# JINXER000/GIE-mapping

Measured on AMD Instinct MI355X. Metric: edt_map_update_throughput, higher is better.
Workload: dtype int32; 1 GPU; 512x512x512 @ 0.05 m, sensor-less hash world (BASELINE config 5): occupied iff hash(x,y,z) < 1 %, full observation, 25 ~; preset=c5, fast_mode=False, tiles=single volume, blocks=360448

## Files before the change

gie-mapping_amd/csrc/gie_api.inc.h:

```cpp
#include <stdio.h>
#include <stdlib.h>
#include <string.h>
#include <math.h>
#include <string>
#include <vector>

enum { GIE_K_CLASSIFY = 0, GIE_K_RAY_REGISTER, GIE_K_RAY_FREE, GIE_K_RAY_FINAL, GIE_K_ALLOC, GIE_K_FUSE, GIE_K_EDT_Y, GIE_K_EDT_X,
       GIE_K_EDT_Z, GIE_K_MARK, GIE_K_FRONTIER, GIE_K_WAVE_A, GIE_K_WAVE_B, GIE_K_WAVE_C, GIE_K_COMMIT, GIE_K_EDT_ZFACES, GIE_K_MARKC, GIE_K_NUM };
#include <cstdio>
#include <unistd.h>
static const char *const gie_kernel_names[GIE_K_NUM] = { "ogm_classify", "ray_register", "ray_free", "ray_finalize", "block_alloc", "fuse",
       "edt_pass_y", "edt_pass_x", "edt_pass_z", "mark", "frontiers", "wave_a", "wave_b", "waves", "commit", "edt_prep", "mark_commit" };

#define GIE_REHASH_PERIOD 64
static thread_local std::string g_gie_err;
static void gie_set_err(const std::string &s) { g_gie_err = s; }
extern "C" const char *gie_last_error(void) { return g_gie_err.c_str(); }

enum gie_owed {
    GIE_OWED_NONE,
    GIE_OWED_FRESH,
    GIE_OWED_STALE
};
struct gie_pivots { int pvt[3], upvt[3], tb0[3]; };
struct gie_pair_state {
    gie_owed owed = GIE_OWED_NONE;
    gie_pivots last = {};
    int flushed_ct = -1;
    int coc_pending = 0;
    int lazy_pending = 0;
    uint32_t *bcoc_alt = nullptr;
    int tsp_pvt[3] = {};
    int fuse_fresh = 0;
    int track_want = 0;
};
struct gie_mapper {
    gie_config cfg;
    gie_ctx c;
    be_state be;
    int ncell;
    int has_pose, has_ogm, merge_open;
    int bar_fault_left;
    gie_pair_state pp;
    int pool_base;
    int evictions;
    long long tomb_bound;
    int retain_box_valid, retain_box_lo[3], retain_box_hi[3];
    int32_t *blk_tab2; int tab_valid, tab_tb0[3];
    int edt_partial;
    int ogm_unlabelled;
    float msg_origin[3];
    float *d_sensor; size_t sensor_cap;
    float *d_pts_g; size_t pts_cap;
    float *d_box_ll, *d_box_ur; uint8_t *d_box_act; int box_cap;
    int32_t *d_rank;
    int32_t *d_srank, *d_slist;
    void *d_stage[2], *h_stage[2];
    std::vector<void *> allocs;
    void *scratch[2]; size_t scratch_cap[2];
    int32_t h_cnt[GIE_CNT_NUM];
    int32_t next_off[3], next_whole[3];
    float us[4];
    const int8_t *labels_pending;
    gie_seendist *d_cm; void *h_cm[2]; size_t cm_bytes; int cm_slot, cm_pending;
    long long *d_round_stats;
};

template <class T> static T *gie_dalloc(gie_mapper *m, size_t n, bool zero = true)
{
    void *p = be_alloc(&m->be, n * sizeof(T), zero);
    if (p) m->allocs.push_back(p);
    {
        static const int dbg = GIE_SWITCH("GIE_DEBUG_ALLOC", 0);
        if (dbg && (dbg > 1 || n * sizeof(T) >= (64u << 20))) fprintf(stderr, "[%d] gie alloc %2d: %p  %8.1f MiB\n", (int)getpid(), (int)m->allocs.size(), p, (double)(n * sizeof(T)) / 1048576.0);
    }
    return (T *)p;
}

static void *gie_scratch(gie_mapper *m, int i, size_t bytes, const char *who)
{
    if (bytes > m->scratch_cap[i]) {
        if (m->scratch[i]) be_free(&m->be, m->scratch[i]);
        m->scratch[i] = be_alloc(&m->be, bytes, false);
        m->scratch_cap[i] = m->scratch[i] ? bytes : 0;
    }
    if (!m->scratch[i]) gie_set_err(std::string(who) + ": device allocation of the export buffer failed");
    return m->scratch[i];
}

#define GIE_SCRATCH_KEEP ((size_t)64 << 20)
static void gie_scratch_trim(gie_mapper *m)
{
    for (int i = 0; i < 2; i++)
        if (m->scratch[i] && m->scratch_cap[i] > GIE_SCRATCH_KEEP) { be_free(&m->be, m->scratch[i]); m->scratch[i] = nullptr; m->scratch_cap[i] = 0; }
}

static void gie_place_calibrate(gie_mapper *m, size_t N, size_t GV)
{
    const int tries = m->cfg.place_tries;
    if (tries <= 1 || N < ((size_t)1 << 24) || !m->c.g_coc || !m->c.pair || !m->c.bcoc || !m->c.glb_type) return;
    gie_ctx &c = m->c;
    (void)be_place_probe(&m->be, c, 12);
    float best = be_place_probe(&m->be, c, 5);
    if (best <= 0.f) return;
    const float first = best;
    struct plane { void **pp; size_t bytes; bool zero; } planes[4] = {
        { reinterpret_cast<void **>(&c.g_coc), GV * sizeof(uint64_t), false }, { reinterpret_cast<void **>(&c.pair), N * sizeof(uint64_t), true },
        { reinterpret_cast<void **>(&c.bcoc), N * sizeof(uint32_t), true }, { reinterpret_cast<void **>(&c.glb_type), N, true } };
    int swaps = 0;
    for (plane &pl : planes) {
        for (int t = 1; t < tries; t++) {
            void *alt = be_alloc(&m->be, pl.bytes, pl.zero);
            if (!alt) break;
            void *old = *pl.pp;
            *pl.pp = alt;
            const float ms = be_place_probe(&m->be, c, 5);
            bool take = ms > 0.f && ms < 0.985f * best;
            if (take) {
                *pl.pp = old;
                const float again = be_place_probe(&m->be, c, 5);
                *pl.pp = alt;
                take = again > 0.f && ms < 0.985f * again;
                if (!take && again > 0.f) best = again;
            }
            if (take) {
                best = ms; swaps++;
                for (void *&q : m->allocs) if (q == old) q = alt;
                be_free(&m->be, old);
            } else { *pl.pp = old; be_free(&m->be, alt); }
        }
    }
    if (GIE_SWITCH("GIE_DEBUG_ALLOC", 0)) fprintf(stderr, "[%d] gie placement: probe %.4f -> %.4f ms after %d re-draws\n", (int)getpid(), first, best, swaps);
}

static int gie_pow2_ge(long long v) { int p = 1; while ((long long)p < v) p <<= 1; return p; }

#define GIE_MAX_POOL_BLOCKS (1 << 26)
static void gie_pp_init(gie_mapper *m); static void gie_pp_pose(gie_mapper *m);
extern "C" gie_mapper *gie_create(const gie_config *cfg)
{
    if (!cfg || cfg->voxel_width <= 0.f || cfg->local_size[0] < 1 || cfg->local_size[1] < 1 || cfg->local_size[2] < 1) {
        gie_set_err("gie_create: bad config"); return nullptr;
    }
    const int X = cfg->local_size[0], Y = cfg->local_size[1], Z = cfg->local_size[2];
    const long long M = (long long)X * X + (long long)Y * Y + (long long)Z * Z;
    const int L = X > Z ? X : Z;
    if (X > 1024 || Y > 1024 || Z > 1024 || M + 1 + (long long)L * L >= (1ll << 22) || (long long)X * Y * Z > 0x7fffffffll) {
        gie_set_err("gie_create: local volume too large (side <= 1024 and X²+Y²+Z²+max(X,Z)² < 2^22)"); return nullptr;
    }
    if (cfg->max_blocks > GIE_MAX_POOL_BLOCKS) {
        gie_set_err("gie_create: max_blocks above 67 108 864 is not supported (and would not fit the device: 19.5 KB per block); "
                    "bound the map with retain_radius_blocks instead");
        return nullptr;
    }
    gie_mapper *m = new gie_mapper();
    m->cfg = *cfg;
    m->has_pose = m->has_ogm = 0; m->merge_open = 0; m->bar_fault_left = 0; m->c.bar_fault = 0; m->edt_partial = 0; m->ogm_unlabelled = 0; m->evictions = 0; m->tomb_bound = 0; m->retain_box_valid = 0; m->labels_pending = nullptr;
    m->d_cm = nullptr; m->h_cm[0] = m->h_cm[1] = nullptr; m->cm_bytes = 0; m->cm_slot = 0; m->cm_pending = 0;
    for (int i = 0; i < 3; i++) { m->next_off[i] = 0; m->next_whole[i] = cfg->local_size[i]; }
    m->d_sensor = nullptr; m->sensor_cap = 0; m->d_pts_g = nullptr; m->pts_cap = 0;
    m->d_box_ll = m->d_box_ur = nullptr; m->d_box_act = nullptr; m->box_cap = 0;
    m->d_srank = m->d_slist = nullptr; m->d_stage[0] = m->d_stage[1] = m->h_stage[0] = m->h_stage[1] = nullptr;
    memset(m->h_cnt, 0, sizeof(m->h_cnt)); memset(m->us, 0, sizeof(m->us));
    m->scratch[0] = m->scratch[1] = nullptr; m->scratch_cap[0] = m->scratch_cap[1] = 0;
    if (cfg->wave_workgroups < 0 || cfg->place_tries < 0) { gie_set_err("gie_create: bad config (wave_workgroups / place_tries are >= 0)"); delete m; return nullptr; }
    if (be_init(&m->be, cfg->device_id, cfg->wave_workgroups) != 0) { delete m; return nullptr; }
    gie_ctx &c = m->c;
    memset(&c, 0, sizeof(c));
    c.X = X; c.Y = Y; c.Z = Z; c.N = X * Y * Z;
    c.voxel_width = cfg->voxel_width; c.occ_thresh = cfg->occupancy_threshold;
    c.min_h = cfg->ogm_min_h; c.max_h = cfg->ogm_max_h; c.cutoff_sq = cfg->cutoff_grids_sq;
    c.fast_mode = cfg->fast_mode; c.for_motion_planner = cfg->for_motion_planner; c.robot_r2 = cfg->robot_r2_grids;
    c.max_width = X + Y + Z; c.max_loc_dist_sq = (int)M;
    if (c.max_width < 1022) {
        c.wr[0] = 2046; c.wr[1] = 2046; c.wr[2] = 1022; c.empty_value = GIE_EMPTY_VALUE; c.invalid_dist_min = 900000;
    } else {
        c.wr[0] = 16382; c.wr[1] = 16382; c.wr[2] = 8190; c.empty_value = 4194303; c.invalid_dist_min = 4000000;
    }
    c.L2G = gie_se3_from_quat(1, 0, 0, 0, 0, 0, 0); c.G2L = gie_se3_inv(c.L2G);
    const size_t N = (size_t)c.N;
    c.ray_count = gie_dalloc<int32_t>(m, N);
    c.inst_type = gie_dalloc<int8_t>(m, N);
    c.glb_type = gie_dalloc<int8_t>(m, N);
    c.edt = gie_dalloc<float>(m, N);
    c.cy1 = gie_dalloc<uint16_t>(m, N);
    c.cxy2 = gie_dalloc<uint32_t>(m, N);
    c.bcoc = gie_dalloc<uint32_t>(m, N);
    m->pp.bcoc_alt = gie_dalloc<uint32_t>(m, N);
    c.pair = gie_dalloc<uint64_t>(m, N);
    c.wl = gie_dalloc<uint32_t>(m, N);
    for (int i = 0; i < 3; i++) c.tfd[i] = (cfg->local_size[i] + 7) / 8;
    const size_t ntile = (size_t)c.tfd[0] * c.tfd[1] * c.tfd[2];
    c.tflag = gie_dalloc<uint8_t>(m, 7 * ntile);
    c.tunk = c.tflag + ntile; c.tsum = c.tflag + 2 * ntile; c.tray = c.tflag + 3 * ntile; c.tact = c.tflag + 4 * ntile;
    c.tknown = c.tflag + 5 * ntile; c.tknown_prev = c.tflag + 6 * ntile;
    c.tmax = gie_dalloc<int32_t>(m, 2 * ntile);
    c.tbmax = gie_dalloc<int32_t>(m, ntile);
    c.tmax_prev = c.tmax ? c.tmax + ntile : nullptr;
    c.tskip = gie_dalloc<uint8_t>(m, 2 * ntile);
    c.tskip_prev = c.tskip ? c.tskip + ntile : nullptr;
    c.tlazy = gie_dalloc<uint8_t>(m, ntile);
    c.scan_labels = nullptr;
    c.ucol = gie_dalloc<uint8_t>(m, (((size_t)X * Y * ((Z + 7) / 8)) + 3) & ~(size_t)3);
    c.zocc = gie_dalloc<uint8_t>(m, (size_t)c.Z);
    c.zneed = gie_dalloc<uint64_t>(m, (size_t)c.tfd[0] * c.tfd[1]);
    c.zredo = gie_dalloc<uint32_t>(m, (size_t)((X + 15) / 16) * Y);
    c.zlist = gie_dalloc<uint16_t>(m, (size_t)c.Z + 8);
    c.zcount = gie_dalloc<int32_t>(m, 4);
    c.tl_known = gie_dalloc<int32_t>(m, ntile);
    c.tl_swept = gie_dalloc<int32_t>(m, ntile);
    c.tl_front = gie_dalloc<int32_t>(m, ntile);
    { const int force = GIE_SWITCH("GIE_TILE_LIST", -1); c.force_lists = force < 0 ? -1 : (force != 0); }
    const int bdr = 2 * (X * Y + Y * Z + X * Z);
    c.lprop = gie_dalloc<uint64_t>(m, (size_t)bdr, false);
    c.cand[0] = gie_dalloc<uint64_t>(m, N, false);
    c.cand[1] = gie_dalloc<uint64_t>(m, N, false);
    for (int i = 0; i < 3; i++) c.tdim[i] = cfg->local_size[i] / 8 + 3;
    m->ncell = c.tdim[0] * c.tdim[1] * c.tdim[2];
    c.blk_tab = gie_dalloc<int32_t>(m, (size_t)m->ncell, false);
    m->blk_tab2 = gie_dalloc<int32_t>(m, (size_t)m->ncell, false);
    c.tab_prev = nullptr; m->tab_valid = 0;
    c.blk_need = gie_dalloc<uint8_t>(m, (size_t)m->ncell);
    c.blk_new = gie_dalloc<int32_t>(m, (size_t)m->ncell);
    m->d_rank = gie_dalloc<int32_t>(m, (size_t)m->ncell);
    long long mb = cfg->max_blocks > 0 ? cfg->max_blocks : 3ll * m->ncell + 4096;
    if (mb > GIE_MAX_POOL_BLOCKS) mb = GIE_MAX_POOL_BLOCKS;
    c.max_blocks = (int)mb;
    const int hcap = gie_pow2_ge(4 * mb);
    c.hmask = (uint32_t)(hcap - 1);
    c.hkeys = gie_dalloc<uint64_t>(m, (size_t)hcap, false);
    c.hvals = gie_dalloc<int32_t>(m, (size_t)hcap, false);
    c.pool_count = gie_dalloc<int32_t>(m, 4);
    m->pool_base = 0;
    c.retain = cfg->retain_radius_blocks > 0 ? cfg->retain_radius_blocks : 0;
    c.free_list = gie_dalloc<int32_t>(m, c.retain > 0 ? (size_t)mb : 1, false);
    const size_t GV = (size_t)mb * GIE_VBSZ;
    c.g_key = gie_dalloc<uint64_t>(m, (size_t)mb, false);
    c.g_nbr = gie_dalloc<int32_t>(m, 8 * (size_t)mb, false);
    c.g_occ = gie_dalloc<uint8_t>(m, GV, false);
    c.g_type = gie_dalloc<int8_t>(m, GV, false);
    c.g_coc = gie_dalloc<uint64_t>(m, GV, false);
    c.g_pair = gie_dalloc<uint64_t>(m, GV, false);
    c.g_prop = gie_dalloc<uint64_t>(m, GV, false);
    c.g_prop2 = gie_dalloc<uint64_t>(m, GV, false);
    for (int i = 0; i < 2; i++) c.wb_list[i] = gie_dalloc<int32_t>(m, (size_t)mb, false);
    c.wb_flag[0] = gie_dalloc<int32_t>(m, 2 * (size_t)mb);
    c.wb_flag[1] = c.wb_flag[0] ? c.wb_flag[0] + mb : nullptr;
    c.g_wl = gie_dalloc<int32_t>(m, GV, false);
    c.g_dirty = gie_dalloc<int32_t>(m, (size_t)mb);
    long long qab = 16ll * bdr; if (qab < 65536) qab = 65536; if (qab > (16 << 20)) qab = 16 << 20;
    long long qc = (long long)c.N; if (qc < 4096) qc = 4096; if (qc > (16 << 20)) qc = 16 << 20;
    c.qcap_ab = (int)qab; c.qcap_c = (int)qc;
    c.qa = gie_dalloc<uint64_t>(m, (size_t)qab, false);
    c.qb = gie_dalloc<uint64_t>(m, (size_t)qab, false);
    c.qa_a = gie_dalloc<gie_vaddr>(m, (size_t)qab, false);
    c.qb_a = gie_dalloc<gie_vaddr>(m, (size_t)qab, false);
    for (int i = 0; i < 2; i++) c.qc[i] = gie_dalloc<int32_t>(m, (size_t)qc, false);
    c.cnt = gie_dalloc<int32_t>(m, GIE_CNT_NUM);
    for (int i = 0; i < 2; i++) c.wc_list[i] = gie_dalloc<int32_t>(m, ntile, false);
    c.wc_flag[0] = gie_dalloc<int32_t>(m, 2 * ntile);
    c.wc_flag[1] = c.wc_flag[0] ? c.wc_flag[0] + ntile : nullptr;
    c.lvl_next = gie_dalloc<int32_t>(m, 6 * GIE_MAX_LEVELS);
    c.lvl_vis = c.lvl_next + GIE_MAX_LEVELS;
    c.lvlb_next = c.lvl_next + 2 * GIE_MAX_LEVELS; c.lvlb_vis = c.lvl_next + 3 * GIE_MAX_LEVELS;
    c.lvla_next = c.lvl_next + 4 * GIE_MAX_LEVELS; c.lvla_vis = c.lvl_next + 5 * GIE_MAX_LEVELS;
    m->d_round_stats = gie_dalloc<long long>(m, 4);
    c.gate = nullptr;
    bool ok = c.cnt != nullptr;
    for (void *p : m->allocs) ok = ok && p != nullptr;
    if (!ok) { gie_set_err("gie_create: device allocation failed"); gie_destroy(m); return nullptr; }
    if (GIE_SWITCH("GIE_DEBUG_POOL_BASE", 0) > 0) {
        const long long b = GIE_SWITCH("GIE_DEBUG_POOL_BASE", 0);
        if (b > 0 && b < mb) {
            const int32_t v = (int32_t)b; be_h2d(&m->be, c.pool_count, &v, sizeof(v)); m->pool_base = (int)b;
            be_memset(&m->be, c.g_key, 0xff, (size_t)b * sizeof(uint64_t));
        }
    }
    gie_place_calibrate(m, N, GV);
    gie_pp_init(m);
    be_memset(&m->be, c.hkeys, 0xff, (size_t)hcap * sizeof(uint64_t));
    be_memset(&m->be, c.lprop, 0xff, (size_t)bdr * sizeof(uint64_t));
    be_memset(&m->be, c.cand[0], 0xff, N * sizeof(uint64_t));
    be_memset(&m->be, c.cand[1], 0xff, N * sizeof(uint64_t));
    be_sync(&m->be);
    return m;
}

extern "C" void gie_destroy(gie_mapper *m)
{
    if (!m) return;
    be_sync(&m->be);
    for (void *p : m->allocs) be_free(&m->be, p);
    if (m->d_sensor) be_free(&m->be, m->d_sensor);
    if (m->d_pts_g) be_free(&m->be, m->d_pts_g);
    if (m->d_box_ll) { be_free(&m->be, m->d_box_ll); be_free(&m->be, m->d_box_ur); be_free(&m->be, m->d_box_act); }
    if (m->d_srank) { be_free(&m->be, m->d_srank); be_free(&m->be, m->d_slist); }
    for (int i = 0; i < 2; i++) if (m->scratch[i]) be_free(&m->be, m->scratch[i]);
    if (m->d_cm) be_free(&m->be, m->d_cm);
    for (int i = 0; i < 2; i++) if (m->h_cm[i]) be_host_free(&m->be, m->h_cm[i]);
    for (int i = 0; i < 2; i++) { if (m->d_stage[i]) be_free(&m->be, m->d_stage[i]); if (m->h_stage[i]) be_host_free(&m->be, m->h_stage[i]); }
    be_fini(&m->be);
    delete m;
}

extern "C" int gie_set_pose(gie_mapper *m, const float pos[3], const float q[4])
{
    if (!m || !pos || !q) { gie_set_err("gie_set_pose: null"); return GIE_ERR_INVALID; }
    gie_ctx &c = m->c;
    int crd[3];
    for (int i = 0; i < 3; i++) {
        if (!(fabsf(pos[i]) <= 1.0e6f)) { gie_set_err("gie_set_pose: position is not finite"); return GIE_ERR_INVALID; }
        crd[i] = gie_pos2coord(pos[i], c.voxel_width);
        if (crd[i] > 900000 || crd[i] < -900000) { gie_set_err("gie_set_pose: position outside the representable map"); return GIE_ERR_INVALID; }
    }
    c.map_ct += 1;
    c.gate = nullptr;
    c.L2G = gie_se3_from_quat(q[0], q[1], q[2], q[3], pos[0], pos[1], pos[2]);
    c.G2L = gie_se3_inv(c.L2G);
    const int sz[3] = { c.X, c.Y, c.Z };
    for (int i = 0; i < 3; i++) {
        c.origin[i] = pos[i];
        c.pvt[i] = crd[i] - sz[i] / 2 + m->next_off[i];
        c.tile_off[i] = m->next_off[i];
        c.whole_lo[i] = -(m->next_whole[i] / 2) + sz[i] / 2 - m->next_off[i];
        c.whole_hi[i] = c.whole_lo[i] + m->next_whole[i];
        m->msg_origin[i] = (float)c.pvt[i] * c.voxel_width;
        c.upvt[i] = crd[i] - c.wr[i] / 2;
        c.tb0[i] = (c.pvt[i] - 1) >> 3;
        c.vb_lo[i] = (c.pvt[i] - 1) >> 3; c.vb_hi[i] = (c.pvt[i] + sz[i]) >> 3;
    }
    c.wr_inside = 1;
    for (int i = 0; i < 3; i++) if (c.pvt[i] - c.upvt[i] < 0 || c.pvt[i] - c.upvt[i] + sz[i] > c.wr[i]) c.wr_inside = 0;
    gie_pp_pose(m);
    c.tab_prev = nullptr;
    const uint32_t f = (uint32_t)c.map_ct & 0x3ffffu;
    if (f == 0) {
        be_memset(&m->be, c.wl, 0, (size_t)c.N * sizeof(uint32_t));
        be_memset(&m->be, c.g_wl, 0xff, (size_t)c.max_blocks * GIE_VBSZ * sizeof(int32_t));
    }
    c.stamp_base = (f + 1u) << 12;
    m->has_pose = 1;
    return GIE_OK;
}

static int gie_need_pose(gie_mapper *m, const char *who)
{
    if (!m) { gie_set_err(std::string(who) + ": null handle"); return GIE_ERR_INVALID; }
    if (!m->has_pose) { gie_set_err(std::string(who) + ": gie_set_pose has not been called"); return GIE_ERR_INVALID; }
    return GIE_OK;
}

static void gie_labels_materialise(gie_mapper *m)
{
    if (!m->labels_pending) return;
    be_labels(&m->be, m->c, m->labels_pending, 0);
    m->labels_pending = nullptr; m->c.scan_labels = nullptr;
}

static int gie_stage_sensor(gie_mapper *m, const float *host, size_t n)
{
    gie_labels_materialise(m);
    if (n > m->sensor_cap) {
        if (m->d_sensor) { be_sync(&m->be); be_free(&m->be, m->d_sensor); }
        m->d_sensor = (float *)be_alloc(&m->be, n * sizeof(float), false);
        m->sensor_cap = m->d_sensor ? n : 0;
        if (!m->d_sensor) { gie_set_err("sensor buffer allocation failed"); return GIE_ERR_DEVICE; }
    }
    be_h2d(&m->be, m->d_sensor, host, n * sizeof(float));
    return GIE_OK;
}

extern "C" int gie_ogm_depth_dev(gie_mapper *m, const float *d_depth, const gie_cam_param *p)
{
    int rc = gie_need_pose(m, "gie_ogm_depth"); if (rc) return rc;
    if (!d_depth || !p || p->rows < 1 || p->cols < 1) { gie_set_err("gie_ogm_depth: bad arguments"); return GIE_ERR_INVALID; }
    gie_labels_materialise(m);
    m->c.pntcld_mode = 0;
    be_time(&m->be, 0);
    op_classify_depth op; op.img = d_depth; op.p = *p;
    be_prof(&m->be, GIE_K_CLASSIFY, 0); be_vox(&m->be, m->c, op); be_prof(&m->be, GIE_K_CLASSIFY, 1);
    be_time(&m->be, 1);
    m->has_ogm = 1;
    return GIE_OK;
}
extern "C" int gie_ogm_depth(gie_mapper *m, const float *depth, const gie_cam_param *p)
{
    int rc = gie_need_pose(m, "gie_ogm_depth"); if (rc) return rc;
    if (!depth || !p || p->rows < 1 || p->cols < 1) { gie_set_err("gie_ogm_depth: bad arguments"); return GIE_ERR_INVALID; }
    rc = gie_stage_sensor(m, depth, (size_t)p->rows * p->cols); if (rc) return rc;
    return gie_ogm_depth_dev(m, m->d_sensor, p);
}
extern "C" int gie_ogm_multiscan_dev(gie_mapper *m, const float *d_ranges, const gie_multiscan_param *p)
{
    int rc = gie_need_pose(m, "gie_ogm_multiscan"); if (rc) return rc;
    if (!d_ranges || !p || p->scan_num < 1 || p->ring_num < 1) { gie_set_err("gie_ogm_multiscan: bad arguments"); return GIE_ERR_INVALID; }
    gie_labels_materialise(m);
    m->c.pntcld_mode = 0;
    be_time(&m->be, 0);
    op_classify_multiscan op; op.img = d_ranges; op.p = *p;
    {
        const double lo = (double)p->phi_min - 0.5 * (double)p->phi_inc, hi = (double)p->phi_min + ((double)p->ring_num - 0.5) * (double)p->phi_inc;
        const double a = (lo < hi ? lo : hi) - 1e-3, b = (lo < hi ? hi : lo) + 1e-3;
        op.fov_test = (a > -1.5 && b < 1.5) ? 1 : 0;
        op.tan_lo = op.fov_test ? (float)(tan(a) - 1e-4 * (1.0 + fabs(tan(a)))) : 0.f;
        op.tan_hi = op.fov_test ? (float)(tan(b) + 1e-4 * (1.0 + fabs(tan(b)))) : 0.f;
    }
    be_prof(&m->be, GIE_K_CLASSIFY, 0); be_vox(&m->be, m->c, op); be_prof(&m->be, GIE_K_CLASSIFY, 1);
    be_time(&m->be, 1);
    m->has_ogm = 1;
    return GIE_OK;
}
extern "C" int gie_ogm_multiscan(gie_mapper *m, const float *ranges, const gie_multiscan_param *p)
{
    int rc = gie_need_pose(m, "gie_ogm_multiscan"); if (rc) return rc;
    if (!ranges || !p || p->scan_num < 1 || p->ring_num < 1) { gie_set_err("gie_ogm_multiscan: bad arguments"); return GIE_ERR_INVALID; }
    rc = gie_stage_sensor(m, ranges, (size_t)p->scan_num * p->ring_num); if (rc) return rc;
    return gie_ogm_multiscan_dev(m, m->d_sensor, p);
}
extern "C" int gie_ogm_scan2d(gie_mapper *m, const float *ranges, const gie_scan_param *p)
{
    int rc = gie_need_pose(m, "gie_ogm_scan2d"); if (rc) return rc;
    if (!ranges || !p || p->scan_num < 1) { gie_set_err("gie_ogm_scan2d: bad arguments"); return GIE_ERR_INVALID; }
    rc = gie_stage_sensor(m, ranges, (size_t)p->scan_num); if (rc) return rc;
    gie_labels_materialise(m);
    m->c.pntcld_mode = 0;
    be_time(&m->be, 0);
    op_classify_scan2d op; op.img = m->d_sensor; op.p = *p;
    be_prof(&m->be, GIE_K_CLASSIFY, 0); be_vox(&m->be, m->c, op); be_prof(&m->be, GIE_K_CLASSIFY, 1);
    be_time(&m->be, 1);
    m->has_ogm = 1;
    return GIE_OK;
}
static int gie_ogm_labels_dev_impl(gie_mapper *m, const int8_t *d_labels, int may_borrow, int *borrowed)
{
    if (borrowed) *borrowed = 0;
    int rc = gie_need_pose(m, "gie_ogm_labels"); if (rc) return rc;
    if (!d_labels) { gie_set_err("gie_ogm_labels: bad arguments"); return GIE_ERR_INVALID; }
    gie_labels_materialise(m);
    m->c.pntcld_mode = 0;
    be_time(&m->be, 0);
    const int in_place = may_borrow && be_labels_in_place_ok(m->c, d_labels);
    be_prof(&m->be, GIE_K_CLASSIFY, 0); be_labels(&m->be, m->c, d_labels, in_place); be_prof(&m->be, GIE_K_CLASSIFY, 1);
    be_time(&m->be, 1);
    if (in_place) { m->labels_pending = d_labels; m->c.scan_labels = d_labels; }
    m->has_ogm = 1;
    if (borrowed) *borrowed = in_place;
    return GIE_OK;
}
extern "C" int gie_ogm_labels_dev(gie_mapper *m, const int8_t *d_labels)
{
    return gie_ogm_labels_dev_impl(m, d_labels, 0, nullptr);
}
extern "C" int gie_ogm_labels_dev_borrow(gie_mapper *m, const int8_t *d_labels, int *borrowed)
{
    return gie_ogm_labels_dev_impl(m, d_labels, 1, borrowed);
}
extern "C" int gie_ogm_labels(gie_mapper *m, const int8_t *labels)
{
    int rc = gie_need_pose(m, "gie_ogm_labels"); if (rc) return rc;
    if (!labels) { gie_set_err("gie_ogm_labels: bad arguments"); return GIE_ERR_INVALID; }
    gie_labels_materialise(m);
    const size_t nfl = ((size_t)m->c.N + 3) / 4;
    if (nfl > m->sensor_cap) {
        if (m->d_sensor) { be_sync(&m->be); be_free(&m->be, m->d_sensor); }
        m->d_sensor = (float *)be_alloc(&m->be, nfl * sizeof(float), false);
        m->sensor_cap = m->d_sensor ? nfl : 0;
        if (!m->d_sensor) { gie_set_err("sensor buffer allocation failed"); return GIE_ERR_DEVICE; }
    }
    be_h2d(&m->be, m->d_sensor, labels, (size_t)m->c.N);
    return gie_ogm_labels_dev_impl(m, (const int8_t *)m->d_sensor, 1, nullptr);
}
extern "C" int gie_ogm_pointcloud_dev(gie_mapper *m, const float *d_xyz, int n)
{
    int rc = gie_need_pose(m, "gie_ogm_pointcloud"); if (rc) return rc;
    if (n < 0 || (n > 0 && !d_xyz)) { gie_set_err("gie_ogm_pointcloud: bad arguments"); return GIE_ERR_INVALID; }
    if ((size_t)n * 3 > m->pts_cap) {
        if (m->d_pts_g) { be_sync(&m->be); be_free(&m->be, m->d_pts_g); }
        m->d_pts_g = (float *)be_alloc(&m->be, (size_t)n * 3 * sizeof(float), false);
        m->pts_cap = m->d_pts_g ? (size_t)n * 3 : 0;
        if (!m->d_pts_g) { gie_set_err("point buffer allocation failed"); return GIE_ERR_DEVICE; }
    }
    gie_labels_materialise(m);
    m->c.pntcld_mode = 1;
    be_time(&m->be, 0);
    if (n > 0) {
        op_register_point r; r.xyz = d_xyz; r.g = m->d_pts_g;
        be_prof(&m->be, GIE_K_RAY_REGISTER, 0); be_lin(&m->be, m->c, r, n); be_prof(&m->be, GIE_K_RAY_REGISTER, 1);
        be_prof(&m->be, GIE_K_RAY_FREE, 0); be_free_rays(&m->be, m->c, m->d_pts_g, n); be_prof(&m->be, GIE_K_RAY_FREE, 1);
// ... 848 lines not shown
```

gie-mapping_amd/csrc/gie_hip.hip:

```cpp
#include <cstdio>
#include <unistd.h>
#include <cstring>
#include <cstdlib>
#include <string>
#include <algorithm>
#include <vector>
#include <hip/hip_runtime.h>
#include <hip/hip_ext.h>
#include <rocprim/rocprim.hpp>
#include "gie_kernels.hip.h"

#define GIE_NEV 8

struct be_state {
    int device;
    int num_cu;
    int cu_total;
    hipStream_t stream;
    hipEvent_t ev[GIE_NEV];
    int ev_set[GIE_NEV];
    void *scan_tmp; size_t scan_bytes;
    void *arena;
    hipEvent_t copy_ev[2];
    hipStream_t side;
    hipEvent_t side_ready, side_done; int side_on, side_busy;
    int prof_on;
    std::vector<hipEvent_t> *pool;
    std::vector<int> *pending;
    int pool_used;
    int cur_id;
    double acc_ms[32]; int acc_n[32];
};
#include <vector>

struct be_arena { char *base; size_t size, top; int k; std::vector<long long> skew; };
static void gie_set_err(const std::string &s);
#include <string>

#define GIE_HIP_OK(expr) do { hipError_t e_ = (expr); if (e_ != hipSuccess) { gie_set_err(std::string(#expr) + ": " + hipGetErrorString(e_)); } } while (0)

#include <mutex>
static std::mutex g_waves_mutex;
static hipEvent_t g_waves_event[64];
static bool g_waves_event_set[64];
static int g_live_mappers[64];

static int be_init(be_state *b, int device, int wave_workgroups)
{
    int n = 0;
    if (hipGetDeviceCount(&n) != hipSuccess || n <= 0) { gie_set_err("no HIP device visible (libgie_hip.so needs an AMD GPU; there is no CPU fallback)"); return 1; }
    if (device < 0 || device >= n) { gie_set_err("bad device_id"); return 1; }
    b->device = device;
    if (hipSetDevice(device) != hipSuccess) { gie_set_err("hipSetDevice failed"); return 1; }
    { hipDeviceProp_t pr; b->num_cu = (hipGetDeviceProperties(&pr, device) == hipSuccess && pr.multiProcessorCount > 0) ? pr.multiProcessorCount : 64; }
    b->cu_total = b->num_cu;
    b->num_cu = b->num_cu >= 64 ? b->num_cu / 2 : b->num_cu;
    if (wave_workgroups > 0) b->num_cu = wave_workgroups < b->cu_total ? wave_workgroups : b->cu_total;
    {
        int per_cu = 0, per_cu_c = 0;
        hipError_t oe = hipOccupancyMaxActiveBlocksPerMultiprocessor(&per_cu, reinterpret_cast<const void *>(&k_waves_ab), GIE_WAVE_THREADS, 0);
        if (oe == hipSuccess) oe = hipOccupancyMaxActiveBlocksPerMultiprocessor(&per_cu_c, reinterpret_cast<const void *>(&k_waves_c), GIE_WAVE_THREADS, 0);
        if (per_cu_c < per_cu) per_cu = per_cu_c;
        if (oe != hipSuccess || per_cu < 1) {
            gie_set_err(std::string("the wavefront kernels cannot be resident on this device (occupancy query: ") + hipGetErrorString(oe) + ", " + std::to_string(per_cu) + " workgroups per compute unit)");
            (void)hipGetLastError();
            return 1;
        }
        if (b->num_cu > per_cu * b->cu_total) b->num_cu = per_cu * b->cu_total;
    }
    if (hipStreamCreateWithFlags(&b->stream, hipStreamNonBlocking) != hipSuccess) { gie_set_err("hipStreamCreate failed"); return 1; }
    for (int i = 0; i < GIE_NEV; i++) { GIE_HIP_OK(hipEventCreate(&b->ev[i])); b->ev_set[i] = 0; }
    b->scan_tmp = nullptr; b->scan_bytes = 0; b->arena = nullptr; b->side_on = 0; b->side_busy = 0;
    for (int i = 0; i < 2; i++) GIE_HIP_OK(hipEventCreateWithFlags(&b->copy_ev[i], hipEventDisableTiming));
    b->prof_on = 0; b->cur_id = -1; b->pool = new std::vector<hipEvent_t>(); b->pending = new std::vector<int>(); b->pool_used = 0;
    for (int i = 0; i < 32; i++) { b->acc_ms[i] = 0; b->acc_n[i] = 0; }
    {
        std::lock_guard<std::mutex> lock(g_waves_mutex);
        if (++g_live_mappers[device & 63] == 2) (void)hipDeviceSynchronize();
    }
    return 0;
}
static void be_fini(be_state *b)
{
    { std::lock_guard<std::mutex> lock(g_waves_mutex); g_live_mappers[b->device & 63]--; }
    if (b->scan_tmp) (void)hipFree(b->scan_tmp);
    for (hipEvent_t e : *b->pool) (void)hipEventDestroy(e);
    delete b->pool; delete b->pending;
    for (int i = 0; i < GIE_NEV; i++) (void)hipEventDestroy(b->ev[i]);
    for (int i = 0; i < 2; i++) (void)hipEventDestroy(b->copy_ev[i]);
    (void)hipStreamDestroy(b->stream);
    if (b->side_on) { (void)hipStreamSynchronize(b->side); (void)hipEventDestroy(b->side_ready); (void)hipEventDestroy(b->side_done); (void)hipStreamDestroy(b->side); }
    if (b->arena) { be_arena *a = (be_arena *)b->arena; if (a->base) (void)hipFree(a->base); delete a; b->arena = nullptr; }
}
static be_arena *be_arena_of(be_state *b)
{
#if !defined(GIE_TEST_HOOKS)
    (void)b; return nullptr;
#else
    static const char *e = getenv("GIE_ARENA_MB");
    if (!e || atoll(e) <= 0) return nullptr;
    if (!b->arena) {
        be_arena *a = new be_arena();
        a->size = (size_t)atoll(e) << 20; a->top = 0; a->k = 0; a->base = nullptr;
        if (const char *sk = getenv("GIE_ARENA_SKEW")) { std::string t(sk); size_t i = 0; while (i < t.size()) { size_t j = t.find(',', i); if (j == std::string::npos) j = t.size(); a->skew.push_back(atoll(t.substr(i, j - i).c_str())); i = j + 1; } }
        if (hipMalloc((void **)&a->base, a->size) != hipSuccess) { a->base = nullptr; a->size = 0; }
        b->arena = a;
    }
    return (be_arena *)b->arena;
#endif
}
static void *be_alloc(be_state *b, size_t bytes, bool zero)
{
    void *p = nullptr;
    (void)hipSetDevice(b->device);
    be_arena *a = bytes >= ((size_t)64 << 20) ? be_arena_of(b) : nullptr;
    if (a && a->base) {
        const size_t sk = (size_t)((a->k < (int)a->skew.size() ? a->skew[a->k] : 0) << 20);
        const size_t at = ((a->top + ((size_t)2 << 20) - 1) & ~(((size_t)2 << 20) - 1)) + sk;
        if (at + bytes <= a->size) { p = a->base + at; a->top = at + bytes; a->k++; }
    }
    if (!p && hipMalloc(&p, bytes ? bytes : 1) != hipSuccess) return nullptr;
    if (zero) GIE_HIP_OK(hipMemsetAsync(p, 0, bytes, b->stream));
    return p;
}
static void be_free(be_state *b, void *p)
{
    (void)hipStreamSynchronize(b->stream);
    be_arena *a = (be_arena *)b->arena;
    if (a && a->base && (char *)p >= a->base && (char *)p < a->base + a->size) return;
    (void)hipFree(p);
}
static void be_memset(be_state *b, void *p, int v, size_t bytes) { GIE_HIP_OK(hipMemsetAsync(p, v, bytes, b->stream)); }
static void be_h2d(be_state *b, void *d, const void *h, size_t bytes)
{
    GIE_HIP_OK(hipMemcpyAsync(d, h, bytes, hipMemcpyHostToDevice, b->stream));
    GIE_HIP_OK(hipStreamSynchronize(b->stream));
}
static void be_d2h(be_state *b, void *h, const void *d, size_t bytes)
{
    GIE_HIP_OK(hipMemcpyAsync(h, d, bytes, hipMemcpyDeviceToHost, b->stream));
    GIE_HIP_OK(hipStreamSynchronize(b->stream));
}
static void *be_host_alloc(be_state *b, size_t bytes) { void *p = nullptr; (void)hipSetDevice(b->device); return hipHostMalloc(&p, bytes, hipHostMallocDefault) == hipSuccess ? p : nullptr; }
static void be_host_free(be_state *, void *p) { (void)hipHostFree(p); }
static void be_d2h_async(be_state *b, void *h, const void *d, size_t bytes, int slot)
{
    GIE_HIP_OK(hipMemcpyAsync(h, d, bytes, hipMemcpyDeviceToHost, b->stream));
    GIE_HIP_OK(hipEventRecord(b->copy_ev[slot], b->stream));
}
static void be_wait(be_state *b, int slot) { GIE_HIP_OK(hipEventSynchronize(b->copy_ev[slot])); }
static void be_side_on(be_state *b)
{
    if (b->side_on) return;
    (void)hipSetDevice(b->device);
    GIE_HIP_OK(hipStreamCreateWithFlags(&b->side, hipStreamNonBlocking));
    GIE_HIP_OK(hipEventCreateWithFlags(&b->side_ready, hipEventDisableTiming));
    GIE_HIP_OK(hipEventCreateWithFlags(&b->side_done, hipEventDisableTiming));
    b->side_on = 1;
}
static void be_side_copy_begin(be_state *b) { be_side_on(b); if (b->side_busy) GIE_HIP_OK(hipStreamWaitEvent(b->stream, b->side_done, 0)); }
static void be_side_copy(be_state *b, void *h, const void *d, size_t bytes)
{
    be_side_on(b);
    GIE_HIP_OK(hipEventRecord(b->side_ready, b->stream));
    GIE_HIP_OK(hipStreamWaitEvent(b->side, b->side_ready, 0));
    GIE_HIP_OK(hipMemcpyAsync(h, d, bytes, hipMemcpyDeviceToHost, b->side));
    GIE_HIP_OK(hipEventRecord(b->side_done, b->side));
    b->side_busy = 1;
}
static int be_side_copy_wait(be_state *b)
{
    if (!b->side_busy) return 0;
    const hipError_t e = hipEventSynchronize(b->side_done);
    if (e != hipSuccess) { gie_set_err(std::string("hipEventSynchronize: ") + hipGetErrorString(e)); return 1; }
    return 0;
}
static void *be_stream_handle(be_state *b) { return (void *)b->stream; }
static int be_sync(be_state *b)
{
    hipError_t e = hipStreamSynchronize(b->stream);
    if (e != hipSuccess) { gie_set_err(std::string("hipStreamSynchronize: ") + hipGetErrorString(e)); return 1; }
    e = hipGetLastError();
    if (e != hipSuccess) { gie_set_err(std::string("HIP error: ") + hipGetErrorString(e)); return 1; }
    return 0;
}
static void be_time(be_state *b, int i)
{
    if (!b->prof_on) { b->ev_set[i] = 0; return; }
    GIE_HIP_OK(hipEventRecord(b->ev[i], b->stream)); b->ev_set[i] = 1;
}
static void be_times(be_state *b, float *ogm, float *fuse, float *edt, float *merge)
{
    float *out[4] = { ogm, fuse, edt, merge };
    for (int k = 0; k < 4; k++) {
        float ms = 0.f;
        if (b->ev_set[2 * k] && b->ev_set[2 * k + 1] && hipEventElapsedTime(&ms, b->ev[2 * k], b->ev[2 * k + 1]) == hipSuccess) *out[k] = ms * 1000.f;
        else *out[k] = 0.f;
    }
}

static int be_prof_event(be_state *b)
{
    if (b->pool_used == (int)b->pool->size()) { hipEvent_t e; GIE_HIP_OK(hipEventCreate(&e)); b->pool->push_back(e); }
    return b->pool_used++;
}
static int be_trace_on() { static const int on = GIE_SWITCH("GIE_TRACE_LAUNCHES", 0); return on; }
#define GIE_LAUNCH(b, kern, grid, block, lds, ...) do { \
        if (be_trace_on()) { fprintf(stderr, "[%d] launch %s\n", (int)getpid(), #kern); fflush(stderr); } \
        GIE_LAUNCH_(b, kern, grid, block, lds, __VA_ARGS__); \
        if (be_trace_on()) { hipError_t e_ = hipStreamSynchronize((b)->stream); if (e_ != hipSuccess) { fprintf(stderr, "[%d] %s: %s\n", (int)getpid(), #kern, hipGetErrorString(e_)); fflush(stderr); } } \
    } while (0)
#define GIE_LAUNCH_(b, kern, grid, block, lds, ...) do { \
        if ((b)->prof_on && (b)->cur_id >= 0) { \
            const int e0_ = be_prof_event(b), e1_ = be_prof_event(b); \
            hipExtLaunchKernelGGL(kern, grid, block, lds, (b)->stream, (*(b)->pool)[e0_], (*(b)->pool)[e1_], 0, __VA_ARGS__); \
            (b)->pending->push_back((b)->cur_id); (b)->pending->push_back(e0_); (b)->pending->push_back(e1_); \
        } else hipLaunchKernelGGL(kern, grid, block, lds, (b)->stream, __VA_ARGS__); \
    } while (0)
static void be_prof_resolve(be_state *b)
{
    if (b->pending->empty()) { b->pool_used = 0; return; }
    GIE_HIP_OK(hipStreamSynchronize(b->stream));
    for (size_t i = 0; i + 2 < b->pending->size(); i += 3) {
        float ms = 0.f;
        if (hipEventElapsedTime(&ms, (*b->pool)[(*b->pending)[i + 1]], (*b->pool)[(*b->pending)[i + 2]]) == hipSuccess) {
            b->acc_ms[(*b->pending)[i]] += ms;
        }
    }
    b->pending->clear(); b->pool_used = 0;
}
static void be_prof(be_state *b, int id, int end)
{
    if (!b->prof_on) return;
    if (!end) {
        if (b->pool_used > 4000) be_prof_resolve(b);
        b->cur_id = id;
    } else { b->cur_id = -1; b->acc_n[id] += 1; }
}
static void be_prof_enable(be_state *b, int on) { be_prof_resolve(b); b->prof_on = on; b->cur_id = -1; }
static void be_prof_collect(be_state *b, float *ms, int *n, int num)
{
    be_prof_resolve(b);
    for (int i = 0; i < num; i++) { ms[i] = (float)b->acc_ms[i]; n[i] = b->acc_n[i]; b->acc_ms[i] = 0; b->acc_n[i] = 0; }
}

template <class F> static void be_vox(be_state *b, const gie_ctx &c, const F &f)
{
    dim3 blk(GIE_VOX_BX, GIE_VOX_BY, 1);
    dim3 grd((c.X + GIE_VOX_BX - 1) / GIE_VOX_BX, (c.Y + GIE_VOX_BY - 1) / GIE_VOX_BY, (c.Z + GIE_VOX_ZPER - 1) / GIE_VOX_ZPER);
    GIE_LAUNCH(b, k_voxz<F>, grd, blk, 0, c, f);
}
template <class F> static void be_lin(be_state *b, const gie_ctx &c, const F &f, int n)
{
    if (n <= 0) return;
    GIE_LAUNCH(b, k_lin<F>, dim3((n + 255) / 256), dim3(256), 0, c, f, n);
}
static void be_flush_clear(be_state *b, const gie_ctx &c, const op_pair_flush &f, int n, const gie_clear_list &l)
{
    const int nclr = gie_clear_total_wgs(l);
    GIE_LAUNCH(b, k_flush_clear, dim3(nclr + (n + 255) / 256), dim3(256), 0, c, f, n, l, nclr);
}
static int be_labels_in_place_ok(const gie_ctx &c, const int8_t *labels)
{ return (c.X & 15) == 0 && !c.for_motion_planner && ((uintptr_t)labels & 15) == 0; }
static void be_labels(be_state *b, const gie_ctx &c, const int8_t *labels, int in_place = 0)
{
    if ((c.X & 15) == 0 && !c.for_motion_planner && ((uintptr_t)labels & 15) == 0) {
        const int nvec = c.N >> 4;
        if (in_place) GIE_LAUNCH(b, k_labels16<false>, dim3((nvec + 255) / 256), dim3(256), 0, c, labels, nvec);
        else GIE_LAUNCH(b, k_labels16<true>, dim3((nvec + 255) / 256), dim3(256), 0, c, labels, nvec);
    } else { op_classify_labels op; op.labels = labels; be_vox(b, c, op); }
}
static void be_clear(be_state *b, const gie_clear_list &l, const int32_t *gate = nullptr)
{
    if (l.n > 0) GIE_LAUNCH(b, k_clear, dim3(gie_clear_total_wgs(l)), dim3(256), 0, l, gate);
}
static void be_round_note(be_state *b, const gie_ctx &c, int32_t *changed, long long *stats, const int32_t *go, int end)
{
    GIE_LAUNCH(b, k_round_note, dim3(1), dim3(64), 0, c, changed, stats, go, end);
}
static void be_block_alloc(be_state *b, const gie_ctx &c, int ncell, int32_t *, int clear_list, int fuse_list_ntile = 0)
{
    if (clear_list) GIE_HIP_OK(hipMemsetAsync(&c.cnt[GIE_CNT_NEWLIST], 0, sizeof(int32_t), b->stream));
    GIE_LAUNCH(b, k_cell_alloc, dim3((ncell + 255) / 256), dim3(256), 0, c, ncell);
    static const int imult = GIE_SWITCH("GIE_INIT_MULT", 4);
    const int ninit = b->cu_total * imult;
    int nfl = (fuse_list_ntile + 255) / 256; if (nfl > 2 * b->cu_total) nfl = 2 * b->cu_total;
    GIE_LAUNCH(b, k_block_init_list, dim3(ninit + nfl), dim3(256), 0, c, ninit, fuse_list_ntile);
}
static void be_free_rays(be_state *b, const gie_ctx &c, const float *g, int n)
{
    if (n <= 0) return;
    GIE_LAUNCH(b, k_free_rays, dim3((n + 63) / 64), dim3(64 * GIE_RAY_SEGS), 0, c, g, n, gie_ray_max_steps(c));
}
static void be_exclusive_scan(be_state *b, const int32_t *flag, int32_t *rank, int n)
{
    size_t bytes = 0;
    (void)hipSetDevice(b->device);
    GIE_HIP_OK(rocprim::exclusive_scan(nullptr, bytes, flag, rank, 0, (size_t)n, rocprim::plus<int32_t>(), b->stream));
    if (bytes > b->scan_bytes) {
        if (b->scan_tmp) { (void)hipStreamSynchronize(b->stream); (void)hipFree(b->scan_tmp); }
        GIE_HIP_OK(hipMalloc(&b->scan_tmp, bytes)); b->scan_bytes = bytes;
    }
    GIE_HIP_OK(rocprim::exclusive_scan(b->scan_tmp, bytes, flag, rank, 0, (size_t)n, rocprim::plus<int32_t>(), b->stream));
}

template <int CP, int TX, int WAVES> static void gie_launch_edt_z(be_state *b, const gie_ctx &c, int full)
{
    constexpr int LP = 64 * CP;
    const size_t tile = ((size_t)c.Z * (TX + 1) + 3) & ~(size_t)3;
    const size_t lds = tile * 4 + (size_t)WAVES * LP * 8 + (size_t)LP * 2 + 16;
    static bool attr_done = false;
    if (!attr_done) {
        GIE_HIP_OK(hipFuncSetAttribute(reinterpret_cast<const void *>(&k_edt_z<CP, TX, WAVES>), hipFuncAttributeMaxDynamicSharedMemorySize, 160 * 1024));
        attr_done = true;
    }
    const int ntx = (c.X + TX - 1) / TX, ntiles = ntx * c.Y;
    int wgs = (int)((160 * 1024) / (lds + 256));
    if (wgs < 1) wgs = 1; if (wgs > 4) wgs = 4;
    int grid = wgs * b->cu_total; if (grid > (ntiles + 1) / 2) grid = (ntiles + 1) / 2;
    GIE_LAUNCH(b, (k_edt_z<CP, TX, WAVES>), dim3(grid), dim3(64 * WAVES), lds, c, ntx, ntiles, full);
}
template <int CP> static void gie_launch_edt_xz(be_state *b, const gie_ctx &c, bool zpass, int full, int zs_fused = 0, bool redo = false)
{
    if (redo) {
        GIE_LAUNCH(b, k_edt_x_redo<CP>, dim3(b->cu_total * 8), dim3(64 * GIE_EDTX_WAVES), 0, c);
    } else if (!zpass) {
        GIE_LAUNCH(b, k_edt_x<CP>, dim3((c.Y + GIE_EDTX_WAVES - 1) / GIE_EDTX_WAVES, c.Z), dim3(64 * GIE_EDTX_WAVES), 0, c, zs_fused, full);
    } else {
        gie_launch_edt_z<CP, 16, 8>(b, c, full);
    }
}
static void gie_launch_edt_dim(be_state *b, const gie_ctx &c, int L, bool zpass, int full, int zs_fused = 0, bool redo = false)
{
    if (L <= 64) gie_launch_edt_xz<1>(b, c, zpass, full, zs_fused, redo);
    else if (L <= 128) gie_launch_edt_xz<2>(b, c, zpass, full, zs_fused, redo);
    else if (L <= 256) gie_launch_edt_xz<4>(b, c, zpass, full, zs_fused, redo);
    else if (L <= 512) gie_launch_edt_xz<8>(b, c, zpass, full, zs_fused, redo);
    else gie_launch_edt_xz<16>(b, c, zpass, full, zs_fused, redo);
}
static int be_zs_mode(const gie_ctx &c)
{
    if (c.Z < 64 || c.Z > 1024) return 0;
    static const int on = GIE_SWITCH("GIE_ZSTREAM", 1);
    static const int fused = GIE_SWITCH("GIE_ZS_FUSED", 1);
    return on ? ((fused && (c.X & 1) == 0) ? 2 : 1) : 0;
}
static int be_edt_z_stream(be_state *b, const gie_ctx &c, int full);
static void be_edt_z_rest(be_state *b, const gie_ctx &c, int full, int zs)
{
    if (zs == 2) gie_launch_edt_dim(b, c, c.X, false, full, 0, true);
    gie_launch_edt_dim(b, c, c.Z, true, full);
}
static void be_edt_z(be_state *b, const gie_ctx &c, int full) { be_edt_z_rest(b, c, full, be_edt_z_stream(b, c, full) ? be_zs_mode(c) : 0); }
template <bool STAGED, class F> static void be_vox_list(be_state *b, const gie_ctx &c, const F &f, const int32_t *list, int count_idx, int always_list, int lx = 64)
{
    static const int mult = GIE_SWITCH("GIE_VOXA_MULT", 32);
    const dim3 g(b->cu_total * mult), t(256);
    if (lx == 32) GIE_LAUNCH(b, (k_voxa<F, STAGED, 32>), g, t, 0, c, f, list, count_idx, always_list);
    else if (lx == 16) GIE_LAUNCH(b, (k_voxa<F, STAGED, 16>), g, t, 0, c, f, list, count_idx, always_list);
    else if (lx == 8) GIE_LAUNCH(b, (k_voxa<F, STAGED, 8>), g, t, 0, c, f, list, count_idx, always_list);
    else GIE_LAUNCH(b, (k_voxa<F, STAGED, 64>), g, t, 0, c, f, list, count_idx, always_list);
}
static void be_markc(be_state *b, const gie_ctx &c, const int32_t *list)
{
    static const int generic = GIE_SWITCH("GIE_MARKC_GENERIC", 0);
    static const int lx = GIE_SWITCH("GIE_MARKC_LX", 32);
    static const int mult = GIE_SWITCH("GIE_VOXA_MULT", 64);
    if (generic) { be_vox_list<true>(b, c, op_markc(), list, GIE_CNT_TL_KNOWN, 0, lx == 16 || lx == 8 || lx == 32 ? lx : 64); return; }
    static const int lmult = GIE_SWITCH("GIE_MARKC_LGRID", 40);
    const dim3 g(b->cu_total * ((c.coc_defer && c.lazy_ok) ? lmult : mult)), t(256);
    if (lx == 16) GIE_LAUNCH(b, k_markc<16>, g, t, 0, c, list);
    else if (lx == 64) GIE_LAUNCH(b, k_markc<64>, g, t, 0, c, list);
    else GIE_LAUNCH(b, k_markc<32>, g, t, 0, c, list);
}
static float be_place_probe(be_state *b, const gie_ctx &c, int reps, int streams = 15)
{
    static const int mult = GIE_SWITCH("GIE_VOXA_MULT", 64);
    const long long ntile = (long long)c.tfd[0] * c.tfd[1] * c.tfd[2];
    const int nslot = (int)(ntile < c.max_blocks ? ntile : c.max_blocks);
    hipEvent_t e0, e1;
    if (hipEventCreate(&e0) != hipSuccess || hipEventCreate(&e1) != hipSuccess) return -1.f;
    std::vector<float> ms;
    hipLaunchKernelGGL(k_place_probe, dim3(b->cu_total * mult), dim3(256), 0, b->stream, c, nslot, streams);
    for (int r = 0; r < reps; r++) {
        (void)hipEventRecord(e0, b->stream);
        hipLaunchKernelGGL(k_place_probe, dim3(b->cu_total * mult), dim3(256), 0, b->stream, c, nslot, streams);
        (void)hipEventRecord(e1, b->stream);
        (void)hipEventSynchronize(e1);
        float t = 0.f; (void)hipEventElapsedTime(&t, e0, e1); ms.push_back(t);
    }
    (void)hipEventDestroy(e0); (void)hipEventDestroy(e1);
    std::sort(ms.begin(), ms.end());
    GIE_HIP_OK(hipMemsetAsync(c.pair, 0, (size_t)c.N * sizeof(uint64_t), b->stream));
    return ms.empty() ? -1.f : ms[ms.size() / 2];
}
static int be_rows_mode() { static const int v = GIE_SWITCH("GIE_ROWS", 1); return v ? 2 : 0; }
static void be_fuse(be_state *b, const gie_ctx &c, const int32_t *list)
{
    static const int mult = GIE_SWITCH("GIE_ROWS_MULT", 32);
    if (be_rows_mode()) {
        if (c.pntcld_mode) GIE_LAUNCH(b, k_fuse_rows<true>, dim3(b->cu_total * mult), dim3(256), 0, c, op_fuse(), list);
        else GIE_LAUNCH(b, k_fuse_rows<false>, dim3(b->cu_total * mult), dim3(256), 0, c, op_fuse(), list);
    }
    else be_vox_list<true>(b, c, op_fuse(), list, GIE_CNT_TL_FUSE, 0);
}
static void be_frontier_tiles(be_state *b, const gie_ctx &c, const int32_t *known, int known_idx, const int32_t *list, int count_idx)
{
    gie_face_patches fp;
    const int da[6] = { c.Y, c.Y, c.X, c.X, c.X, c.X }, db[6] = { c.Z, c.Z, c.Z, c.Z, c.Y, c.Y };
    fp.off[0] = 0;
    for (int f = 0; f < 6; f++) { fp.na[f] = (da[f] + 7) / 8; fp.off[f + 1] = fp.off[f] + fp.na[f] * ((db[f] + 7) / 8); }
    const long long ntile = (long long)c.tfd[0] * c.tfd[1] * c.tfd[2];
    int nsum = (int)((ntile + 64 * GIE_FF_WAVES - 1) / (64 * GIE_FF_WAVES));
    if (nsum > 2 * b->cu_total) nsum = 2 * b->cu_total;
    const int nface = (fp.off[6] + GIE_FF_WAVES - 1) / GIE_FF_WAVES;
    GIE_LAUNCH(b, k_frontier_faces, dim3(nsum + nface), dim3(64 * GIE_FF_WAVES), 0, c, fp, known, known_idx, nsum);
    static int mult = GIE_SWITCH("GIE_FRONT_MULT", 0);
    if (mult <= 0) {
        int per_cu = 0;
        if (hipOccupancyMaxActiveBlocksPerMultiprocessor(&per_cu, reinterpret_cast<const void *>(&k_frontier_tiles), 64 * GIE_FR_WAVES, 0) != hipSuccess || per_cu < 1) per_cu = 2;
        mult = per_cu;
    }
    GIE_LAUNCH(b, k_frontier_tiles, dim3(b->cu_total * mult), dim3(64 * GIE_FR_WAVES), 0, c, list, count_idx);
}
static void be_edt_z_direct(be_state *b, const gie_ctx &c)
{
    GIE_LAUNCH(b, k_edt_z_direct, dim3(b->cu_total * 16), dim3(256), 0, c);
}
static int be_edt_z_stream(be_state *b, const gie_ctx &c, int full)
{
    const int zs = be_zs_mode(c);
    if (!zs) return 0;
    const int nxr = (c.X + 63) / 64;
    static const int target = GIE_SWITCH("GIE_ZSTREAM_WAVES", 8);
    const long long want = (long long)b->cu_total * 4 * target;
    int nseg = (int)((want + (long long)nxr * c.Y - 1) / ((long long)nxr * c.Y));
    const int maxseg = c.Z / 64 > 0 ? c.Z / 64 : 1;
    if (nseg > maxseg) nseg = maxseg; if (nseg < 1) nseg = 1;
    int seg_len = ((c.Z + nseg - 1) / nseg + 31) & ~31;
    nseg = (c.Z + seg_len - 1) / seg_len;
    const long long waves = (long long)nxr * nseg * c.Y;
    long long grid = (waves + 3) / 4;
    const long long cap = (long long)b->cu_total * 8 * 4;
    if (grid > cap) grid = cap;
    if (!full && grid < (long long)b->cu_total * 16) grid = (long long)b->cu_total * 16;
    if (zs == 2) GIE_LAUNCH(b, k_edt_z_stream<true>, dim3((unsigned)grid), dim3(256), 0, c, full, nseg, seg_len, zs);
    else GIE_LAUNCH(b, k_edt_z_stream<false>, dim3((unsigned)grid), dim3(256), 0, c, full, nseg, seg_len, zs);
    return 1;
}
static void be_tile_oldskip(be_state *b, const gie_ctx &c, const int pupvt[3])
{
    const int ntile = c.tfd[0] * c.tfd[1] * c.tfd[2];
    int32_t *const count = &c.cnt[GIE_CNT_STATE1];
    GIE_LAUNCH(b, k_tile_oldskip, dim3((ntile + 255) / 256), dim3(256), 0, c, ntile, c.wc_list[0], count);
    if (c.catchup_fast) GIE_LAUNCH(b, k_coc_catchup_new, dim3(b->cu_total * 8), dim3(256), 0, c, pupvt[0], pupvt[1], pupvt[2], c.wc_list[0], count);
}
static void be_pair_materialise(be_state *b, const gie_ctx &c, int stay)
{
    const int ntile = c.tfd[0] * c.tfd[1] * c.tfd[2];
    int32_t *const count = &c.cnt[GIE_CNT_STATE2];
    GIE_LAUNCH(b, k_pair_lazy_list, dim3((ntile + 255) / 256), dim3(256), 0, c, ntile, stay, c.wc_list[1], count);
    GIE_LAUNCH(b, k_pair_lazy_run, dim3(b->cu_total * 8), dim3(256), 0, c, c.wc_list[1], count);
}
static void be_coc_catchup(be_state *b, const gie_ctx &c, const gie_catchup &p)
{
    const int ntile = c.tfd[0] * c.tfd[1] * c.tfd[2];
    int32_t *const count = &c.cnt[GIE_CNT_STATE1];
    GIE_HIP_OK(hipMemsetAsync(count, 0, sizeof(int32_t), b->stream));
    GIE_LAUNCH(b, k_coc_catchup_list, dim3((ntile + 255) / 256), dim3(256), 0, c, p, ntile, c.wc_list[0], count);
    GIE_LAUNCH(b, k_coc_catchup_run, dim3(b->cu_total * 4), dim3(256), 0, c, p, c.wc_list[0], count);
}
static void be_edt_prep(be_state *b, const gie_ctx &c)
{
    const int ncol = c.tfd[0] * c.tfd[1];
    GIE_LAUNCH(b, k_edt_prep, dim3((ncol + GIE_PREP_WAVES - 1) / GIE_PREP_WAVES), dim3(64 * GIE_PREP_WAVES), 0, c, ncol);
}
static void be_edt(be_state *b, const gie_ctx &c, int full)
{
    dim3 gy((c.X + GIE_EDTY_COLS - 1) / GIE_EDTY_COLS, c.Z);
    be_prof(b, 6, 0);
    static const int y4 = GIE_SWITCH("GIE_EDTY4", 1);
    if (y4 && (c.X & 3) == 0) {
        const int yb = c.Y > 512 ? 32 : 16, nq = (c.Y + yb - 1) / yb;
        const int lanes = (y4 == 3) ? 32 : 16;
        dim3 g4((c.X / 4 + lanes - 1) / lanes, c.Z), b4(lanes, nq);
        if (yb == 16 && lanes == 16) GIE_LAUNCH(b, (k_edt_y4<16, 16>), g4, b4, 0, c);
        else if (yb == 16) GIE_LAUNCH(b, (k_edt_y4<16, 32>), g4, b4, 0, c);
        else if (lanes == 16) GIE_LAUNCH(b, (k_edt_y4<32, 16>), g4, b4, 0, c);
        else GIE_LAUNCH(b, (k_edt_y4<32, 32>), g4, b4, 0, c);
    }
    else if (c.Y <= 256) GIE_LAUNCH(b, (k_edt_y<8, 8>), gy, dim3(GIE_EDTY_COLS, 8), 0, c);
    else if (c.Y <= 512) GIE_LAUNCH(b, (k_edt_y<16, 16>), gy, dim3(GIE_EDTY_COLS, 16), 0, c);
    else GIE_LAUNCH(b, (k_edt_y<32, 16>), gy, dim3(GIE_EDTY_COLS, 16), 0, c);
    be_prof(b, 6, 1);
    const int zs = be_zs_mode(c);
    be_prof(b, 7, 0); gie_launch_edt_dim(b, c, c.X, false, full, zs == 2 ? zs : 0); be_prof(b, 7, 1);
    be_prof(b, 8, 0);
    const int zl = be_edt_z_stream(b, c, full);
    if (!zl && !full) be_edt_z_direct(b, c);
    be_edt_z_rest(b, c, full, zl ? zs : 0);
    be_prof(b, 8, 1);

}
static void be_waves(be_state *b, const gie_ctx &c, int with_ab, int record_seeds, int clear_first)
{
    std::lock_guard<std::mutex> lock(g_waves_mutex);
    const int dv = b->device & 63;
    (void)hipSetDevice(b->device);
    const bool chain = g_live_mappers[dv] > 1;
    if (chain) {
        if (g_waves_event_set[dv]) GIE_HIP_OK(hipStreamWaitEvent(b->stream, g_waves_event[dv], 0));
        else { GIE_HIP_OK(hipEventCreateWithFlags(&g_waves_event[dv], hipEventDisableTiming)); g_waves_event_set[dv] = true; }
    }
    if (clear_first) {
        GIE_HIP_OK(hipMemsetAsync(&c.cnt[GIE_CNT_BAR_B], 0, 2 * sizeof(int32_t), b->stream));
        GIE_HIP_OK(hipMemsetAsync(c.lvl_next, 0, 2 * GIE_MAX_LEVELS * sizeof(int32_t), b->stream));
    }
    if (with_ab) GIE_LAUNCH(b, k_waves_ab, dim3(b->num_cu), dim3(GIE_WAVE_THREADS), 0, c);
    GIE_LAUNCH(b, k_waves_c, dim3(b->num_cu), dim3(GIE_WAVE_THREADS), 0, c, with_ab, record_seeds);
    if (chain) GIE_HIP_OK(hipEventRecord(g_waves_event[dv], b->stream));
}

#include "gie_api.inc.h"
```

gie-mapping_amd/csrc/gie_kernels.hip.h:

```cpp
#ifndef GIE_KERNELS_HIP_H
#define GIE_KERNELS_HIP_H

#include <hip/hip_runtime.h>
#include "gie_functors.h"

#if defined(GIE_WAVE_TIMING) || defined(GIE_RAY_TIMING)
#include "../../tools/measure/gie_timing.h"
#endif
#if !defined(GIE_WAVE_TIMING)
#define GIE_TS2(tag, n) do { } while (0)
#define GIE_WPROF_DECL do { } while (0)
#define GIE_WPROF_MARK(base) do { } while (0)
#define GIE_WPROF_ADD(i, v) do { } while (0)
#define GIE_WPROF_END(base) do { } while (0)
#define GIE_WPROF_DRAIN() do { } while (0)
#define GIE_WPROF_SUB(i) do { } while (0)
#define GIE_WPROF_SUBSTART() do { } while (0)
#define GIE_WPROF_DUMP() do { } while (0)
#define GIE_WPROF_CLK() 0ull
#define GIE_WAVE_TIMING_RESET(cond) do { } while (0)
#endif
#if !defined(GIE_RAY_TIMING)
#define GIE_RTS(k) do { } while (0)
#endif
// ... 33 lines not shown
    } else {
#pragma unroll
        for (int k = 0; k < GIE_VOX_ZPER; k++)
            if (!sk[k]) f(c, x, y, z0 + k);
    }
}

template <class F>
__global__ __launch_bounds__(256) void k_lin(const gie_ctx c, const F f, const int n)
{
    if (GIE_GATE_CLOSED(c)) return;
    const int i = blockIdx.x * 256 + threadIdx.x;
    if (i < n) f(c, i);
}

template <bool STORE>
__global__ __launch_bounds__(256) void k_labels16(const gie_ctx c, const int8_t *labels, const int nvec)
{
    const int v = blockIdx.x * 256 + threadIdx.x;
    if (v >= nvec) return;
    const int xv = c.X >> 4;
    const int x0 = (v % xv) << 4, row = v / xv, y = row % c.Y, z = row / c.Y;
    const uint4 q = reinterpret_cast<const uint4 *>(labels)[v];
    uint32_t w[4] = { q.x, q.y, q.z, q.w };
    unsigned known = 0;
#pragma unroll
    for (int j = 0; j < 4; j++) {
#pragma unroll
        for (int b = 0; b < 4; b++) {
            const uint32_t l = (w[j] >> (8 * b)) & 0xffu;
            const bool ok = (l == (uint32_t)GIE_VOX_FREE) | (l == (uint32_t)GIE_VOX_OCCUPIED);
            if (!ok) w[j] &= ~(0xffu << (8 * b));
            known |= (ok ? 1u : 0u) << (4 * j + b);
        }
    }
    if (STORE) reinterpret_cast<uint4 *>(c.inst_type)[v] = make_uint4(w[0], w[1], w[2], w[3]);
    if (!known) return;
    const int gx0 = x0 + c.pvt[0], gy = y + c.pvt[1], gz = z + c.pvt[2];
    const int cell0 = (((gz >> 3) - c.tb0[2]) * c.tdim[1] + ((gy >> 3) - c.tb0[1])) * c.tdim[0] - c.tb0[0];
    const int b0 = gx0 >> 3, b1 = (gx0 + 15) >> 3;
    for (int bx = b0; bx <= b1; bx++) {
        const int lo = max(bx * 8 - gx0, 0), hi = min(bx * 8 + 7 - gx0, 15);
        const unsigned m = ((2u << hi) - 1u) & ~((1u << lo) - 1u);
        if (known & m) c.blk_need[cell0 + bx] = 1;
    }
}

#ifndef GIE_RAY_SEGS
#define GIE_RAY_SEGS 8
#endif
#ifndef GIE_RAY_SPIN_SLEEP
#define GIE_RAY_SPIN_SLEEP 4
#endif
__device__ __forceinline__ int gie_ray_cell(const gie_ctx &c, const gie_dda &d, int &lx, int &ly, int &lz)
{
    lx = d.cur[0] - c.pvt[0]; ly = d.cur[1] - c.pvt[1]; lz = d.cur[2] - c.pvt[2];
    const bool in = ((unsigned)lx < (unsigned)c.X) & ((unsigned)ly < (unsigned)c.Y) & ((unsigned)lz < (unsigned)c.Z);
    return in ? __mul24(__mul24(lz, c.Y) + ly, c.X) + lx : -1;
}
__device__ __forceinline__ void gie_ray_touch_k(const gie_ctx &c, const gie_dda &d, const int lx, const int ly, const int lz, gie_ray_marks *last)
{
    const int t = __mul24(__mul24(lz >> 3, c.tfd[1]) + (ly >> 3), c.tfd[0]) + (lx >> 3);
    const int b = __mul24(__mul24((d.cur[2] >> 3) - c.tb0[2], c.tdim[1]) + ((d.cur[1] >> 3) - c.tb0[1]), c.tdim[0]) + ((d.cur[0] >> 3) - c.tb0[0]);
    if ((t != last->tile) | (b != last->blk)) { c.tray[t] = 1; c.blk_need[b] = 1; last->tile = t; last->blk = b; }
}
__device__ __forceinline__ bool gie_dda_before(const gie_dda &d, const float limit)
{
    return fminf(fminf(d.tMax[0], d.tMax[1]), d.tMax[2]) < limit;
}

__device__ __forceinline__ void gie_dda_skip_to(gie_dda &d, const float limit, const int max_steps)
{
    float t0 = d.tMax[0], t1 = d.tMax[1], t2 = d.tMax[2];
    int n0 = 0, n1 = 0, n2 = 0;
    for (int k0 = 0; k0 < max_steps && __any((t0 < limit) | (t1 < limit) | (t2 < limit)); k0 += 8) {
#pragma unroll
        for (int k = 0; k < 8; k++) {
            const bool a0 = t0 < limit, a1 = t1 < limit, a2 = t2 < limit;
            t0 += a0 ? d.tDelta[0] : 0.0f; n0 += a0 ? 1 : 0;
            t1 += a1 ? d.tDelta[1] : 0.0f; n1 += a1 ? 1 : 0;
            t2 += a2 ? d.tDelta[2] : 0.0f; n2 += a2 ? 1 : 0;
        }
    }
    d.cur[0] += d.step[0] * n0; d.tMax[0] = t0;
    d.cur[1] += d.step[1] * n1; d.tMax[1] = t1;
    d.cur[2] += d.step[2] * n2; d.tMax[2] = t2;
}

__global__ __launch_bounds__(64 * GIE_RAY_SEGS) void k_free_rays(const gie_ctx c, const float *g, const int n, const int max_steps)
{
    __shared__ int s_stop[64];
    __shared__ int s_cur[GIE_RAY_SEGS][3][64];
    __shared__ float s_tmax[GIE_RAY_SEGS][3][64];
    __shared__ int s_ready[GIE_RAY_SEGS];
    const int lane = threadIdx.x & 63, seg = threadIdx.x >> 6;
    const int i = blockIdx.x * 64 + lane;
    const bool ray = i < n && gie_point_ok(g[3 * (i < n ? i : 0)], g[3 * (i < n ? i : 0) + 1], g[3 * (i < n ? i : 0) + 2]);
    if (seg == 0) s_stop[lane] = 0x7fffffff;
    if (threadIdx.x < GIE_RAY_SEGS) s_ready[threadIdx.x] = 0;
    gie_dda d;
    int s0[3] = { 0, 0, 0 };
    gie_ray_marks last_tile = { -1, -1 };
    const bool walk = ray && gie_dda_init(c, g, i, d, s0);
    if (!walk) {
#pragma unroll
        for (int k = 0; k < 3; k++) { d.cur[k] = 0; d.step[k] = 0; d.tMax[k] = 3.402823466e+38f; d.tDelta[k] = 0.0f; }
        d.len = 0.0f;
    }
    __syncthreads();
    const float L = walk ? (d.len < d.max_length ? d.len : d.max_length) : 0.0f;
    float Ts = 0.0f, Te = L;
    bool open_end = true;
    if (walk) {
        const float w = c.voxel_width;
        const int dim[3] = { c.X, c.Y, c.Z };
        float tin = 0.0f, tout = 3.402823466e+38f;
        bool hit = true;
#pragma unroll
        for (int a = 0; a < 3; a++) {
            const float lo = ((float)c.pvt[a] - 1.5f) * w, hi = ((float)(c.pvt[a] + dim[a]) + 0.5f) * w;
            if (d.step[a] != 0) {
                const float inv = (float)d.step[a] * d.tDelta[a] / w;
                const float ta = (lo - c.origin[a]) * inv, tb = (hi - c.origin[a]) * inv;
                tin = fmaxf(tin, fminf(ta, tb)); tout = fminf(tout, fmaxf(ta, tb));
            } else if (c.origin[a] < lo || c.origin[a] > hi) hit = false;
        }
        const float slack = 2.0f * w;
        float te_box = tout + slack;
        Ts = fmaxf(0.0f, tin - slack);
        if (!hit || !(Ts < te_box)) { Ts = 0.0f; te_box = 0.0f; }
        if (te_box < L) { Te = te_box; open_end = false; }
        if (Ts > Te) Ts = Te;
    }
    const float Tn = (seg + 1 < GIE_RAY_SEGS) ? Ts + (Te - Ts) * ((float)(seg + 1) * (1.0f / (float)GIE_RAY_SEGS))
                                              : (open_end ? __builtin_inff() : Te);
    if (seg == 0) {
        const int id0 = (ray && gie_in_loc(c, s0[0], s0[1], s0[2])) ? gie_lid(c, s0[0], s0[1], s0[2]) : -1;
        if (id0 >= 0) gie_ray_touch(c, s0[0], s0[1], s0[2], &last_tile);
        gie_wave_add(c, (id0 >= 0 && c.inst_type[id0] != GIE_VOX_OCCUPIED) ? id0 : -1, -1);
        gie_dda_skip_to(d, Ts, max_steps);
    } else {
        volatile int *rdy = &s_ready[seg - 1];
        while (*rdy == 0) __builtin_amdgcn_s_sleep(GIE_RAY_SPIN_SLEEP);
        __builtin_amdgcn_fence(__ATOMIC_ACQUIRE, "workgroup");
#pragma unroll
        for (int k = 0; k < 3; k++) { d.cur[k] = s_cur[seg - 1][k][lane]; d.tMax[k] = s_tmax[seg - 1][k][lane]; }
    }
    GIE_RTS(0);
    const int base = seg << 20;
    const gie_dda at_start = d;
    if (seg + 1 < GIE_RAY_SEGS) {
        gie_dda nx = d;
        gie_dda_skip_to(nx, Tn, max_steps);
#pragma unroll
        for (int k = 0; k < 3; k++) { s_cur[seg][k][lane] = nx.cur[k]; s_tmax[seg][k][lane] = nx.tMax[k]; }
        __builtin_amdgcn_fence(__ATOMIC_RELEASE, "workgroup");
        if (lane == 0) { volatile int *w = &s_ready[seg]; *w = 1; }
    }
    GIE_RTS(1);
    if (walk) {
        int stop = 0x7fffffff;
        bool more = true;
        for (int k0 = 0; k0 < max_steps && more && stop == 0x7fffffff; k0 += GIE_RAY_BATCH) {
            if (*(volatile int *)&s_stop[lane] < base) break;
            int ids[GIE_RAY_BATCH], end[GIE_RAY_BATCH];
            bool went[GIE_RAY_BATCH];
#pragma unroll
            for (int j = 0; j < GIE_RAY_BATCH; j++) {
                went[j] = gie_dda_before(d, Tn);
                end[j] = 0; ids[j] = -1;
                if (went[j]) { int lx, ly, lz; end[j] = gie_dda_step(d); ids[j] = gie_ray_cell(c, d, lx, ly, lz); }
            }
            int8_t ty[GIE_RAY_BATCH];
#pragma unroll
            for (int j = 0; j < GIE_RAY_BATCH; j++) ty[j] = ids[j] >= 0 ? c.inst_type[ids[j]] : (int8_t)GIE_VOX_UNKNOWN;
#pragma unroll
            for (int j = 0; j < GIE_RAY_BATCH; j++) {
                if (stop != 0x7fffffff || !went[j]) continue;
                if (ty[j] == GIE_VOX_OCCUPIED) stop = base + k0 + j;
                else if (end[j]) stop = base + k0 + j + 1;
            }
            more = went[GIE_RAY_BATCH - 1];
        }
        if (stop != 0x7fffffff) atomicMin(&s_stop[lane], stop);
    }
    GIE_RTS(2);
    __syncthreads();
    GIE_RTS(3);
    const int stop = s_stop[lane];
    d = at_start;
    for (int k = 0; k < max_steps; k++) {
        int id = -1;
        const bool went = walk && base + k < stop && gie_dda_before(d, Tn);
        if (went) {
            int lx, ly, lz;
            gie_dda_step(d);
            id = gie_ray_cell(c, d, lx, ly, lz);
            if (id >= 0) gie_ray_touch_k(c, d, lx, ly, lz, &last_tile);
        }
        if (__ballot(went) == 0ull) break;
        if (__ballot(id >= 0) == 0ull) continue;
        gie_wave_add(c, id, -1);
    }
    GIE_RTS(4);
}

__device__ __forceinline__ void gie_clear_part(const gie_clear_list &l, int w)
{
    int r = 0, nw = gie_clear_wgs(l.bytes[0]);
    while (w >= nw && r + 1 < l.n) { w -= nw; r++; nw = gie_clear_wgs(l.bytes[r]); }
    if (w >= nw) return;
    unsigned char *p = (unsigned char *)l.p[r];
    const uint32_t bytes = l.bytes[r];
    const uint32_t head = (uint32_t)((16u - ((uintptr_t)p & 15u)) & 15u) < bytes ? (uint32_t)((16u - ((uintptr_t)p & 15u)) & 15u) : bytes;
    const uint32_t nvec = (bytes - head) / 16u, tail0 = head + nvec * 16u;
    const uint32_t tid = (uint32_t)w * 256u + threadIdx.x, nth = (uint32_t)nw * 256u;
    for (uint32_t i = tid; i < head; i += nth) p[i] = 0;
    uint4 *v = (uint4 *)(p + head);
    for (uint32_t i = tid; i < nvec; i += nth) v[i] = make_uint4(0, 0, 0, 0);
    for (uint32_t i = tail0 + tid; i < bytes; i += nth) p[i] = 0;
}
__global__ __launch_bounds__(256) void k_clear(const gie_clear_list l, const int32_t *gate)
{
    if (gate != nullptr && *(const volatile int32_t *)gate == 0) return;
    gie_clear_part(l, (int)blockIdx.x);
}

__global__ __launch_bounds__(256) void k_flush_clear(const gie_ctx c, const op_pair_flush f, const int n, const gie_clear_list l, const int nclr)
{
    if ((int)blockIdx.x >= nclr) { const int i = ((int)blockIdx.x - nclr) * 256 + (int)threadIdx.x; if (i < n) f(c, i); return; }
    gie_clear_part(l, (int)blockIdx.x);
}

__global__ __launch_bounds__(256) void k_cell_alloc(const gie_ctx c, const int ncell)
{
    if (GIE_GATE_CLOSED(c)) return;
    const int i = blockIdx.x * 256 + threadIdx.x;
    int found = -1;
    bool isnew = false;
    if (i < ncell) {
        const int bx = i % c.tdim[0], by = (i / c.tdim[0]) % c.tdim[1], bz = i / (c.tdim[0] * c.tdim[1]);
        found = gie_cell_prev_slot(c, bx, by, bz);
        if (found < 0) found = gie_hash_find(c, bx + c.tb0[0], by + c.tb0[1], bz + c.tb0[2]);
        isnew = found < 0 && c.blk_need[i];
        c.blk_need[i] = 0;
    }
    __shared__ int s_cnt[4], s_base[4];
    const int lane = __lane_id(), wave = threadIdx.x >> 6;
    const unsigned long long m = __ballot(isnew);
    if (lane == 0) s_cnt[wave] = __popcll(m);
    __syncthreads();
    const int c0 = s_cnt[0], c1 = s_cnt[1], c2 = s_cnt[2], c3 = s_cnt[3];
    const int cnt = c0 + c1 + c2 + c3;
    if (cnt > 0) {
        if (threadIdx.x == 0) {
            int ftop = 0, nf = 0, base = 0;
            if (c.retain > 0) { ftop = atomicSub(&c.pool_count[1], cnt); nf = ftop < 0 ? 0 : (ftop < cnt ? ftop : cnt); }
            if (cnt > nf) base = atomicAdd(&c.pool_count[0], cnt - nf);
            const int lbase = atomicAdd(&c.cnt[GIE_CNT_NEWLIST], cnt);
            atomicAdd(&c.cnt[GIE_CNT_NEWBLK], cnt);
            s_base[0] = base; s_base[1] = lbase; s_base[2] = nf; s_base[3] = ftop;
        }
        __syncthreads();
        if (isnew) {
            const int base = s_base[0], lbase = s_base[1], nf = s_base[2], ftop = s_base[3];
            const int before = (wave > 0 ? c0 : 0) + (wave > 1 ? c1 : 0) + (wave > 2 ? c2 : 0);
            const int r = before + __popcll(m & ((1ull << lane) - 1ull));
            const int slot = gie_alloc_slot(c, r, nf, ftop, base);
            if (slot >= c.max_blocks) { gie_aor32(&c.cnt[GIE_CNT_ERR], GIE_ERRF_POOL); c.blk_new[lbase + r] = -1; }
            else { gie_cell_insert(c, i, slot); c.blk_new[lbase + r] = slot; found = slot; }
        }
    }
    if (i < ncell) {
        c.blk_tab[i] = found;
        if (found >= 0) gie_cell_mark_tiles(c, i);
    }
}
__global__ __launch_bounds__(256) void k_block_init_list(const gie_ctx c, const int ninit, const int ntile)
{
    if (GIE_GATE_CLOSED(c)) return;
    if ((int)blockIdx.x >= ninit) {
        const op_fuse_list f;
        const int nfl = (int)gridDim.x - ninit;
        for (int i0 = ((int)blockIdx.x - ninit) * 256; i0 < ntile; i0 += nfl * 256) {
            const int i = i0 + (int)threadIdx.x;
            f(c, i < ntile ? i : -1);
        }
        return;
    }
    const int n = c.cnt[GIE_CNT_NEWLIST];
    if (blockIdx.x == 0 && threadIdx.x == 0) {
        if (c.pool_count[0] > c.max_blocks) c.pool_count[0] = c.max_blocks;
        if (c.pool_count[1] < 0) c.pool_count[1] = 0;
    }
    for (int e = blockIdx.x; e < n; e += ninit) {
        const int slot = c.blk_new[e];
        if (slot < 0) continue;
        gie_init_voxel(c, slot, threadIdx.x);
        gie_init_voxel(c, slot, threadIdx.x + 256);
        if (threadIdx.x < 6) gie_nbr_link(c, slot, (int)threadIdx.x);
    }
}

#ifndef GIE_EDTY_COLS
#define GIE_EDTY_COLS 64
#endif
template <int YW, int TPC>
__global__ __launch_bounds__(GIE_EDTY_COLS * TPC) void k_edt_y(const gie_ctx c)
{
    constexpr int QW = YW / TPC;
    __shared__ uint32_t s_bits[YW][GIE_EDTY_COLS];
    const int col = threadIdx.x, q = threadIdx.y;
    const int x = blockIdx.x * GIE_EDTY_COLS + col;
    const int z = blockIdx.y;
    if (!c.zocc[z]) return;
    const int X = c.X, Y = c.Y;
    const bool in = x < X;
    const int8_t *t = c.glb_type + (size_t)z * X * Y + (in ? x : 0);
#pragma unroll
    for (int j = 0; j < QW; j++) {
        const int w = q * QW + j;
        uint32_t m = 0;
        if (in && w * 32 < Y) {
#pragma unroll
            for (int k = 0; k < 32; k++) {
                const int y = w * 32 + k;
                if (y < Y) m |= (uint32_t)(t[(size_t)y * X] == GIE_VOX_OCCUPIED) << k;
            }
        }
        s_bits[w][col] = m;
    }
    __syncthreads();
    if (!in) return;
    uint32_t bits[YW];
#pragma unroll
    for (int w = 0; w < YW; w++) bits[w] = s_bits[w][col];
    int prev_last[YW], next_first[YW];
    int last = -1;
#pragma unroll
    for (int w = 0; w < YW; w++) { prev_last[w] = last; if (bits[w]) last = w * 32 + 31 - __clz(bits[w]); }
    int first = -1;
#pragma unroll
    for (int w = YW - 1; w >= 0; w--) { next_first[w] = first; if (bits[w]) first = w * 32 + __ffs(bits[w]) - 1; }
    uint16_t *out = c.cy1 + (size_t)z * X * Y + x;
#pragma unroll
    for (int w = 0; w < YW; w++) {
        if (w / QW != q) continue;
        if (w * 32 >= Y) break;
        const uint32_t bw = bits[w];
        const int pl = prev_last[w], nf = next_first[w];
        for (int k = 0; k < 32; k++) {
            const int y = w * 32 + k;
            if (y >= Y) break;
            const uint32_t lo = bw & (0xffffffffu >> (31 - k));
            const int below = lo ? w * 32 + 31 - __clz(lo) : pl;
            const uint32_t hi = bw >> k;
            const int above = hi ? y + __ffs(hi) - 1 : nf;
            int r;
            if (above >= 0 && (below < 0 || above - y <= y - below)) r = above; else r = below;
            out[(size_t)y * X] = r < 0 ? (uint16_t)0xffff : (uint16_t)r;
        }
    }
}

template <int YB, int LANES>
__global__ __launch_bounds__(32 * LANES) void k_edt_y4(const gie_ctx c)
{
    __shared__ __attribute__((aligned(16))) uint32_t s_m[32][LANES * 4];
    const int l = threadIdx.x, q = threadIdx.y, nq = blockDim.y;
    const int x = (blockIdx.x * LANES + l) * 4;
    const int z = blockIdx.y;
    if (!c.zocc[z]) return;
    const int X = c.X, Y = c.Y;
    const bool in = x < X;
    const size_t base = (size_t)z * X * Y + (in ? x : 0);
    uint32_t m[4] = {0u, 0u, 0u, 0u};
    if (in) {
        const int8_t *t = c.glb_type + base;
        uint32_t v[YB];
#pragma unroll
        for (int k = 0; k < YB; k++) {
            const int y = q * YB + k;
            v[k] = *reinterpret_cast<const uint32_t *>(t + (size_t)min(y, Y - 1) * X);
        }
        const uint32_t ymask = (q * YB + YB <= Y) ? 0xffffffffu : ((q * YB < Y) ? (0xffffffffu >> (32 - (Y - q * YB))) : 0u);
#pragma unroll
        for (int k = 0; k < YB; k++) {
#pragma unroll
            for (int cc = 0; cc < 4; cc++) m[cc] |= (uint32_t)(((v[k] >> (8 * cc)) & 0xffu) == (uint32_t)GIE_VOX_OCCUPIED) << k;
        }
#pragma unroll
        for (int cc = 0; cc < 4; cc++) m[cc] &= ymask;
    }
    *reinterpret_cast<uint4 *>(&s_m[q][4 * l]) = make_uint4(m[0], m[1], m[2], m[3]);
    __syncthreads();
    if (!in) return;
    int pl[4] = {-1, -1, -1, -1}, nf[4] = {-1, -1, -1, -1};
    for (int w = 0; w < q; w++) {
        const uint4 o = *reinterpret_cast<const uint4 *>(&s_m[w][4 * l]);
        const uint32_t ow[4] = {o.x, o.y, o.z, o.w};
#pragma unroll
        for (int cc = 0; cc < 4; cc++) if (ow[cc]) pl[cc] = w * YB + 31 - __clz(ow[cc]);
    }
    for (int w = nq - 1; w > q; w--) {
        const uint4 o = *reinterpret_cast<const uint4 *>(&s_m[w][4 * l]);
        const uint32_t ow[4] = {o.x, o.y, o.z, o.w};
#pragma unroll
        for (int cc = 0; cc < 4; cc++) if (ow[cc]) nf[cc] = w * YB + __ffs(ow[cc]) - 1;
    }
    uint16_t *out = c.cy1 + base;
#pragma unroll
    for (int k = 0; k < YB; k++) {
        const int y = q * YB + k;
        if (y >= Y) break;
        uint32_t r4[4];
#pragma unroll
        for (int cc = 0; cc < 4; cc++) {
            const uint32_t bw = m[cc];
            const uint32_t lo = bw & (0xffffffffu >> (31 - k));
            const int below = lo ? q * YB + 31 - __clz(lo) : pl[cc];
            const uint32_t hi = bw >> k;
            const int above = hi ? y + __ffs(hi) - 1 : nf[cc];
            int r;
            if (above >= 0 && (below < 0 || above - y <= y - below)) r = above; else r = below;
            r4[cc] = r < 0 ? 0xffffu : (uint32_t)r;
        }
        *reinterpret_cast<uint2 *>(out + (size_t)y * X) = make_uint2(r4[0] | (r4[1] << 16), r4[2] | (r4[3] << 16));
    }
}

__device__ __forceinline__ void gie_wave_sync()
{
    __builtin_amdgcn_fence(__ATOMIC_RELEASE, "wavefront");
    __builtin_amdgcn_wave_barrier();
    __builtin_amdgcn_fence(__ATOMIC_ACQUIRE, "wavefront");
}

__device__ __forceinline__ uint32_t gie_scan_sites(const uint2 *ce, const int up, const int lo, const int hi)
{
    uint32_t b0 = 0xffffffffu, b1 = 0xffffffffu, b2 = 0xffffffffu, b3 = 0xffffffffu;
    for (int j = lo; j <= hi; j += 4) {
        const uint2 v0 = ce[j], v1 = ce[min(j + 1, hi)], v2 = ce[min(j + 2, hi)], v3 = ce[min(j + 3, hi)];
        const int d0 = up - (int)(v0.y & 0xffffu), d1 = up - (int)(v1.y & 0xffffu);
        const int d2 = up - (int)(v2.y & 0xffffu), d3 = up - (int)(v3.y & 0xffffu);
        b0 = min(b0, (uint32_t)__mul24(d0, d0) + v0.x);
        b1 = min(b1, (uint32_t)__mul24(d1, d1) + v1.x);
        b2 = min(b2, (uint32_t)__mul24(d2, d2) + v2.x);
        b3 = min(b3, (uint32_t)__mul24(d3, d3) + v3.x);
    }
    return min(min(b0, b1), min(b2, b3));
}

template <int CP>
__device__ __forceinline__ void gie_row_argmin(const uint2 *ce, const int K, const int L, const int lane, int (&sj)[CP])
{
    const int u0 = lane * CP;
    int s0;
    {
        const int g8 = lane & ~7, r = lane & 7;
        const int ug = g8 * CP;
        uint32_t b0 = 0xffffffffu, b1 = 0xffffffffu, b2 = 0xffffffffu, b3 = 0xffffffffu;
        {
            const int up = ug << 5, kl = K - 1;
            for (int j = r; j < K; j += 32) {
                const uint2 v0 = ce[j], v1 = ce[min(j + 8, kl)], v2 = ce[min(j + 16, kl)], v3 = ce[min(j + 24, kl)];
                const int d0 = up - (int)(v0.y & 0xffffu), d1 = up - (int)(v1.y & 0xffffu);
                const int d2 = up - (int)(v2.y & 0xffffu), d3 = up - (int)(v3.y & 0xffffu);
                b0 = min(b0, (uint32_t)__mul24(d0, d0) + v0.x);
                b1 = min(b1, (uint32_t)__mul24(d1, d1) + v1.x);
                b2 = min(b2, (uint32_t)__mul24(d2, d2) + v2.x);
                b3 = min(b3, (uint32_t)__mul24(d3, d3) + v3.x);
            }
        }
        uint32_t bg = min(min(b0, b1), min(b2, b3));
        bg = min(bg, (uint32_t)__shfl_xor((int)bg, 1));
        bg = min(bg, (uint32_t)__shfl_xor((int)bg, 2));
        bg = min(bg, (uint32_t)__shfl_xor((int)bg, 4));
        const int sg = (ug < L) ? (int)(bg & 1023u) : K - 1;
        int sn = __shfl_down(sg, 8);
        if (lane >= 56) sn = K - 1;
        s0 = sg;
        if (r != 0 && u0 < L && sn > sg) s0 = (int)(gie_scan_sites(ce, u0 << 5, sg, sn) & 1023u);
        if (u0 >= L) s0 = K - 1;
    }
    int sup = __shfl_down(s0, 1);
    if (lane == 63) sup = K - 1;
    int sx[CP + 1];
    sx[0] = s0; sx[CP] = sup;
#pragma unroll
    for (int step = CP / 2; step >= 1; step >>= 1) {
#pragma unroll
        for (int m = step; m < CP; m += 2 * step) {
            const int u = u0 + m;
            const int lo = sx[m - step], hi = sx[m + step];
            int r = lo;
            if (u < L && hi > lo) r = (int)(gie_scan_sites(ce, u << 5, lo, hi) & 1023u);
            sx[m] = (u < L) ? r : K - 1;
        }
    }
#pragma unroll
    for (int m = 0; m < CP; m++) sj[m] = sx[m];
}

#define GIE_BAND_MAXK 160
template <int CP>
__device__ __forceinline__ void gie_row_argmin_banded(const uint2 *ce, const int K, const int L, const int lane, int (&sj)[CP], const unsigned bandneed = ~0u)
{
    constexpr int G = 64 / CP;
    const int b = lane / G, r = lane % G;
    uint32_t b0 = 0xffffffffu, b1 = 0xffffffffu;
    {
        const int up = (64 * b) << 5, kl = K - 1;
        for (int j = r; j < K; j += 2 * G) {
            const uint2 v0 = ce[j], v1 = ce[min(j + G, kl)];
            const int d0 = up - (int)(v0.y & 0xffffu), d1 = up - (int)(v1.y & 0xffffu);
            b0 = min(b0, (uint32_t)__mul24(d0, d0) + v0.x);
            b1 = min(b1, (uint32_t)__mul24(d1, d1) + v1.x);
        }
    }
    uint32_t bg = min(b0, b1);
#pragma unroll
    for (int w = 1; w < G; w <<= 1) bg = min(bg, (uint32_t)__shfl_xor((int)bg, w));
    const int sg = (64 * b < L) ? (int)(bg & 1023u) : K - 1;
    int sa[CP + 1];
#pragma unroll
    for (int m = 0; m < CP; m++) sa[m] = __builtin_amdgcn_readlane(sg, m * G);
    sa[CP] = K - 1;
#pragma unroll
    for (int m = 0; m < CP; m++) {
        if (!((bandneed >> m) & 1u)) { sj[m] = 0; continue; }
        const int lo = sa[m], hi = sa[m + 1];
        const int up = (64 * m + lane) << 5;
        uint32_t c0 = 0xffffffffu, c1 = 0xffffffffu, c2 = 0xffffffffu, c3 = 0xffffffffu;
        for (int j = lo; j <= hi; j += 4) {
            const uint2 v0 = ce[j], v1 = ce[min(j + 1, hi)], v2 = ce[min(j + 2, hi)], v3 = ce[min(j + 3, hi)];
            const int d0 = up - (int)(v0.y & 0xffffu), d1 = up - (int)(v1.y & 0xffffu);
            const int d2 = up - (int)(v2.y & 0xffffu), d3 = up - (int)(v3.y & 0xffffu);
            c0 = min(c0, (uint32_t)__mul24(d0, d0) + v0.x);
            c1 = min(c1, (uint32_t)__mul24(d1, d1) + v1.x);
            c2 = min(c2, (uint32_t)__mul24(d2, d2) + v2.x);
            c3 = min(c3, (uint32_t)__mul24(d3, d3) + v3.x);
        }
        sj[m] = (int)(min(min(c0, c1), min(c2, c3)) & 1023u);
    }
}

#ifndef GIE_BAND_TRIP
#define GIE_BAND_TRIP 8
#endif
#define GIE_BAND_PAD 16
__device__ __forceinline__ void gie_row_mb_pad(int2 *mb, const int K, const int lane)
{
    if (lane < GIE_BAND_PAD - 1) mb[K + lane] = make_int2(0, 0x7fffffff);
}
template <int CP>
__device__ __forceinline__ void gie_row_argmin_banded_lin(const int2 *mb, const int K, const int L, const int lane, int (&sj)[CP])
{
    constexpr int G = 64 / CP;
    const int b = lane / G, r = lane % G;
    int b0 = 0x7fffffff, b1 = 0x7fffffff, b2 = 0x7fffffff, b3 = 0x7fffffff;
    {
        const int u = 64 * b, kl = K - 1;
        for (int j = r; j < K; j += 4 * G) {
            const int2 v0 = mb[j], v1 = mb[min(j + G, kl)], v2 = mb[min(j + 2 * G, kl)], v3 = mb[min(j + 3 * G, kl)];
            b0 = min(b0, __mul24(u, v0.x) + v0.y);
            b1 = min(b1, __mul24(u, v1.x) + v1.y);
            b2 = min(b2, __mul24(u, v2.x) + v2.y);
            b3 = min(b3, __mul24(u, v3.x) + v3.y);
        }
    }
    int bg = min(min(b0, b1), min(b2, b3));
#pragma unroll
    for (int w = 1; w < G; w <<= 1) bg = min(bg, __shfl_xor(bg, w));
    const int sg = (64 * b < L) ? (bg & 1023) : K - 1;
    int sa[CP + 1];
#pragma unroll
    for (int m = 0; m < CP; m++) sa[m] = __builtin_amdgcn_readlane(sg, m * G);
    sa[CP] = K - 1;
#pragma unroll
    for (int m = 0; m < CP; m++) {
        const int lo = sa[m] & ~(GIE_BAND_TRIP - 1), hi = sa[m + 1];
        const int u = 64 * m + lane;
        int c0 = 0x7fffffff, c1 = 0x7fffffff, c2 = 0x7fffffff, c3 = 0x7fffffff;
        for (int j = lo; j <= hi; j += GIE_BAND_TRIP) {
            const int4 p0 = *reinterpret_cast<const int4 *>(mb + j), p1 = *reinterpret_cast<const int4 *>(mb + j + 2);
#if GIE_BAND_TRIP >= 8
            const int4 p2 = *reinterpret_cast<const int4 *>(mb + j + 4), p3 = *reinterpret_cast<const int4 *>(mb + j + 6);
#endif
#if GIE_BAND_TRIP == 16
            const int4 p4 = *reinterpret_cast<const int4 *>(mb + j + 8), p5 = *reinterpret_cast<const int4 *>(mb + j + 10);
            const int4 p6 = *reinterpret_cast<const int4 *>(mb + j + 12), p7 = *reinterpret_cast<const int4 *>(mb + j + 14);
#endif
            c0 = min(c0, __mul24(u, p0.x) + p0.y);
            c1 = min(c1, __mul24(u, p0.z) + p0.w);
            c2 = min(c2, __mul24(u, p1.x) + p1.y);
            c3 = min(c3, __mul24(u, p1.z) + p1.w);
#if GIE_BAND_TRIP >= 8
            c0 = min(c0, __mul24(u, p2.x) + p2.y);
            c1 = min(c1, __mul24(u, p2.z) + p2.w);
            c2 = min(c2, __mul24(u, p3.x) + p3.y);
            c3 = min(c3, __mul24(u, p3.z) + p3.w);
#endif
#if GIE_BAND_TRIP == 16
            c0 = min(c0, __mul24(u, p4.x) + p4.y);
            c1 = min(c1, __mul24(u, p4.z) + p4.w);
            c2 = min(c2, __mul24(u, p5.x) + p5.y);
            c3 = min(c3, __mul24(u, p5.z) + p5.w);
            c0 = min(c0, __mul24(u, p6.x) + p6.y);
            c1 = min(c1, __mul24(u, p6.z) + p6.w);
            c2 = min(c2, __mul24(u, p7.x) + p7.y);
            c3 = min(c3, __mul24(u, p7.z) + p7.w);
#endif
        }
        sj[m] = min(min(c0, c1), min(c2, c3)) & 1023;
    }
}

#define GIE_WIN_MAX 48
#define GIE_WIN_NONE 0x7fffffffu
template <int CP>
__device__ __forceinline__ bool gie_row_window(const uint32_t *sk, const int L, const int lane, uint32_t (&best)[CP], const unsigned bandneed = ~0u)
{
#pragma unroll
    for (int m = 0; m < CP; m++) best[m] = (64 * m + lane < L) ? sk[64 * m + lane] : 0u;
    unsigned active = 0;
#pragma unroll
    for (int m = 0; m < CP; m++) if (64 * m < L && ((bandneed >> m) & 1u)) active |= 1u << m;
    int W = 0;
#pragma unroll 1
    for (;;) {
        const uint32_t w1 = (uint32_t)((W + 1) * (W + 1));
#pragma unroll
        for (int m = 0; m < CP; m++) {
            if (!((active >> m) & 1u)) continue;
            if (!__any(best[m] >= (w1 << 10))) active &= ~(1u << m);
        }
        if (!active) return true;
        if (W >= GIE_WIN_MAX) return false;
        const uint32_t *lo = sk + (lane - W - 4), *hi = sk + (lane + W + 1);
        const uint32_t a1 = w1 << 10, a2 = (uint32_t)((W + 2) * (W + 2)) << 10;
        const uint32_t a3 = (uint32_t)((W + 3) * (W + 3)) << 10, a4 = (uint32_t)((W + 4) * (W + 4)) << 10;
#pragma unroll
        for (int m = 0; m < CP; m++) {
            if (!((active >> m) & 1u)) continue;
            const uint32_t l4 = lo[64 * m], l3 = lo[64 * m + 1], l2 = lo[64 * m + 2], l1 = lo[64 * m + 3];
            const uint32_t h1 = hi[64 * m], h2 = hi[64 * m + 1], h3 = hi[64 * m + 2], h4 = hi[64 * m + 3];
            uint32_t b = best[m];
            b = min(b, min(l1, h1) + a1);
            b = min(b, min(l2, h2) + a2);
            b = min(b, min(l3, h3) + a3);
            b = min(b, min(l4, h4) + a4);
            best[m] = b;
        }
        W += 4;
    }
}

__device__ __forceinline__ int gie_row_compact_push(uint2 *ce, int base, const bool valid, const uint32_t a, const int i, const uint32_t hi16, const int lane, int2 *mb = nullptr)
{
    const unsigned long long m = __ballot(valid);
    if (valid) {
        const int j = base + __popcll(m & ((1ull << lane) - 1ull));
        ce[j] = make_uint2((a << 10) | (uint32_t)j, ((uint32_t)i << 5) | (hi16 << 16));
        if (mb && j < GIE_BAND_MAXK) mb[j] = make_int2(-(i << 11), (int)((((uint32_t)(i * i) + a) << 10) | (uint32_t)j));
    }
    return base + __popcll(m);
}

#ifndef GIE_EDTX_WAVES
#define GIE_EDTX_WAVES 4
#endif
GIE_HD int gie_zs_takes(const gie_ctx &c, const int zs, const int full)
{
    return zs && !(full == 0 && gie_z_use_lists(c, c.cnt[GIE_CNT_TL_KNOWN])) && *c.zcount > GIE_BAND_MAXK;
}
template <int CP>
__device__ __forceinline__ void gie_edt_x_row(const gie_ctx &c, const int y, const int z)
{
    constexpr int LP = 64 * CP;
    __shared__ __attribute__((aligned(16))) uint2 s_ce[GIE_EDTX_WAVES][LP];
    constexpr bool OVL = LP >= 2 * (GIE_BAND_MAXK + GIE_BAND_PAD) && LP / 2 >= GIE_BAND_MAXK;
    __shared__ __attribute__((aligned(16))) int2 s_mb[OVL ? 1 : GIE_EDTX_WAVES][OVL ? 1 : GIE_BAND_MAXK + GIE_BAND_PAD];
    const int wave = threadIdx.x >> 6, lane = threadIdx.x & 63;
    if (!c.zocc[z]) return;
    if (y >= c.Y) return;
    const int X = c.X;
    const size_t row = (size_t)z * c.Y + y;
    const uint16_t *in = c.cy1 + row * X;
    uint2 *ce = s_ce[wave];
    int2 *mb = OVL ? reinterpret_cast<int2 *>(ce + LP / 2) : s_mb[OVL ? 0 : wave];
    int K = 0;
    uint16_t cyv[CP];
#pragma unroll
    for (int m = 0; m < CP; m++) { const int i = 64 * m + lane; cyv[m] = __builtin_nontemporal_load(&in[min(i, X - 1)]); }
    uint32_t *out = c.cxy2 + row * X;
    if (CP >= 4) {
        int kall = 0;
#pragma unroll
        for (int m = 0; m < CP; m++) if (64 * m < X) kall += __popcll(__ballot(64 * m + lane < X && cyv[m] != 0xffff));
        if (kall > GIE_BAND_MAXK && kall * 8 >= X * 7) {
            static_assert(CP < 4 || (LP + 2 * GIE_WIN_MAX) * 4 + LP * 2 <= LP * 8, "the windowed row must fit the wave's site list");
            uint32_t *sk = reinterpret_cast<uint32_t *>(ce) + GIE_WIN_MAX;
            uint16_t *scy = reinterpret_cast<uint16_t *>(ce) + 2 * (LP + 2 * GIE_WIN_MAX);
#pragma unroll
            for (int m = 0; m < CP; m++) {
                const int i = 64 * m + lane;
                const uint16_t cy = (i < X) ? cyv[m] : (uint16_t)0xffff;
                const int d = y - (int)cy;
                sk[i] = (cy != 0xffff) ? (((uint32_t)(d * d) << 10) | (uint32_t)i) : GIE_WIN_NONE;
                scy[i] = cy;
            }
            if (lane < GIE_WIN_MAX) { sk[-1 - lane] = GIE_WIN_NONE; sk[LP + lane] = GIE_WIN_NONE; }
            gie_wave_sync();
            uint32_t best[CP];
            if (gie_row_window<CP>(sk, X, lane, best)) {
#pragma unroll
                for (int m = 0; m < CP; m++) {
                    const int sx = (int)(best[m] & 1023u);
                    if (64 * m + lane < X) __builtin_nontemporal_store((uint32_t)sx | ((uint32_t)scy[sx] << 16), &out[64 * m + lane]);
                }
                return;
            }
            gie_wave_sync();
        }
    }
#pragma unroll
    for (int m = 0; m < CP; m++) {
        const int i = 64 * m + lane;
        const uint16_t cy = (i < X) ? cyv[m] : (uint16_t)0xffff;
        const int d = y - (int)cy;
        if (64 * m < X) K = gie_row_compact_push(ce, K, cy != 0xffff, (uint32_t)(d * d), i, (uint32_t)cy, lane, mb);
    }
    const int u0 = lane * CP;
    uint32_t o[CP];
    if (K == 0) {
#pragma unroll
        for (int m = 0; m < CP; m++) o[m] = 0xffffffffu;
    } else if (K <= GIE_BAND_MAXK) {
        gie_row_mb_pad(mb, K, lane);
        gie_wave_sync();
        int sj[CP];
        gie_row_argmin_banded_lin<CP>(mb, K, X, lane, sj);
#pragma unroll
        for (int m = 0; m < CP; m++) {
            const uint32_t e = ce[sj[m]].y;
            if (64 * m + lane < X) out[64 * m + lane] = ((e & 0xffffu) >> 5) | (e & 0xffff0000u);
        }
        return;
    } else {
        gie_wave_sync();
        int sj[CP];
        gie_row_argmin<CP>(ce, K, X, lane, sj);
#pragma unroll
        for (int m = 0; m < CP; m++) {
            const uint32_t e = ce[sj[m]].y;
            o[m] = ((e & 0xffffu) >> 5) | (e & 0xffff0000u);
        }
    }
    if (CP >= 4 && (X & 3) == 0) {
#pragma unroll
        for (int m = 0; m < CP; m += 4)
            if (u0 + m < X) *reinterpret_cast<uint4 *>(out + u0 + m) = make_uint4(o[m], o[m + 1 < CP ? m + 1 : m], o[m + 2 < CP ? m + 2 : m], o[m + 3 < CP ? m + 3 : m]);
    } else {
#pragma unroll
        for (int m = 0; m < CP; m++) if (u0 + m < X) out[u0 + m] = o[m];
    }
}
template <int CP>
__global__ __launch_bounds__(64 * GIE_EDTX_WAVES) void k_edt_x(const gie_ctx c, const int zs, const int full)
{
    if (zs && gie_zs_takes(c, zs, full)) return;
    gie_edt_x_row<CP>(c, blockIdx.x * GIE_EDTX_WAVES + (int)(threadIdx.x >> 6), blockIdx.y);
}
template <int CP>
__global__ __launch_bounds__(64 * GIE_EDTX_WAVES) void k_edt_x_redo(const gie_ctx c)
{
    if (c.cnt[GIE_CNT_ZFAIL] == 0) return;
    const int K = *c.zcount, Y = c.Y, lane = threadIdx.x & 63;
    const int nw = (int)gridDim.x * GIE_EDTX_WAVES, w0 = (int)blockIdx.x * GIE_EDTX_WAVES + (int)(threadIdx.x >> 6);
    const int ntx = (c.X + 15) >> 4, nkc = (K + 7) >> 3;
#pragma unroll 1
    for (int u = w0; u < Y * nkc; u += nw) {
        const int uu = __builtin_amdgcn_readfirstlane(u);
        const int y = uu / nkc, k0 = (uu % nkc) * 8;
        bool f = false;
        for (int i = lane; i < ntx; i += 64) f |= c.zredo[(size_t)y * ntx + i] != 0u;
        if (!__any(f)) continue;
#pragma unroll 1
        for (int k = k0; k < min(k0 + 8, K); k++) {
            gie_wave_sync();
            gie_edt_x_row<CP>(c, y, c.zlist[k]);
        }
    }
}

template <int CP, int TX, int WAVES>
__global__ __launch_bounds__(64 * WAVES, (CP <= 8 ? 4 : 2)) void k_edt_z(const gie_ctx c, const int ntiles_x, const int ntiles, const int full)
{
    static_assert(TX == 16 && WAVES == 8, "a workgroup tile spans two 8-voxel tile columns, one column per wave and half");
    if (full == 0 && gie_z_use_lists(c, c.cnt[GIE_CNT_TL_KNOWN])) return;
    const int repair = c.cnt[GIE_CNT_ZSTREAM];
    if (repair && c.cnt[GIE_CNT_ZFAIL] == 0) return;
    constexpr int LP = 64 * CP;
    constexpr int TS = TX + 1;
    constexpr int NT = 64 * WAVES;
    constexpr int ZSTEP = NT / TX;
    constexpr int NLD = (LP + ZSTEP - 1) / ZSTEP;
    extern __shared__ __attribute__((aligned(16))) unsigned char smem[];
    const int Z = c.Z, X = c.X, Y = c.Y;
    uint32_t *tile = reinterpret_cast<uint32_t *>(smem);
    uint2 *s_ce = reinterpret_cast<uint2 *>(tile + (((size_t)Z * TS + 3) & ~(size_t)3));
    uint16_t *s_zl = reinterpret_cast<uint16_t *>(s_ce + WAVES * LP);
    const int wave = threadIdx.x >> 6, lane = threadIdx.x & 63;
    const int tx = threadIdx.x & (TX - 1), tz = threadIdx.x / TX;
    const size_t plane = (size_t)X * Y;
    uint2 *ce = s_ce + wave * LP;
    uint32_t pre[NLD];
    unsigned zmask = 0, zin = 0;
#pragma unroll
    for (int j = 0; j < NLD; j++) { const int z = tz + j * ZSTEP; if (z < Z) { zin |= 1u << j; if (c.zocc[z]) zmask |= 1u << j; } }
    const int K = *c.zcount;
    for (int j = threadIdx.x; j < K; j += NT) s_zl[j] = c.zlist[j];
    unsigned zvalid = 0;
#pragma unroll
    for (int m = 0; m < CP; m++) { const int z = 64 * m + lane; if (z < Z && c.zocc[z]) zvalid |= 1u << m; }
    __syncthreads();

    int it = 0;
    const bool xpair = (gridDim.x & 15u) == 0u;
    const int pq = ((int)blockIdx.x & 7) | (((int)blockIdx.x >> 4) << 3), ph = ((int)blockIdx.x >> 3) & 1, phalf = (int)gridDim.x >> 1;
#define GIE_ZTILE(i) (xpair ? (((i) * phalf + pq) * 2 + ph) : ((((i) >> 1) * (int)gridDim.x + (int)blockIdx.x) * 2 + ((i) & 1)))
    int t = GIE_ZTILE(0);
#define GIE_BUF_OOB 0xfffffff0u
    const unsigned nbytes = (unsigned)((size_t)X * Y * Z * 4u);
    const __amdgpu_buffer_rsrc_t rs_in = __builtin_amdgcn_make_buffer_rsrc(const_cast<uint32_t *>(c.cxy2), 0, nbytes, 0x00020000);
    const __amdgpu_buffer_rsrc_t rs_out = __builtin_amdgcn_make_buffer_rsrc(c.bcoc, 0, nbytes, 0x00020000);
    const unsigned zstride_b = (unsigned)(plane * ZSTEP * 4u);
    const unsigned tzoff_b = (unsigned)((size_t)tz * plane * 4u);
    uint64_t nd0, nd1, ndn0 = 0, ndn1 = 0;
#define GIE_LOAD_NEED(tt, o0, o1) do { \
        const int txc_ = (((tt) % ntiles_x) * TX) >> 3, tyc_ = ((tt) / ntiles_x) >> 3; \
        const uint64_t *p_ = c.zneed + ((size_t)tyc_ * c.tfd[0] + txc_); \
        o0 = ~0ull; o1 = ~0ull; \
        if (repair) { uint32_t r_; asm volatile("s_load_dword %0, %1, 0x0\n\ts_waitcnt lgkmcnt(0)" : "=s"(r_) : "s"(c.zredo + (tt)) : "memory"); if (!r_) { o0 = 0ull; o1 = 0ull; } } \
        if (!full && (o0 | o1) != 0ull) { \
            uint64_t a_, b_ = 0ull; \
            asm volatile("s_load_dwordx2 %0, %1, 0x0\n\ts_waitcnt lgkmcnt(0)" : "=s"(a_) : "s"(p_) : "memory"); \
            if (txc_ + 1 < c.tfd[0]) asm volatile("s_load_dwordx2 %0, %1, 0x8\n\ts_waitcnt lgkmcnt(0)" : "=s"(b_) : "s"(p_) : "memory"); \
            o0 = a_; o1 = b_; } } while (0)
    if (t < ntiles) {
        GIE_LOAD_NEED(t, ndn0, ndn1);
        const int x = (t % ntiles_x) * TX + tx, y = t / ntiles_x;
        const unsigned voff = tzoff_b + (unsigned)(y * X + x) * 4u;
        if ((ndn0 | ndn1) != 0ull) {
#pragma unroll
            for (int j = 0; j < NLD; j++) pre[j] = __builtin_amdgcn_raw_buffer_load_b32(rs_in, (((zmask >> j) & 1u) && x < X) ? voff : GIE_BUF_OOB, j * zstride_b, 0);
        }
    }
    for (; t < ntiles; t = GIE_ZTILE(it)) {
        it++;
        const int x0 = (t % ntiles_x) * TX, y = t / ntiles_x;
        nd0 = ndn0; nd1 = ndn1;
        const bool work = (nd0 | nd1) != 0ull;
        if (work) {
#pragma unroll
            for (int j = 0; j < NLD; j++) { if ((zmask >> j) & 1u) tile[(tz + j * ZSTEP) * TS + tx] = pre[j]; }
        }
        __syncthreads();
        const int tn = GIE_ZTILE(it);
        if (tn < ntiles) {
            GIE_LOAD_NEED(tn, ndn0, ndn1);
            if ((ndn0 | ndn1) != 0ull) {
                const int xn = (tn % ntiles_x) * TX + tx, yn = tn / ntiles_x;
                const unsigned voff = tzoff_b + (unsigned)(yn * X + xn) * 4u;
#pragma unroll
                for (int j = 0; j < NLD; j++) pre[j] = __builtin_amdgcn_raw_buffer_load_b32(rs_in, (((zmask >> j) & 1u) && xn < X) ? voff : GIE_BUF_OOB, j * zstride_b, 0);
            }
        }
        if (!work) continue;
#pragma unroll 1
        for (int half = 0; half < 2; half++) {
            const int col = wave + 8 * half;
            const int x = x0 + col;
            if (x >= X) break;
            const uint64_t nc = half ? nd1 : nd0;
            if (nc == 0ull) continue;
            if (CP >= 4 && K > GIE_BAND_MAXK) {
                unsigned bn = 0;
#pragma unroll
                for (int m = 0; m < CP && m < 8; m++) if ((nc >> (8 * m)) & 0xffull) bn |= 1u << m;
                if (full) bn = ~0u;
                uint32_t *sk = reinterpret_cast<uint32_t *>(ce) + GIE_WIN_MAX;
#pragma unroll
                for (int m = 0; m < CP; m++) {
                    const int i = 64 * m + lane;
                    uint32_t key = GIE_WIN_NONE;
                    if ((zvalid >> m) & 1u) {
                        const uint32_t v = tile[i * TS + col];
                        if (v != 0xffffffffu) { const int dx = x - (int)(v & 0xffffu), dy = y - (int)(v >> 16); key = ((uint32_t)(dx * dx + dy * dy) << 10) | (uint32_t)i; }
                    }
                    sk[i] = key;
                }
                if (lane < GIE_WIN_MAX) { sk[-1 - lane] = GIE_WIN_NONE; sk[LP + lane] = GIE_WIN_NONE; }
                gie_wave_sync();
                uint32_t best[CP];
                const bool okw = gie_row_window<CP>(sk, Z, lane, best, bn);
                if (okw) {
                    uint32_t oc[CP];
#pragma unroll
                    for (int m = 0; m < CP; m++) {
                        if (64 * m + lane < Z && ((bn >> m) & 1u)) {
                            const int s = (int)(best[m] & 1023u);
                            const uint32_t v = tile[s * TS + col];
                            oc[m] = gie_pack_bcoc((int)(v & 0xffffu), (int)(v >> 16), s);
                        }
                    }
                    gie_wave_sync();
#pragma unroll
                    for (int m = 0; m < CP; m++)
                        if (64 * m + lane < Z && ((bn >> m) & 1u)) tile[(64 * m + lane) * TS + col] = oc[m];
                    gie_wave_sync();
                    continue;
                }
                gie_wave_sync();
            }
            for (int j = lane; j < K; j += 64) {
                const int i = s_zl[j];
                const uint32_t v = tile[i * TS + col];
                const int dx = x - (int)(v & 0xffffu), dy = y - (int)(v >> 16);
                ce[j] = make_uint2(((uint32_t)(dx * dx + dy * dy) << 10) | (uint32_t)j, (uint32_t)i << 5);
            }
            gie_wave_sync();
            if (K == 0) {
                for (int i = lane; i < Z; i += 64) tile[i * TS + col] = GIE_BCOC_NONE;
            } else {
                unsigned bandneed = 0;
#pragma unroll
                for (int m = 0; m < CP && m < 8; m++) if ((nc >> (8 * m)) & 0xffull) bandneed |= 1u << m;
                if (full) bandneed = ~0u;
                int sj[CP];
                const bool banded = K <= GIE_BAND_MAXK;
                if (banded) gie_row_argmin_banded<CP>(ce, K, Z, lane, sj, bandneed);
                else gie_row_argmin<CP>(ce, K, Z, lane, sj);
                const int ub = banded ? lane : lane * CP, us = banded ? 64 : 1;
                uint32_t oc[CP];
#pragma unroll
                for (int m = 0; m < CP; m++) {
                    if (ub + m * us < Z && (!banded || ((bandneed >> m) & 1u))) {
                        const int s = (int)((ce[sj[m]].y & 0xffffu) >> 5);
                        const uint32_t v = tile[s * TS + col];
                        oc[m] = gie_pack_bcoc((int)(v & 0xffffu), (int)(v >> 16), s);
                    }
                }
                gie_wave_sync();
#pragma unroll
                for (int m = 0; m < CP; m++)
                    if (ub + m * us < Z && (!banded || ((bandneed >> m) & 1u))) tile[(ub + m * us) * TS + col] = oc[m];
            }
            gie_wave_sync();
        }
        __syncthreads();
        {
            const int x = x0 + tx;
            {
                const unsigned voff = tzoff_b + (unsigned)(y * X + x) * 4u;
                static_assert(ZSTEP % 8 == 0, "a thread's rows are whole z tiles apart");
                const uint64_t nds = ((tx >> 3) ? nd1 : nd0) >> (tz >> 3);
                unsigned wm = 0;
#pragma unroll
                for (int j = 0; j < NLD; j++) if (full || (j * (ZSTEP / 8) < 64 && ((nds >> (j * (ZSTEP / 8))) & 1ull))) wm |= 1u << j;
                {
                    unsigned zl = zin;
                    asm volatile("" : "+v"(zl));
                    wm &= zl;
                    if (x >= X) wm = 0;
                }
                {
#pragma unroll
                    for (int j0 = 0; j0 < NLD; j0 += 4) {
                        uint32_t ov[4];
#pragma unroll
                        for (int u = 0; u < 4; u++) ov[u] = (j0 + u < NLD) ? tile[(tz + (j0 + u) * ZSTEP) * TS + tx] : 0u;
#pragma unroll
                        for (int u = 0; u < 4; u++) if (j0 + u < NLD) __builtin_amdgcn_raw_buffer_store_b32(ov[u], rs_out, ((wm >> (j0 + u)) & 1u) ? voff : GIE_BUF_OOB, (j0 + u) * zstride_b, 0);
                    }
                }
            }
        }
        __syncthreads();
    }
}

#ifndef GIE_ZS_R
#define GIE_ZS_R 8
#endif
#ifndef GIE_ZS_C
#define GIE_ZS_C 16
#endif
#define GIE_ZS_W (GIE_ZS_C + 2 * GIE_ZS_R)
#define GIE_ZS_LDAUX 2
#define GIE_ZS_STAUX 2
#define GIE_ZS_NONE 0xb0000000u
#define GIE_ZS_LIMIT ((uint32_t)((GIE_ZS_R + 1) * (GIE_ZS_R + 1)) << 24)
__device__ __forceinline__ uint32_t gie_zs_key(const uint32_t v, const bool plane_ok, const int x8, const int y8, const int j)
{
    const uint32_t ux = (uint32_t)(x8 - (int)(v & 0xffffu)), uy = (uint32_t)(y8 - (int)(v >> 16));
    const int dx = (int)ux - 8, dy = (int)uy - 8;
    const uint32_t a = (uint32_t)(__mul24(dx, dx) + __mul24(dy, dy));
    const bool ok = plane_ok && max(ux, uy) <= 16u && a < (uint32_t)((GIE_ZS_R + 1) * (GIE_ZS_R + 1));
    return ok ? ((a << 24) | ((uint32_t)j << 18) | (ux << 13) | (uy << 8)) : (GIE_ZS_NONE | ((uint32_t)j << 18));
}
#define GIE_ZS_XW (64 + 2 * GIE_ZS_R)
#define GIE_ZS_ROWS 8
#ifndef GIE_ZS_CHAINS
#define GIE_ZS_CHAINS 4
#endif
#ifndef GIE_ZS_FUSED_WGS
#define GIE_ZS_FUSED_WGS 7
#endif
__device__ __forceinline__ uint32_t gie_zs_col(const uint32_t cy, const bool ok, const int y8)
{
    const uint32_t uy = (uint32_t)(y8 - (int)cy);
    const int dy = (int)uy - 8;
    return (ok && uy <= 16u) ? (((uint32_t)__mul24(dy, dy) << 24) | (uy << 8)) : GIE_ZS_NONE;
}
typedef __attribute__((address_space(3))) uint32_t gie_lds_u32;
__device__ __forceinline__ uint32_t gie_zs_fused_key(const gie_lds_u32 *row, const int j)
{
    uint32_t m = 0xffffffffu;
#pragma unroll
    for (int k = 0; k <= 2 * GIE_ZS_R; k++) m = min(m, row[k] + (((uint32_t)((k - GIE_ZS_R) * (k - GIE_ZS_R)) << 24) | ((uint32_t)(15 + k) << 13)));
    return m < GIE_ZS_LIMIT ? ((m ^ (31u << 13)) | ((uint32_t)j << 18)) : (GIE_ZS_NONE | ((uint32_t)j << 18));
}
template <int NP, int JB, int AUX>
__device__ __forceinline__ void gie_zs_fused_keys(uint32_t (&wk)[GIE_ZS_W], uint32_t (*srow)[GIE_ZS_XW], const __amdgpu_buffer_rsrc_t rs, const unsigned vo,
                                                  const unsigned ps2, const int zfirst, const int Z, const unsigned long long pm, const bool ok0, const bool ok1, const int y8, const int lane)
{
    static_assert(NP % GIE_ZS_ROWS == 0, "whole batches of rows");
    uint32_t v[NP];
#pragma unroll
    for (int j = 0; j < NP; j++) {
        const unsigned so = (unsigned)min(max(__builtin_amdgcn_readfirstlane(zfirst) + j, 0), Z - 1) * ps2;
        v[j] = __builtin_amdgcn_raw_buffer_load_b32(rs, vo, so, AUX);
    }
#pragma unroll
    for (int j0 = 0; j0 < NP; j0 += GIE_ZS_ROWS) {
#pragma unroll
        for (int j = j0; j < j0 + GIE_ZS_ROWS; j++) {
            const bool po = (pm >> j) & 1ull;
            if (lane < GIE_ZS_XW / 2)
                *reinterpret_cast<uint2 *>(&srow[j - j0][2 * lane]) = make_uint2(gie_zs_col(v[j] & 0xffffu, po && ok0, y8), gie_zs_col(v[j] >> 16, po && ok1, y8));
        }
        gie_wave_sync();
        gie_lds_u32 *rp[GIE_ZS_CHAINS];
#pragma unroll
        for (int q = 0; q < GIE_ZS_CHAINS; q++) rp[q] = (gie_lds_u32 *)&srow[0][lane];
#pragma unroll
        for (int j = j0; j < j0 + GIE_ZS_ROWS; j++) {
            wk[JB + j] = gie_zs_fused_key(rp[j % GIE_ZS_CHAINS] + (j - j0) * GIE_ZS_XW, JB + j);
            asm volatile("" : "+v"(rp[j % GIE_ZS_CHAINS]) : "v"(wk[JB + j]));
        }
        gie_wave_sync();
    }
}
__device__ __forceinline__ void gie_edt_z_direct_body(const gie_ctx &c);
#define GIE_ZS_R2 24
__device__ __noinline__ bool gie_zs_wide_trip(const uint32_t *cxy2, uint32_t *bcoc, const unsigned nbytes, const unsigned voff, const unsigned pstride,
                                              const int zc, const int z1, const int Z, const int x, const int y, const bool inx, const uint8_t *occ)
{
    const __amdgpu_buffer_rsrc_t rs_in = __builtin_amdgcn_make_buffer_rsrc(const_cast<uint32_t *>(cxy2), 0, nbytes, 0x00020000);
    const __amdgpu_buffer_rsrc_t rs_out = __builtin_amdgcn_make_buffer_rsrc(bcoc, 0, nbytes, 0x00020000);
    uint32_t best[GIE_ZS_C];
#pragma unroll
    for (int t = 0; t < GIE_ZS_C; t++) best[t] = 0xffffffffu;
    const int lo = max(zc - GIE_ZS_R2, 0), hi = min(zc + GIE_ZS_C + GIE_ZS_R2, Z);
#pragma unroll 1
    for (int i0 = lo; i0 < hi; i0 += 8) {
        uint32_t v[8];
#pragma unroll
        for (int k = 0; k < 8; k++) v[k] = __builtin_amdgcn_raw_buffer_load_b32(rs_in, voff, (unsigned)min(i0 + k, Z - 1) * pstride, 0);
#pragma unroll
        for (int k = 0; k < 8; k++) {
            const int i = i0 + k;
            if (i >= hi || !occ[i]) continue;
            const int dx = x - (int)(v[k] & 0xffffu), dy = y - (int)(v[k] >> 16);
            const uint32_t a = (v[k] == 0xffffffffu) ? 0x3fffffu : (uint32_t)(dx * dx + dy * dy);
#pragma unroll
            for (int t = 0; t < GIE_ZS_C; t++) { const int d = zc + t - i; best[t] = min(best[t], (min(a + (uint32_t)(d * d), 0x3fffffu) << 10) | (uint32_t)i); }
        }
    }
    uint32_t worst = 0;
#pragma unroll
    for (int t = 0; t < GIE_ZS_C; t++) if (zc + t < z1) worst = max(worst, best[t]);
    if (__any(inx && worst >= ((uint32_t)((GIE_ZS_R2 + 1) * (GIE_ZS_R2 + 1)) << 10))) return false;
#pragma unroll
    for (int t = 0; t < GIE_ZS_C; t++) {
        const int sp = (int)(best[t] & 1023u);
        const uint32_t v = __builtin_amdgcn_raw_buffer_load_b32(rs_in, voff, (unsigned)sp * pstride, 0);
        __builtin_amdgcn_raw_buffer_store_b32(gie_pack_bcoc((int)(v & 0xffffu), (int)(v >> 16), sp), rs_out, (zc + t < z1) ? voff : GIE_BUF_OOB, (unsigned)min(zc + t, Z - 1) * pstride, 0);
    }
    return true;
}
#define GIE_ZS_XW2 (64 + 2 * GIE_ZS_R2)
static_assert(2 * GIE_ZS_XW2 <= GIE_ZS_ROWS * GIE_ZS_XW, "the wide trip's row and its cy fit the wave's LDS rows");
__device__ __forceinline__ bool gie_zs_wide_trip_fused(const __amdgpu_buffer_rsrc_t rs_cy, const __amdgpu_buffer_rsrc_t rs_out, gie_lds_u32 *srow, const unsigned voff,
                                                       const unsigned pstride, const unsigned ps2, const int zc, const int z1, const int Z, const int x0, const int x,
                                                       const int y, const int X, const uint8_t *occ, const int lane)
{
    const int xa = x0 - GIE_ZS_R2 + lane, xb = x0 + 64 - GIE_ZS_R2 + lane;
    const bool oka = xa >= 0 && xa < X, okb = lane < 2 * GIE_ZS_R2 && xb < X;
    const unsigned voa = oka ? (unsigned)(y * X + xa) * 2u : GIE_BUF_OOB, vob = okb ? (unsigned)(y * X + xb) * 2u : GIE_BUF_OOB;
    gie_lds_u32 *sq = srow, *scy = srow + GIE_ZS_XW2;
    uint32_t best[GIE_ZS_C], bc[GIE_ZS_C];
#pragma unroll
    for (int t = 0; t < GIE_ZS_C; t++) { best[t] = 0xffffffffu; bc[t] = GIE_BCOC_NONE; }
    const int lo = max(zc - GIE_ZS_R2, 0), hi = min(zc + GIE_ZS_C + GIE_ZS_R2, Z);
#pragma unroll 1
    for (int i0 = lo; i0 < hi; i0 += 8) {
        uint16_t va[8], vb[8];
#pragma unroll
        for (int k = 0; k < 8; k++) {
            const unsigned so = (unsigned)min(i0 + k, Z - 1) * ps2;
            va[k] = __builtin_amdgcn_raw_buffer_load_b16(rs_cy, voa, so, 0);
            vb[k] = __builtin_amdgcn_raw_buffer_load_b16(rs_cy, vob, so, 0);
        }
#pragma unroll
        for (int k = 0; k < 8; k++) {
            const int i = i0 + k;
            if (i >= hi || !occ[i]) continue;
            {
                const int da = y - (int)va[k], db = y - (int)vb[k];
                sq[lane] = (oka && va[k] != 0xffffu) ? ((uint32_t)(da * da) << 6) : 0x3fffffc0u; scy[lane] = va[k];
                if (lane < 2 * GIE_ZS_R2) { sq[64 + lane] = (okb && vb[k] != 0xffffu) ? ((uint32_t)(db * db) << 6) : 0x3fffffc0u; scy[64 + lane] = vb[k]; }
            }
            gie_wave_sync();
            uint32_t m = 0xffffffffu;
#pragma unroll
            for (int q = 0; q <= 2 * GIE_ZS_R2; q++) m = min(m, sq[lane + q] + (((uint32_t)((q - GIE_ZS_R2) * (q - GIE_ZS_R2)) << 6) | (uint32_t)q));
            const int q = (int)(m & 63u);
            const uint32_t cc = gie_pack_bcoc(x - GIE_ZS_R2 + q, (int)scy[lane + q], i);
            gie_wave_sync();
            const uint32_t a = min(m >> 6, 0x3fffffu);
#pragma unroll
            for (int t = 0; t < GIE_ZS_C; t++) {
                const int d = zc + t - i;
                const uint32_t nb = (min(a + (uint32_t)(d * d), 0x3fffffu) << 10) | (uint32_t)i;
                if (nb < best[t]) { best[t] = nb; bc[t] = cc; }
            }
        }
    }
    uint32_t worst = 0;
#pragma unroll
    for (int t = 0; t < GIE_ZS_C; t++) if (zc + t < z1) worst = max(worst, best[t]);
    if (__any(x < X && worst >= ((uint32_t)((GIE_ZS_R2 + 1) * (GIE_ZS_R2 + 1)) << 10))) return false;
#pragma unroll
    for (int t = 0; t < GIE_ZS_C; t++)
        __builtin_amdgcn_raw_buffer_store_b32(bc[t], rs_out, (zc + t < z1) ? voff : GIE_BUF_OOB, (unsigned)min(zc + t, Z - 1) * pstride, 0);
    return true;
}
template <bool FUSED>
__global__ __launch_bounds__(256, FUSED ? GIE_ZS_FUSED_WGS : 6) void k_edt_z_stream(const gie_ctx c, const int full, const int nseg, const int seg_len, const int zs)
{
    __shared__ uint8_t s_occ[1024 + 2 * (32 + 2 * GIE_ZS_R)];
    const int Z = c.Z, X = c.X, Y = c.Y;
    if (full == 0 && gie_z_use_lists(c, c.cnt[GIE_CNT_TL_KNOWN])) { gie_edt_z_direct_body(c); return; }
    if (!gie_zs_takes(c, zs, full)) return;
    __shared__ __attribute__((aligned(16))) uint32_t s_row[FUSED ? 4 : 1][FUSED ? GIE_ZS_ROWS : 1][GIE_ZS_XW];
    if (blockIdx.x == 0 && threadIdx.x == 0) c.cnt[GIE_CNT_ZSTREAM] = 1;
    for (int i = threadIdx.x; i < Z + 2 * GIE_ZS_W; i += 256) { const int z = i - GIE_ZS_W; s_occ[i] = (z >= 0 && z < Z) ? c.zocc[z] : (uint8_t)0; }
    __syncthreads();
    const int lane = threadIdx.x & 63;
    const int nxr = (X + 63) >> 6;
    const int total = nxr * nseg * Y;
    const size_t plane = (size_t)X * Y;
    const unsigned nbytes = (unsigned)((size_t)X * Y * Z * 4u);
    const __amdgpu_buffer_rsrc_t rs_in = __builtin_amdgcn_make_buffer_rsrc(const_cast<uint32_t *>(c.cxy2), 0, nbytes, 0x00020000);
    const __amdgpu_buffer_rsrc_t rs_cy = __builtin_amdgcn_make_buffer_rsrc(const_cast<uint16_t *>(c.cy1), 0, nbytes / 2u, 0x00020000);
    const __amdgpu_buffer_rsrc_t rs_out = __builtin_amdgcn_make_buffer_rsrc(c.bcoc, 0, nbytes, 0x00020000);
    const unsigned pstride = (unsigned)(plane * 4u), pstride2 = (unsigned)(plane * 2u);
    for (int w = (int)blockIdx.x * 4 + (int)(threadIdx.x >> 6); w < total; w += (int)gridDim.x * 4) {
        const int wu = __builtin_amdgcn_readfirstlane(w);
        const int xr = wu % nxr, seg = (wu / nxr) % nseg, y = wu / (nxr * nseg);
        const int x = xr * 64 + lane;
        const int z0 = seg * seg_len, z1 = min(Z, z0 + seg_len);
        if (z0 >= Z) continue;
        const unsigned voff = x < X ? (unsigned)(y * X + x) * 4u : GIE_BUF_OOB;
        const int x8 = x + 8, y8 = y + 8;
        uint32_t wk[GIE_ZS_W];
        const int xa = xr * 64 - GIE_ZS_R + 2 * lane;
        const bool oka = lane < GIE_ZS_XW / 2 && xa >= 0 && xa < X, okb = lane < GIE_ZS_XW / 2 && xa + 1 >= 0 && xa + 1 < X;
        const unsigned vpa = (oka || okb) ? (unsigned)(y * X + xa) * 2u : GIE_BUF_OOB;
        uint32_t (*srow)[GIE_ZS_XW] = s_row[FUSED ? (threadIdx.x >> 6) : 0];
        if (FUSED) {
            const int zz = z0 - GIE_ZS_R + lane;
            const unsigned long long pm = __ballot(lane < 2 * GIE_ZS_R && s_occ[zz + GIE_ZS_W] != 0);
            gie_zs_fused_keys<2 * GIE_ZS_R, 0, 0>(wk, srow, rs_cy, vpa, pstride2, z0 - GIE_ZS_R, Z, pm, oka, okb, y8, lane);
        } else {
            const int zz = z0 - GIE_ZS_R + lane;
            const unsigned long long pm = __ballot(lane < 2 * GIE_ZS_R && s_occ[zz + GIE_ZS_W] != 0);
            uint32_t v[2 * GIE_ZS_R];
#pragma unroll
            for (int j = 0; j < 2 * GIE_ZS_R; j++) { const int zp = min(max(z0 - GIE_ZS_R + j, 0), Z - 1); v[j] = __builtin_amdgcn_raw_buffer_load_b32(rs_in, voff, (unsigned)zp * pstride, 0); }
#pragma unroll
            for (int j = 0; j < 2 * GIE_ZS_R; j++) wk[j] = gie_zs_key(v[j], (pm >> j) & 1ull, x8, y8, j);
        }
        bool failed = false;
        int wide = 0, wz0 = 0, wz1 = 0;
#pragma unroll 1
        for (int zc = z0; zc < z1; zc += GIE_ZS_C) {
            if (FUSED) {
                const int zz = zc + GIE_ZS_R + lane;
                const unsigned long long pm = __ballot(lane < GIE_ZS_C && s_occ[zz + GIE_ZS_W] != 0);
                gie_zs_fused_keys<GIE_ZS_C, 2 * GIE_ZS_R, GIE_ZS_LDAUX>(wk, srow, rs_cy, vpa, pstride2, zc + GIE_ZS_R, Z, pm, oka, okb, y8, lane);
            } else {
                const int zz = zc + GIE_ZS_R + lane;
                const unsigned long long pm = __ballot(lane < GIE_ZS_C && s_occ[zz + GIE_ZS_W] != 0);
                uint32_t v[GIE_ZS_C];
#pragma unroll
                for (int j = 0; j < GIE_ZS_C; j++) { const int zp = min(zc + GIE_ZS_R + j, Z - 1); v[j] = __builtin_amdgcn_raw_buffer_load_b32(rs_in, voff, (unsigned)zp * pstride, GIE_ZS_LDAUX); }
#pragma unroll
                for (int j = 0; j < GIE_ZS_C; j++) wk[2 * GIE_ZS_R + j] = gie_zs_key(v[j], (pm >> j) & 1ull, x8, y8, 2 * GIE_ZS_R + j);
            }
            uint32_t wlo = 0, whi = 0;
#pragma unroll
            for (int t = 0; t < GIE_ZS_C; t++) {
                const int p = GIE_ZS_R + t;
                uint32_t b = wk[p];
#pragma unroll
                for (int d = 1; d <= GIE_ZS_R; d++) b = min(b, min(wk[p - d], wk[p + d]) + ((uint32_t)(d * d) << 24));
                const bool in = zc + t < z1;
                if (in) { if (t < 8) wlo = max(wlo, b); else whi = max(whi, b); }
                const int s = zc - GIE_ZS_R + (int)((b >> 18) & 63u);
                const int cx = x8 - (int)((b >> 13) & 31u), cy = y8 - (int)((b >> 8) & 31u);
                __builtin_amdgcn_raw_buffer_store_b32(gie_pack_bcoc(cx, cy, s), rs_out, in ? voff : GIE_BUF_OOB, (unsigned)min(zc + t, Z - 1) * pstride, GIE_ZS_STAUX);
            }
            const uint32_t worst = max(wlo, whi);
            {
                static_assert(GIE_ZS_C == 16, "a trip is two tiles high");
                uint32_t m0 = x < X ? (wlo >> 24) : 0u, m1 = x < X ? (whi >> 24) : 0u;
                m0 = max(m0, (uint32_t)__shfl_xor((int)m0, 1)); m1 = max(m1, (uint32_t)__shfl_xor((int)m1, 1));
                m0 = max(m0, (uint32_t)__shfl_xor((int)m0, 2)); m1 = max(m1, (uint32_t)__shfl_xor((int)m1, 2));
                m0 = max(m0, (uint32_t)__shfl_xor((int)m0, 4)); m1 = max(m1, (uint32_t)__shfl_xor((int)m1, 4));
                if ((lane & 7) == 0 && x < X) {
                    const int t0 = gie_tile_index(c, x, y, zc);
                    __hip_atomic_fetch_max(&c.tbmax[t0], (int32_t)m0, __ATOMIC_RELAXED, __HIP_MEMORY_SCOPE_AGENT);
                    if (zc + 8 < z1) __hip_atomic_fetch_max(&c.tbmax[t0 + c.tfd[0] * c.tfd[1]], (int32_t)m1, __ATOMIC_RELAXED, __HIP_MEMORY_SCOPE_AGENT);
                }
            }
            if (__any(x < X && worst >= GIE_ZS_LIMIT)) {
                if (wide == 2) { failed = true; break; }
                if (wide == 0) wz0 = zc; else wz1 = zc;
                wide++;
            }
#pragma unroll
            for (int j = 0; j < 2 * GIE_ZS_R; j++) wk[j] = wk[GIE_ZS_C + j] - ((uint32_t)GIE_ZS_C << 18);
        }
        if (wide > 0 && lane == 0) atomicAdd(&c.cnt[GIE_CNT_ZWIDE], wide);
        if (FUSED) {
#pragma unroll 1
            for (int k = 0; k < wide && !failed; k++)
                failed = !gie_zs_wide_trip_fused(rs_cy, rs_out, (gie_lds_u32 *)&srow[0][0], voff, pstride, pstride2, __builtin_amdgcn_readfirstlane(k ? wz1 : wz0), z1, Z, xr * 64, x, y, X,
                                                 s_occ + GIE_ZS_W, lane);
        } else {
            if (!failed && wide > 0) failed = !gie_zs_wide_trip(c.cxy2, c.bcoc, nbytes, voff, pstride, wz0, z1, Z, x, y, x < X, s_occ + GIE_ZS_W);
            if (!failed && wide > 1) failed = !gie_zs_wide_trip(c.cxy2, c.bcoc, nbytes, voff, pstride, wz1, z1, Z, x, y, x < X, s_occ + GIE_ZS_W);
        }
        if (failed) {
            if (lane < 4) {
                const int tx16 = xr * 4 + lane;
                if (tx16 * 16 < X) c.zredo[(size_t)y * ((X + 15) >> 4) + tx16] = 1u;
                if (lane == 0) atomicAdd(&c.cnt[GIE_CNT_ZFAIL], 1);
            }
            if ((lane & 7) == 0 && x < X)
                for (int zt = z0; zt < z1; zt += 8) __hip_atomic_fetch_max(&c.tbmax[gie_tile_index(c, x, y, zt)], (int32_t)((GIE_ZS_R + 1) * (GIE_ZS_R + 1)), __ATOMIC_RELAXED, __HIP_MEMORY_SCOPE_AGENT);
        }
    }
}

#define GIE_PREP_WAVES 16
__global__ __launch_bounds__(64 * GIE_PREP_WAVES) void k_edt_prep(const gie_ctx c, const int ncol)
{
    if (blockIdx.x == 0 && threadIdx.x < 64) {
        uint8_t f[16];
#pragma unroll
        for (int i = 0; i < 16; i++) { const int z = 64 * i + (int)threadIdx.x; f[i] = c.zocc[min(z, c.Z - 1)]; }
        int k = 0;
#pragma unroll
        for (int i = 0; i < 16; i++) {
            const int z = 64 * i + (int)threadIdx.x;
            const bool v = z < c.Z && f[i];
            const unsigned long long m = __ballot(v);
            if (v) c.zlist[k + __popcll(m & ((1ull << threadIdx.x) - 1ull))] = (uint16_t)z;
            k += __popcll(m);
        }
        if (threadIdx.x == 0) *c.zcount = k;
    }
    const int col = blockIdx.x * GIE_PREP_WAVES + (threadIdx.x >> 6);
    const bool colok = col < ncol;
    const int tx = colok ? col % c.tfd[0] : 0, ty = colok ? col / c.tfd[0] : 0;
    for (int tz0 = 0; tz0 < c.tfd[2]; tz0 += 64) {
        const int tz = tz0 + (int)(threadIdx.x & 63);
        const int t = (tz * c.tfd[1] + ty) * c.tfd[0] + tx;
        const bool k = colok && tz < c.tfd[2] && c.tknown[t];
        const unsigned long long m = __ballot(k);
        if (colok && tz == 0) c.zneed[col] = m;
        const int slot = gie_wg_reserve(&c.cnt[GIE_CNT_TL_KNOWN], k);
        if (slot >= 0) c.tl_known[slot] = t;
        const int slot2 = gie_wg_reserve(&c.cnt[GIE_CNT_TL_SWEPT], k && c.tskip[t] != 2);
        if (slot2 >= 0) c.tl_swept[slot2] = t;
    }
}

__global__ __launch_bounds__(256) void k_tile_oldskip(const gie_ctx c, const int ntile, int32_t *list, int32_t *count)
{
    int any = 0;
    for (int z = threadIdx.x; z < c.Z; z += 256) any |= c.zocc[z];
    any = __syncthreads_or(any);
    const int t = blockIdx.x * 256 + threadIdx.x;
    bool need = false;
    if (t < ntile) need = gie_tile_oldskip(c, t, any) != 0;
    const int slot = gie_wg_reserve(count, need);
    if (slot >= 0) list[slot] = t;
}
__global__ __launch_bounds__(256) void k_coc_catchup_new(const gie_ctx c, const int pu0, const int pu1, const int pu2, const int32_t *list, const int32_t *count)
{
    const int n = *count;
    const int lane = threadIdx.x & 63;
    const int pupvt[3] = { pu0, pu1, pu2 };
    for (int e = (int)blockIdx.x * 4 + (int)(threadIdx.x >> 6); e < n; e += (int)gridDim.x * 4) gie_coc_catchup_newcolumn(c, pupvt, list[e], lane);
}

__global__ __launch_bounds__(256) void k_pair_lazy_list(const gie_ctx c, const int ntile, const int stay, int32_t *list, int32_t *count)
{
    const int t = blockIdx.x * 256 + threadIdx.x;
    const bool need = t < ntile && c.tlazy[t] != 0 && !(stay && c.tskip[t] == 2);
    const int slot = gie_wg_reserve(count, need);
    if (slot >= 0) list[slot] = t;
}
__global__ __launch_bounds__(256) void k_pair_lazy_run(const gie_ctx c, const int32_t *list, const int32_t *count)
{
    const int n = *count;
    const int lane = threadIdx.x & 63;
    for (int e = (int)blockIdx.x * 4 + (int)(threadIdx.x >> 6); e < n; e += (int)gridDim.x * 4) {
        const int t = list[e];
        gie_pair_materialise_column(c, t, lane);
        if (lane == 0) c.tlazy[t] = 0;
    }
}

__global__ __launch_bounds__(256) void k_coc_catchup_list(const gie_ctx c, const gie_catchup p, const int ntile, int32_t *list, int32_t *count)
{
    const int t = blockIdx.x * 256 + threadIdx.x;
    const bool need = t < ntile && gie_coc_catchup_tile(c, p, t);
    const int slot = gie_wg_reserve(count, need);
    if (slot >= 0) list[slot] = t;
}
__global__ __launch_bounds__(256) void k_coc_catchup_run(const gie_ctx c, const gie_catchup p, const int32_t *list, const int32_t *count)
{
    const int n = *count;
    const int lane = threadIdx.x & 63;
    for (int e = (int)blockIdx.x * 4 + (int)(threadIdx.x >> 6); e < n; e += (int)gridDim.x * 4) gie_coc_catchup_column(c, p, list[e], lane);
}

template <class F, bool STAGED>
__device__ __forceinline__ void gie_vox_column(const gie_ctx &c, const F &f, const int x, const int y, const int z0)
{
    if (x >= c.X || y >= c.Y || f.tile_skip(c, x, y, z0)) return;
    bool sk[8];
    int id[8];
#pragma unroll
    for (int k = 0; k < 8; k++) {
        const int z = z0 + k;
        id[k] = (z < c.Z) ? gie_lid(c, x, y, z) : 0;
        sk[k] = z >= c.Z || f.skip(c, id[k], x, y, z);
    }
    if (STAGED) {
        typename F::st s[8];
#pragma unroll
        for (int k = 0; k < 8; k++) if (!sk[k]) f.load1(c, id[k], x, y, z0 + k, s[k]);
#pragma unroll
        for (int k = 0; k < 8; k++) if (!sk[k]) f.load2(c, id[k], x, y, z0 + k, s[k]);
        unsigned known = 0, valid = 0;
        int vmax = 0;
#pragma unroll
        for (int k = 0; k < 8; k++) {
            if (z0 + k < c.Z) valid |= 1u << k;
            if (!sk[k]) { const int r = f.finish(c, id[k], x, y, z0 + k, s[k]); known |= (unsigned)(r != 0) << k; vmax = r > vmax ? r : vmax; }
        }
        gie_column_hook_impl(f, c, x, y, z0, known, valid, 0);
        gie_column_max_hook_impl(f, c, x, y, z0, known, valid, vmax, 0);
    } else {
#pragma unroll
        for (int k = 0; k < 8; k++) if (!sk[k]) f(c, x, y, z0 + k);
    }
}
template <class F, bool STAGED, int LX>
__global__ __launch_bounds__(256) void k_voxa(const gie_ctx c, const F f, const int32_t *list, const int count_idx, const int always_list)
{
    if (GIE_GATE_CLOSED(c)) return;
    const int n = c.cnt[count_idx];
    const int lane = threadIdx.x & 63;
    if (always_list == 2 && !gie_use_lists(c, n)) return;
    if (always_list || gie_use_lists(c, n)) {
        const int waves = gridDim.x * 4;
        for (int e = blockIdx.x * 4 + (threadIdx.x >> 6); e < n; e += waves) {
            const int t = list[e];
            const int tx = t % c.tfd[0], ty = (t / c.tfd[0]) % c.tfd[1], tz = t / (c.tfd[0] * c.tfd[1]);
            gie_vox_column<F, STAGED>(c, f, tx * 8 + (lane & 7), ty * 8 + (lane >> 3), tz * 8);
        }
    } else {
        constexpr int LY = 64 / LX, WY = 4 * LY;
        const int gx = (c.X + LX - 1) / LX, gy = (c.Y + WY - 1) / WY, gz = (c.Z + 7) / 8;
        const int nv = gx * gy * gz;
        const int per = (nv + (int)gridDim.x - 1) / (int)gridDim.x;
        const int lx = lane % LX, ly = (int)(threadIdx.x >> 6) * LY + lane / LX;
        int v = (int)blockIdx.x * per;
        const int vend = min(nv, ((int)blockIdx.x + 1) * per);
        int vx = v % gx, vy = (v / gx) % gy, vz = v / (gx * gy);
        for (; v < vend; v++) {
            gie_vox_column<F, STAGED>(c, f, vx * LX + lx, vy * WY + ly, vz * 8);
            if (++vx == gx) { vx = 0; if (++vy == gy) { vy = 0; vz++; } }
        }
    }
}

__device__ __forceinline__ void gie_markc_lazy_tile(const gie_ctx &c, const int t)
{
    if (!c.tknown[t] || c.tskip[t] != 2) return;
    const int tx = t % c.tfd[0], ty = (t / c.tfd[0]) % c.tfd[1], tz = t / (c.tfd[0] * c.tfd[1]);
    const int x = tx * 8, y = ty * 8, z0 = tz * 8;
    const size_t plane = (size_t)c.X * c.Y;
    const size_t id0 = ((size_t)z0 * c.Y + y) * c.X + x;
    const int wb = c.cnt[GIE_CNT_ZSTREAM] ? c.tbmax[t] : 0x7fffffff;
    int vmax = wb <= 80 ? wb + 1 : 0;
    if (wb > 80) {
        uint32_t sb[8];
#pragma unroll
        for (int k = 0; k < 8; k++) sb[k] = c.bcoc[id0 + (size_t)(1 + 4 * (k >> 2)) * plane + (size_t)(1 + 4 * ((k >> 1) & 1)) * c.X + (size_t)(1 + 4 * (k & 1))];
        vmax = 0;
#pragma unroll
        for (int k = 0; k < 8; k++) {
            const int sx = x + 1 + 4 * (k & 1), sy = y + 1 + 4 * ((k >> 1) & 1), sz = z0 + 1 + 4 * (k >> 2);
            int v = GIE_TMAX_INF;
            if (sb[k] != GIE_BCOC_NONE) {
                const int dx = sx - (int)(sb[k] & 1023u), dy = sy - (int)((sb[k] >> 10) & 1023u), dz = sz - (int)(sb[k] >> 20);
                const int r = (int)ceilf(sqrtf((float)(dx * dx + dy * dy + dz * dz))) + 4;
                v = r * r + 1;
            }
            vmax = v > vmax ? v : vmax;
        }
    }
    c.tmax[t] = vmax;
    c.tlazy[t] = 1;
    uint8_t *const u0 = c.ucol + gie_ucol_index(c, x, y, z0);
    if ((c.X & 7) == 0) {
        uint64_t ub[8];
#pragma unroll
        for (int r = 0; r < 8; r++) ub[r] = *reinterpret_cast<const uint64_t *>(u0 + (size_t)r * c.X);
#pragma unroll
        for (int r = 0; r < 8; r++) if (ub[r]) *reinterpret_cast<uint64_t *>(u0 + (size_t)r * c.X) = 0ull;
    } else {
        for (int r = 0; r < 8; r++) for (int q = 0; q < 8; q++) if (u0[(size_t)r * c.X + q]) u0[(size_t)r * c.X + q] = 0;
    }
}
struct gie_markc_pre { uint32_t flags; int32_t slot_lo, slot_hi; };
__device__ __forceinline__ gie_markc_pre gie_markc_flags(const gie_ctx &c, const int x, const int y, const int z0)
{
    gie_markc_pre p = { 0u, -1, -1 };
    if (x >= c.X || y >= c.Y || z0 >= c.Z) return p;
    const int t = gie_tile_index(c, x, y, z0);
    const int nz = min(8, c.Z - z0);
    const int gx = x + c.pvt[0], gy = y + c.pvt[1], gz0 = z0 + c.pvt[2];
    const uint32_t kn = c.tknown[t], sk = c.tskip[t], ub = c.ucol[gie_ucol_index(c, x, y, z0)];
    p.slot_lo = c.blk_tab[gie_tab_index(c, gx, gy, gz0)];
    p.slot_hi = c.blk_tab[gie_tab_index(c, gx, gy, gz0 + nz - 1)];
    p.flags = (kn ? 1u : 0u) | (sk << 8) | (ub << 16);
    return p;
}
__device__ __forceinline__ void gie_markc_column_fast(const gie_ctx &c, const int x, const int y, const int z0, const gie_markc_pre pre)
{
    const uint32_t flags = pre.flags;
    if (!(flags & 1u)) return;
    const int t = gie_tile_index(c, x, y, z0);
    const size_t plane = (size_t)c.X * c.Y;
    const size_t id0 = ((size_t)z0 * c.Y + y) * c.X + x;
    const int nz = min(8, c.Z - z0);
    const int gx = x + c.pvt[0], gy = y + c.pvt[1], gz0 = z0 + c.pvt[2];
    const int skipold = (int)((flags >> 8) & 255u);
    const bool nostore = c.coc_defer && skipold == 2;
    const size_t ui = gie_ucol_index(c, x, y, z0);
    const unsigned ub = flags >> 16;
    if (nostore && c.lazy_ok) return;
    int8_t ty[8]; uint32_t bc[8]; gie_vaddr a[8]; uint64_t oc[8];
    const int slot_lo = pre.slot_lo, slot_hi = pre.slot_hi;
#pragma unroll
    for (int k = 0; k < 8; k++) {
        const size_t id = id0 + (size_t)(k < nz ? k : 0) * plane;
        ty[k] = c.glb_type[id]; bc[k] = __builtin_nontemporal_load(&c.bcoc[id]);
        const int gz = gz0 + k;
        const int slot = ((gz >> 3) == (gz0 >> 3)) ? slot_lo : slot_hi;
        a[k] = slot < 0 ? (gie_vaddr)-1 : (gie_vaddr)slot * GIE_VBSZ + gie_vox_in_blk(gx, gy, gz);
        oc[k] = 0;
        if (!skipold && k < nz && a[k] >= 0) oc[k] = c.g_coc[a[k]];
    }
    if (nostore && c.wr_inside) {
        unsigned want = 0;
        bool plain = true;
#pragma unroll
        for (int k = 0; k < 8; k++) if (k < nz && ty[k] != GIE_VOX_UNKNOWN) { want |= 1u << k; if (bc[k] == GIE_BCOC_NONE) plain = false; }
        if (plain) {
            const uint32_t ox = (uint32_t)(c.pvt[0] - c.upvt[0]), oy = (uint32_t)(c.pvt[1] - c.upvt[1]), oz = (uint32_t)(c.pvt[2] - c.upvt[2]);
            int vmax = 0;
            uint64_t *const pp = c.pair + id0;
#pragma unroll
            for (int k = 0; k < 8; k++) {
                if (!((want >> k) & 1u)) continue;
                const uint32_t b = bc[k];
                const uint32_t cx = b & 1023u, cy = (b >> 10) & 1023u, cz = b >> 20;
                const int dx = x - (int)cx, dy = y - (int)cy, dz = z0 + k - (int)cz;
                const uint32_t d = (uint32_t)(__mul24(dx, dx) + __mul24(dy, dy) + __mul24(dz, dz));
                const uint32_t wz = cz + oz;
                const uint32_t lo = (cx + ox) | ((cy + oy) << 14) | (wz << 28), hi = (wz >> 4) | (d << (GIE_PAIR_DIST_SHIFT - 32));
                __builtin_nontemporal_store(((uint64_t)hi << 32) | lo, &pp[(size_t)k * plane]);
                vmax = (int)d + 1 > vmax ? (int)d + 1 : vmax;
            }
            if (ub & want) c.ucol[ui] = (uint8_t)(ub & ~want);
            gie_markc_column(c, x, y, z0, want, (1u << nz) - 1u, vmax);
            return;
        }
    }
    int dold[8];
    unsigned want = 0;
#pragma unroll
    for (int k = 0; k < 8; k++) {
        if (k < nz && ty[k] != GIE_VOX_UNKNOWN) want |= 1u << k;
        dold[k] = GIE_TMAX_INF;
    }
    if (!skipold) {
#pragma unroll
        for (int k = 0; k < 8; k++) if (((want >> k) & 1u) && a[k] >= 0) dold[k] = gie_gdist(c, oc[k], gx, gy, gz0 + k);
    }
    unsigned known = 0, valid = 0;
    int vmax = 0, flag = 0;
#pragma unroll
    for (int k = 0; k < 8; k++) {
        if (k < nz) valid |= 1u << k;
        if (!((want >> k) & 1u)) continue;
        const size_t id = id0 + (size_t)k * plane;
        int r;
        if (a[k] < 0) { gie_commit_pair<false>(c, (int)id, -1, c.pair[id]); r = GIE_TMAX_INF; }
        else {
            int ft;
            const uint64_t pr = gie_mark_logic(c, x, y, z0 + k, bc[k], dold[k], oc[k], &c.pair[id], &ft);
            flag |= ft;
            gie_edt_before_keep(c, (int)id, pr, (ub >> k) & 1u);
            c.pair[id] = pr;
            if (!nostore) gie_commit_pair<false>(c, (int)id, a[k], pr);
            const int d = gie_pair_dist(pr);
            r = d == c.empty_value ? GIE_TMAX_INF : d + 1;
        }
        known |= 1u << k; vmax = r > vmax ? r : vmax;
    }
    if (flag) c.tflag[t] = 1;
    if (ub & known) c.ucol[ui] = (uint8_t)(ub & ~known);
    gie_markc_column(c, x, y, z0, known, valid, vmax);
// ... 1638 lines not shown
```

gie-mapping_amd/csrc/gie_types.h:

```cpp
#ifndef GIE_TYPES_H
#define GIE_TYPES_H

#include <stdint.h>
#include "../../include/gie.h"
#include "../../include/gie_math.h"

#define GIE_VB 8
#define GIE_VBSZ 512
typedef long long gie_vaddr;

#define GIE_PAIR_DIST_SHIFT 42
#define GIE_PAIR_NEW (1ull << 41)
#define GIE_PAIR_PAR_MASK ((1ull << 41) - 1ull)
#define GIE_PAR_NONE GIE_PAIR_PAR_MASK
#define GIE_NOPROP 0xffffffffffffffffull

GIE_HD uint64_t gie_pair_make(int dist, uint64_t par) { return ((uint64_t)(uint32_t)dist << GIE_PAIR_DIST_SHIFT) | (par & GIE_PAIR_PAR_MASK); }
GIE_HD int gie_pair_dist(uint64_t p) { return (int)(p >> GIE_PAIR_DIST_SHIFT); }
GIE_HD uint64_t gie_pair_par(uint64_t p) { return p & GIE_PAIR_PAR_MASK; }
GIE_HD uint64_t gie_pack_wr(int x, int y, int z) { return (uint64_t)(uint32_t)x | ((uint64_t)(uint32_t)y << 14) | ((uint64_t)(uint32_t)z << 28); }
GIE_HD void gie_unpack_wr(uint64_t id, int *x, int *y, int *z)
{
    *x = (int)(id & 0x3fff); *y = (int)((id >> 14) & 0x3fff); *z = (int)((id >> 28) & 0x1fff);
    if ((id & GIE_PAIR_PAR_MASK) == GIE_PAR_NONE) *z = 0x3fff;
}

#define GIE_CRD_OFF (1 << 20)
GIE_HD uint64_t gie_pack_crd(int x, int y, int z)
{ return (uint64_t)(uint32_t)(x + GIE_CRD_OFF) | ((uint64_t)(uint32_t)(y + GIE_CRD_OFF) << 21) | ((uint64_t)(uint32_t)(z + GIE_CRD_OFF) << 42); }
GIE_HD void gie_unpack_crd(uint64_t k, int *x, int *y, int *z)
{ *x = (int)(k & 0x1fffff) - GIE_CRD_OFF; *y = (int)((k >> 21) & 0x1fffff) - GIE_CRD_OFF; *z = (int)((k >> 42) & 0x1fffff) - GIE_CRD_OFF; }
#define GIE_KEY_EMPTY 0xffffffffffffffffull
#define GIE_KEY_TOMB 0xfffffffffffffffeull

#define GIE_BCOC_NONE 0xffffffffu
GIE_HD uint32_t gie_pack_bcoc(int x, int y, int z) { return (uint32_t)x | ((uint32_t)y << 10) | ((uint32_t)z << 20); }
GIE_HD int gie_bcoc_dist(uint32_t bc, int x, int y, int z, int none_value)
{
    if (bc == GIE_BCOC_NONE) return none_value;
    const int dx = x - (int)(bc & 1023u), dy = y - (int)((bc >> 10) & 1023u), dz = z - (int)(bc >> 20);
    return dx * dx + dy * dy + dz * dz;
}

typedef struct gie_ctx {
    int X, Y, Z, N;
    float voxel_width;
    int occ_thresh;
    float min_h, max_h;
    int cutoff_sq;
    int fast_mode, for_motion_planner, robot_r2;
    int bar_fault;
    int max_width, max_loc_dist_sq;
    int wr[3];
    int empty_value;
    int invalid_dist_min;
    int map_ct;
    int pvt[3], upvt[3];
    int tile_off[3];
    int whole_lo[3], whole_hi[3];
    float origin[3];
    gie_se3 L2G, G2L;
    int pntcld_mode;
    uint32_t stamp_base;
    int32_t *ray_count;
    int8_t *inst_type;
    int8_t *glb_type;
    float *edt;
    uint16_t *cy1;
    uint32_t *cxy2;
    uint32_t *bcoc;
    uint64_t *pair;
    uint32_t *wl;
    uint8_t *tflag;
    int tfd[3];
    uint8_t *tknown, *tunk;
    uint8_t *tknown_prev;
    uint8_t *tray;
    uint8_t *tact;
    uint8_t *tsum;
    int32_t *tbmax;
    int32_t *tmax, *tmax_prev;
    uint8_t *ucol;
    int oldskip;
    uint8_t *tskip;
    uint8_t *tskip_prev;
    int ts_pvt[3];
    const int8_t *scan_labels;
    int wr_inside;
    int skip2_ok;
    int catchup_fast;
    int coc_defer;
    uint8_t *tlazy;
    const uint32_t *bcoc_lazy;
    int lazy_ok;
    int qdefer;
    int pp_pvt[3], pp_upvt[3];
    int prev_valid;
    int prev_shift[3];
    uint8_t *zocc;
    uint64_t *zneed;
    uint32_t *zredo;
    uint16_t *zlist;
    int32_t *zcount;
    int32_t *tl_known;
    int32_t *tl_swept;
    int32_t *tl_front;
    int force_lists;
    uint64_t *lprop;
    uint64_t *cand[2];
    int tb0[3];
    int tdim[3];
    int32_t *blk_tab;
    const int32_t *tab_prev;
    int tab_prev_d[3];
    uint8_t *blk_need;
    int32_t *blk_new;
    uint64_t *hkeys;
    int32_t *hvals;
    uint32_t hmask;
    int max_blocks;
    int32_t *pool_count;
    int32_t *free_list;
    int retain;
    int vb_lo[3], vb_hi[3];
    uint64_t *g_key;
    int32_t *g_nbr;
    uint8_t *g_occ;
    int8_t *g_type;
    uint64_t *g_coc;
    uint64_t *g_pair;
    uint64_t *g_prop;
    uint64_t *g_prop2;
    int32_t *wb_list[2];
    int32_t *wb_flag[2];
    int32_t *lvlb_next, *lvlb_vis;
    int32_t *lvla_next, *lvla_vis;
    int32_t *g_wl;
    int track;
    int fused;
    int32_t *g_dirty;
    int nbox;
    const float *box_ll, *box_ur;
    const uint8_t *box_act;
    uint64_t *qa, *qb;
    gie_vaddr *qa_a, *qb_a;
    int32_t *qc[2];
    int qcap_ab, qcap_c;
    int32_t *cnt;
    int32_t *lvl_next, *lvl_vis;
    int32_t *wc_list[2];
    int32_t *wc_flag[2];
    const int32_t *gate;
} gie_ctx;
#define GIE_GATE_CLOSED(c) ((c).gate != nullptr && *(const volatile int32_t *)(c).gate == 0)

enum {
    GIE_CNT_A = 0, GIE_CNT_B, GIE_CNT_C,
    GIE_CNT_TL_SWEPT,
    GIE_CNT_ZWIDE,
    GIE_CNT_FREE5,
    GIE_CNT_LV0, GIE_CNT_LV1, GIE_CNT_LV2,
    GIE_CNT_ERR,
    GIE_CNT_NEWBLK,
    GIE_CNT_VIS_A, GIE_CNT_VIS_B, GIE_CNT_VIS_C,
    GIE_CNT_LVL_A, GIE_CNT_LVL_B, GIE_CNT_LVL_C,
    GIE_CNT_FRONT_B, GIE_CNT_FRONT_C,
    GIE_CNT_SEED_A, GIE_CNT_SEED_B, GIE_CNT_SEED_C,
    GIE_CNT_ZSTREAM,
    GIE_CNT_ZFAIL,
    GIE_CNT_STATE1, GIE_CNT_STATE2,
    GIE_CNT_FRAME_END = 28,
    GIE_CNT_TOT_A = 28, GIE_CNT_TOT_B = 30, GIE_CNT_TOT_C = 32,
    GIE_CNT_BAR_B = 34,
    GIE_CNT_BAR_C = 35,
    GIE_CNT_NEWLIST = 36,
    GIE_CNT_TL_KNOWN = 37, GIE_CNT_TL_FRONT = 38,
    GIE_CNT_BAR_AB2 = 39,
    GIE_CNT_TL_FUSE = 40,
    GIE_CNT_BARFAIL = 42,
    GIE_CNT_TSKIP = 41,
    GIE_CNT_INL = 43,
    GIE_CNT_AUX_END = 44,
    GIE_CNT_LAZY_EXACT = 44,
    GIE_CNT_NUM = 48
};
#define GIE_MAX_LEVELS 4096
#define GIE_ERRF_POOL 1
#define GIE_ERRF_QUEUE 2
#define GIE_ERRF_HASH 4
#define GIE_ERRF_BARRIER 8

#define GIE_CLEAR_MAX 16
typedef struct gie_clear_list { void *p[GIE_CLEAR_MAX]; uint32_t bytes[GIE_CLEAR_MAX]; int n; } gie_clear_list;
#define GIE_CLEAR_WG_BYTES 16384u
GIE_HD int gie_clear_wgs(uint32_t bytes) { const uint32_t n = (bytes + GIE_CLEAR_WG_BYTES - 1u) / GIE_CLEAR_WG_BYTES; return n < 1u ? 1 : (n > 256u ? 256 : (int)n); }
GIE_HD int gie_clear_total_wgs(const gie_clear_list &l) { int t = 0; for (int i = 0; i < l.n; i++) t += gie_clear_wgs(l.bytes[i]); return t; }

#define GIE_WL_SEED(c) ((c).stamp_base + 1u)
#define GIE_WL_PUSHED(c) ((c).stamp_base + 2u)
#define GIE_WL_LEVEL(c, lvl) ((c).stamp_base + 8u + (uint32_t)(lvl))

GIE_HD int gie_in_loc(const gie_ctx &c, int x, int y, int z) { return x >= 0 && x < c.X && y >= 0 && y < c.Y && z >= 0 && z < c.Z; }
GIE_HD int gie_in_whole(const gie_ctx &c, int x, int y, int z)
{ return x >= c.whole_lo[0] && x < c.whole_hi[0] && y >= c.whole_lo[1] && y < c.whole_hi[1] && z >= c.whole_lo[2] && z < c.whole_hi[2]; }
GIE_HD int gie_in_wr(const gie_ctx &c, int x, int y, int z) { return x >= 0 && x < c.wr[0] && y >= 0 && y < c.wr[1] && z >= 0 && z < c.wr[2]; }
GIE_HD int gie_lid(const gie_ctx &c, int x, int y, int z) { return (z * c.Y + y) * c.X + x; }
GIE_HD int gie_use_lists(const gie_ctx &c, int listed)
{
    if (c.force_lists >= 0) return c.force_lists;
    return (long long)listed * 8 <= (long long)c.tfd[0] * c.tfd[1] * c.tfd[2];
}
#ifndef GIE_Z_SHORT_LISTS
#define GIE_Z_SHORT_LISTS 1
#endif
#ifndef GIE_Z_LIST_DIV
#define GIE_Z_LIST_DIV 8
#endif
GIE_HD int gie_z_use_lists(const gie_ctx &c, int listed)
{
    if (c.force_lists >= 0) return c.force_lists;
    if (GIE_Z_SHORT_LISTS && c.tfd[2] <= 8) return 1;
    return (long long)listed * GIE_Z_LIST_DIV <= (long long)c.tfd[0] * c.tfd[1] * c.tfd[2];
}
GIE_HD int gie_tile_index(const gie_ctx &c, int x, int y, int z) { return ((z >> 3) * c.tfd[1] + (y >> 3)) * c.tfd[0] + (x >> 3); }
GIE_HD int gie_vox_in_blk(int gx, int gy, int gz) { return ((gz & 7) << 6) | ((gy & 7) << 3) | (gx & 7); }
GIE_HD int gie_d2(int ax, int ay, int az, int bx, int by, int bz)
{
    const long long dx = ax - bx, dy = ay - by, dz = az - bz;
    const long long r = dx * dx + dy * dy + dz * dz;
    return r > 0x7fffffffLL ? 0x7fffffff : (int)r;
}
GIE_HD int gie_invalid_dist(const gie_ctx &c, int d) { return d < 0 || d >= c.invalid_dist_min; }
GIE_HD int gie_invalid_coc(int x, int y, int z) { return x > 900000 || y > 900000 || z > 900000; }

GIE_HD int gie_tab_index(const gie_ctx &c, int gx, int gy, int gz)
{
    const int bx = (gx >> 3) - c.tb0[0], by = (gy >> 3) - c.tb0[1], bz = (gz >> 3) - c.tb0[2];
    return (bz * c.tdim[1] + by) * c.tdim[0] + bx;
}

GIE_HD uint32_t gie_hash_key(int bx, int by, int bz)
{
    uint64_t h = gie_pack_crd(bx, by, bz);
    h ^= h >> 33; h *= 0xff51afd7ed558ccdull; h ^= h >> 33; h *= 0xc4ceb9fe1a85ec53ull; h ^= h >> 33;
    return (uint32_t)h;
}

GIE_HD int gie_hash_find(const gie_ctx &c, int bx, int by, int bz)
{
    const uint64_t key = gie_pack_crd(bx, by, bz);
    uint32_t h = gie_hash_key(bx, by, bz) & c.hmask;
    for (uint32_t probes = 0; probes <= c.hmask; probes++) {
        const uint64_t k = c.hkeys[h];
        const int v = c.hvals[h];
        if (k == key) return v;
        if (k == GIE_KEY_EMPTY) return -1;
        h = (h + 1) & c.hmask;
    }
    return -1;
}

GIE_HD int gie_bdr_index(const gie_ctx &c, int x, int y, int z)
{
    const int YZ = c.Y * c.Z, XZ = c.X * c.Z, XY = c.X * c.Y;
    if (x == 0) return y + c.Y * z;
    if (x == c.X - 1) return YZ + y + c.Y * z;
    if (y == 0) return 2 * YZ + x + c.X * z;
    if (y == c.Y - 1) return 2 * YZ + XZ + x + c.X * z;
    if (z == 0) return 2 * YZ + 2 * XZ + x + c.X * y;
    return 2 * YZ + 2 * XZ + XY + x + c.X * y;
}

#if defined(GIE_TEST_HOOKS)
#include <stdlib.h>
static inline int gie_switch_env(const char *name, int dflt) { const char *e = getenv(name); return e ? atoi(e) : dflt; }
#define GIE_SWITCH(name, dflt) gie_switch_env(name, dflt)
#else
#define GIE_SWITCH(name, dflt) (dflt)
#endif

#endif
```

Before: 98900 Mvoxels/s.

## Feed fused z-stream EDT from packed y-occupancy bitmasks instead of cy1

Adds a packed per-16-row y-occupancy bitmask buffer (yb32), written by the y4 EDT pass with 8-row halos from neighbouring blocks. When z-stream takes over, the y pass can skip the full cy1 computation. The fused z-stream kernel and its x-redo path then derive the nearest-y distance from these bits with ctz/clz instead of loading 16-bit cy1 values. This cuts y-pass work and the bytes read in the z stream, at the cost of an extra buffer, more ALU bit work per column, and fallback walks across blocks in the redo path.

```diff
diff --git a/gie-mapping_amd/csrc/gie_api.inc.h b/gie-mapping_amd/csrc/gie_api.inc.h
--- a/gie-mapping_amd/csrc/gie_api.inc.h
+++ b/gie-mapping_amd/csrc/gie_api.inc.h
@@ -184,6 +184,7 @@
     c.glb_type = gie_dalloc<int8_t>(m, N);
     c.edt = gie_dalloc<float>(m, N);
     c.cy1 = gie_dalloc<uint16_t>(m, N);
+    c.yb32 = gie_dalloc<uint32_t>(m, (size_t)Z * ((Y + 15) / 16) * X);
     c.cxy2 = gie_dalloc<uint32_t>(m, N);
     c.bcoc = gie_dalloc<uint32_t>(m, N);
     m->pp.bcoc_alt = gie_dalloc<uint32_t>(m, N);
diff --git a/gie-mapping_amd/csrc/gie_hip.hip b/gie-mapping_amd/csrc/gie_hip.hip
--- a/gie-mapping_amd/csrc/gie_hip.hip
+++ b/gie-mapping_amd/csrc/gie_hip.hip
@@ -323,7 +323,8 @@
 template <int CP> static void gie_launch_edt_xz(be_state *b, const gie_ctx &c, bool zpass, int full, int zs_fused = 0, bool redo = false)
 {
     if (redo) {
-        GIE_LAUNCH(b, k_edt_x_redo<CP>, dim3(b->cu_total * 8), dim3(64 * GIE_EDTX_WAVES), 0, c);
+        if (zs_fused == 3) GIE_LAUNCH(b, (k_edt_x_redo<CP, true>), dim3(b->cu_total * 8), dim3(64 * GIE_EDTX_WAVES), 0, c);
+        else GIE_LAUNCH(b, (k_edt_x_redo<CP, false>), dim3(b->cu_total * 8), dim3(64 * GIE_EDTX_WAVES), 0, c);
     } else if (!zpass) {
         GIE_LAUNCH(b, k_edt_x<CP>, dim3((c.Y + GIE_EDTX_WAVES - 1) / GIE_EDTX_WAVES, c.Z), dim3(64 * GIE_EDTX_WAVES), 0, c, zs_fused, full);
     } else {
@@ -338,17 +339,25 @@
     else if (L <= 512) gie_launch_edt_xz<8>(b, c, zpass, full, zs_fused, redo);
     else gie_launch_edt_xz<16>(b, c, zpass, full, zs_fused, redo);
 }
+static int be_edty4_mode(const gie_ctx &c)
+{
+    static const int y4 = GIE_SWITCH("GIE_EDTY4", 1);
+    return (c.X & 3) == 0 ? y4 : 0;
+}
 static int be_zs_mode(const gie_ctx &c)
 {
     if (c.Z < 64 || c.Z > 1024) return 0;
     static const int on = GIE_SWITCH("GIE_ZSTREAM", 1);
     static const int fused = GIE_SWITCH("GIE_ZS_FUSED", 1);
-    return on ? ((fused && (c.X & 1) == 0) ? 2 : 1) : 0;
+    static const int ybits = GIE_SWITCH("GIE_ZS_YBITS", 1);
+    if (!on) return 0;
+    if (!fused || (c.X & 1)) return 1;
+    return (ybits && be_edty4_mode(c) && c.Y <= 512) ? 3 : 2;
 }
 static int be_edt_z_stream(be_state *b, const gie_ctx &c, int full);
 static void be_edt_z_rest(be_state *b, const gie_ctx &c, int full, int zs)
 {
-    if (zs == 2) gie_launch_edt_dim(b, c, c.X, false, full, 0, true);
+    if (zs >= 2) gie_launch_edt_dim(b, c, c.X, false, full, zs, true);
     gie_launch_edt_dim(b, c, c.Z, true, full);
 }
 static void be_edt_z(be_state *b, const gie_ctx &c, int full) { be_edt_z_rest(b, c, full, be_edt_z_stream(b, c, full) ? be_zs_mode(c) : 0); }
@@ -444,8 +453,9 @@
     const long long cap = (long long)b->cu_total * 8 * 4;
     if (grid > cap) grid = cap;
     if (!full && grid < (long long)b->cu_total * 16) grid = (long long)b->cu_total * 16;
-    if (zs == 2) GIE_LAUNCH(b, k_edt_z_stream<true>, dim3((unsigned)grid), dim3(256), 0, c, full, nseg, seg_len, zs);
-    else GIE_LAUNCH(b, k_edt_z_stream<false>, dim3((unsigned)grid), dim3(256), 0, c, full, nseg, seg_len, zs);
+    if (zs == 3) GIE_LAUNCH(b, k_edt_z_stream<3>, dim3((unsigned)grid), dim3(256), 0, c, full, nseg, seg_len, zs);
+    else if (zs == 2) GIE_LAUNCH(b, k_edt_z_stream<2>, dim3((unsigned)grid), dim3(256), 0, c, full, nseg, seg_len, zs);
+    else GIE_LAUNCH(b, k_edt_z_stream<1>, dim3((unsigned)grid), dim3(256), 0, c, full, nseg, seg_len, zs);
     return 1;
 }
 static void be_tile_oldskip(be_state *b, const gie_ctx &c, const int pupvt[3])
@@ -479,22 +489,21 @@
 {
     dim3 gy((c.X + GIE_EDTY_COLS - 1) / GIE_EDTY_COLS, c.Z);
     be_prof(b, 6, 0);
-    static const int y4 = GIE_SWITCH("GIE_EDTY4", 1);
-    if (y4 && (c.X & 3) == 0) {
+    const int y4 = be_edty4_mode(c), zs = be_zs_mode(c);
+    if (y4) {
         const int yb = c.Y > 512 ? 32 : 16, nq = (c.Y + yb - 1) / yb;
         const int lanes = (y4 == 3) ? 32 : 16;
         dim3 g4((c.X / 4 + lanes - 1) / lanes, c.Z), b4(lanes, nq);
-        if (yb == 16 && lanes == 16) GIE_LAUNCH(b, (k_edt_y4<16, 16>), g4, b4, 0, c);
-        else if (yb == 16) GIE_LAUNCH(b, (k_edt_y4<16, 32>), g4, b4, 0, c);
-        else if (lanes == 16) GIE_LAUNCH(b, (k_edt_y4<32, 16>), g4, b4, 0, c);
-        else GIE_LAUNCH(b, (k_edt_y4<32, 32>), g4, b4, 0, c);
+        if (yb == 16 && lanes == 16) GIE_LAUNCH(b, (k_edt_y4<16, 16>), g4, b4, 0, c, zs, full);
+        else if (yb == 16) GIE_LAUNCH(b, (k_edt_y4<16, 32>), g4, b4, 0, c, zs, full);
+        else if (lanes == 16) GIE_LAUNCH(b, (k_edt_y4<32, 16>), g4, b4, 0, c, zs, full);
+        else GIE_LAUNCH(b, (k_edt_y4<32, 32>), g4, b4, 0, c, zs, full);
     }
     else if (c.Y <= 256) GIE_LAUNCH(b, (k_edt_y<8, 8>), gy, dim3(GIE_EDTY_COLS, 8), 0, c);
     else if (c.Y <= 512) GIE_LAUNCH(b, (k_edt_y<16, 16>), gy, dim3(GIE_EDTY_COLS, 16), 0, c);
     else GIE_LAUNCH(b, (k_edt_y<32, 16>), gy, dim3(GIE_EDTY_COLS, 16), 0, c);
     be_prof(b, 6, 1);
-    const int zs = be_zs_mode(c);
-    be_prof(b, 7, 0); gie_launch_edt_dim(b, c, c.X, false, full, zs == 2 ? zs : 0); be_prof(b, 7, 1);
+    be_prof(b, 7, 0); gie_launch_edt_dim(b, c, c.X, false, full, zs >= 2 ? zs : 0); be_prof(b, 7, 1);
     be_prof(b, 8, 0);
     const int zl = be_edt_z_stream(b, c, full);
     if (!zl && !full) be_edt_z_direct(b, c);
diff --git a/gie-mapping_amd/csrc/gie_kernels.hip.h b/gie-mapping_amd/csrc/gie_kernels.hip.h
--- a/gie-mapping_amd/csrc/gie_kernels.hip.h
+++ b/gie-mapping_amd/csrc/gie_kernels.hip.h
@@ -359,6 +359,7 @@
     }
 }
 
+GIE_HD int gie_zs_takes(const gie_ctx &c, const int zs, const int full);
 #ifndef GIE_EDTY_COLS
 #define GIE_EDTY_COLS 64
 #endif
@@ -421,7 +422,7 @@
 }
 
 template <int YB, int LANES>
-__global__ __launch_bounds__(32 * LANES) void k_edt_y4(const gie_ctx c)
+__global__ __launch_bounds__(32 * LANES) void k_edt_y4(const gie_ctx c, const int zs, const int full)
 {
     __shared__ __attribute__((aligned(16))) uint32_t s_m[32][LANES * 4];
     const int l = threadIdx.x, q = threadIdx.y, nq = blockDim.y;
@@ -452,6 +453,15 @@
     *reinterpret_cast<uint4 *>(&s_m[q][4 * l]) = make_uint4(m[0], m[1], m[2], m[3]);
     __syncthreads();
     if (!in) return;
+    if (YB == 16 && zs == 3 && gie_zs_takes(c, zs, 1)) {
+        const uint4 zero = make_uint4(0u, 0u, 0u, 0u);
+        const uint4 lo = q > 0 ? *reinterpret_cast<const uint4 *>(&s_m[q - 1][4 * l]) : zero;
+        const uint4 hi = q + 1 < nq ? *reinterpret_cast<const uint4 *>(&s_m[q + 1][4 * l]) : zero;
+        const size_t o = ((size_t)z * nq + q) * X + x;
+        *reinterpret_cast<uint4 *>(c.yb32 + o) = make_uint4((lo.x >> 8) | (m[0] << 8) | (hi.x << 24), (lo.y >> 8) | (m[1] << 8) | (hi.y << 24),
+                                                            (lo.z >> 8) | (m[2] << 8) | (hi.z << 24), (lo.w >> 8) | (m[3] << 8) | (hi.w << 24));
+        if (gie_zs_takes(c, zs, full)) return;
+    }
     int pl[4] = {-1, -1, -1, -1}, nf[4] = {-1, -1, -1, -1};
     for (int w = 0; w < q; w++) {
         const uint4 o = *reinterpret_cast<const uint4 *>(&s_m[w][4 * l]);
@@ -731,7 +741,32 @@
 {
     return zs && !(full == 0 && gie_z_use_lists(c, c.cnt[GIE_CNT_TL_KNOWN])) && *c.zcount > GIE_BAND_MAXK;
 }
-template <int CP>
+
+__device__ __forceinline__ uint32_t gie_yb_frame_half(const uint32_t w, const bool hi, const int b, const int nb)
+{
+    return hi ? (b + 1 < nb ? w : w >> 16) : (b > 0 ? w : w << 16);
+}
+__device__ __forceinline__ uint64_t gie_yb_frame(const uint32_t *w, const int b, const int nb, const int X)
+{
+    const uint32_t lo = w[(size_t)(b > 0 ? b - 1 : b) * X], hi = w[(size_t)(b + 1 < nb ? b + 1 : b) * X];
+    return (uint64_t)gie_yb_frame_half(lo, false, b, nb) | ((uint64_t)gie_yb_frame_half(hi, true, b, nb) << 32);
+}
+__device__ __forceinline__ uint16_t gie_cy_of_bits(const gie_ctx &c, const int x, const int y, const int z)
+{
+    const int X = c.X, nb = (c.Y + 15) >> 4, b = y >> 4, p = (y & 15) + 24;
+    const uint32_t *w = c.yb32 + (size_t)z * nb * X + x;
+    const uint64_t f = gie_yb_frame(w, b, nb, X);
+    const uint64_t hi = f >> p, lo = f << (63 - p);
+    int ua = hi ? __builtin_ctzll(hi) : -1, ub = lo ? __builtin_clzll(lo) : -1;
+    const bool walk_a = ua < 0 && !(ub >= 0 && ub <= 24), walk_b = ub < 0 && !(ua >= 0 && ua <= 24);
+    if (walk_a)
+        for (int bb = b + 2; bb < nb; bb++) { const uint32_t m = (w[(size_t)bb * X] >> 8) & 0xffffu; if (m) { ua = 16 * bb + __ffs(m) - 1 - y; break; } }
+    if (walk_b)
+        for (int bb = b - 2; bb >= 0; bb--) { const uint32_t m = (w[(size_t)bb * X] >> 8) & 0xffffu; if (m) { ub = y - (16 * bb + 31 - __clz(m)); break; } }
+    if (ua >= 0 && (ub < 0 || ua <= ub)) return (uint16_t)(y + ua);
+    return ub >= 0 ? (uint16_t)(y - ub) : (uint16_t)0xffff;
+}
+template <int CP, bool BITS = false>
 __device__ __forceinline__ void gie_edt_x_row(const gie_ctx &c, const int y, const int z)
 {
     constexpr int LP = 64 * CP;
@@ -749,7 +784,7 @@
     int K = 0;
     uint16_t cyv[CP];
 #pragma unroll
-    for (int m = 0; m < CP; m++) { const int i = 64 * m + lane; cyv[m] = __builtin_nontemporal_load(&in[min(i, X - 1)]); }
+    for (int m = 0; m < CP; m++) { const int i = 64 * m + lane; cyv[m] = BITS ? gie_cy_of_bits(c, min(i, X - 1), y, z) : __builtin_nontemporal_load(&in[min(i, X - 1)]); }
     uint32_t *out = c.cxy2 + row * X;
     if (CP >= 4) {
         int kall = 0;
@@ -829,7 +864,7 @@
     if (zs && gie_zs_takes(c, zs, full)) return;
     gie_edt_x_row<CP>(c, blockIdx.x * GIE_EDTX_WAVES + (int)(threadIdx.x >> 6), blockIdx.y);
 }
-template <int CP>
+template <int CP, bool BITS>
 __global__ __launch_bounds__(64 * GIE_EDTX_WAVES) void k_edt_x_redo(const gie_ctx c)
 {
     if (c.cnt[GIE_CNT_ZFAIL] == 0) return;
@@ -846,7 +881,7 @@
 #pragma unroll 1
         for (int k = k0; k < min(k0 + 8, K); k++) {
             gie_wave_sync();
-            gie_edt_x_row<CP>(c, y, c.zlist[k]);
+            gie_edt_x_row<CP, BITS>(c, y, c.zlist[k]);
         }
     }
 }
@@ -1075,12 +1110,23 @@
 #ifndef GIE_ZS_FUSED_WGS
 #define GIE_ZS_FUSED_WGS 7
 #endif
+#ifndef GIE_ZS_BITS_WGS
+#define GIE_ZS_BITS_WGS 6
+#endif
 __device__ __forceinline__ uint32_t gie_zs_col(const uint32_t cy, const bool ok, const int y8)
 {
     const uint32_t uy = (uint32_t)(y8 - (int)cy);
     const int dy = (int)uy - 8;
     return (ok && uy <= 16u) ? (((uint32_t)__mul24(dy, dy) << 24) | (uy << 8)) : GIE_ZS_NONE;
 }
+typedef unsigned int gie_u32x2 __attribute__((ext_vector_type(2)));
+__device__ __forceinline__ uint32_t gie_zs_col_bits(const uint32_t w, const bool ok, const int p)
+{
+    const uint32_t ua = (uint32_t)__ffs((int)(w >> p)) - 1u;
+    const uint32_t ub = (uint32_t)__clz((int)(w << (31 - p)));
+    const uint32_t d = min(ua, ub), uy = ua <= ub ? 8u - ua : 8u + ub;
+    return (ok && d <= 8u) ? ((d * d << 24) | (uy << 8)) : GIE_ZS_NONE;
+}
 typedef __attribute__((address_space(3))) uint32_t gie_lds_u32;
 __device__ __forceinline__ uint32_t gie_zs_fused_key(const gie_lds_u32 *row, const int j)
 {
@@ -1089,24 +1135,30 @@
     for (int k = 0; k <= 2 * GIE_ZS_R; k++) m = min(m, row[k] + (((uint32_t)((k - GIE_ZS_R) * (k - GIE_ZS_R)) << 24) | ((uint32_t)(15 + k) << 13)));
     return m < GIE_ZS_LIMIT ? ((m ^ (31u << 13)) | ((uint32_t)j << 18)) : (GIE_ZS_NONE | ((uint32_t)j << 18));
 }
-template <int NP, int JB, int AUX>
+template <int NP, int JB, int AUX, bool BITS>
 __device__ __forceinline__ void gie_zs_fused_keys(uint32_t (&wk)[GIE_ZS_W], uint32_t (*srow)[GIE_ZS_XW], const __amdgpu_buffer_rsrc_t rs, const unsigned vo,
-                                                  const unsigned ps2, const int zfirst, const int Z, const unsigned long long pm, const bool ok0, const bool ok1, const int y8, const int lane)
+                                                  const unsigned ps2, const int zfirst, const int Z, const unsigned long long pm, const bool ok0, const bool ok1, const int yv, const int lane)
 {
     static_assert(NP % GIE_ZS_ROWS == 0, "whole batches of rows");
-    uint32_t v[NP];
+    typedef typename std::conditional<BITS, gie_u32x2, uint32_t>::type ld_t;
+    ld_t v[NP];
 #pragma unroll
     for (int j = 0; j < NP; j++) {
         const unsigned so = (unsigned)min(max(__builtin_amdgcn_readfirstlane(zfirst) + j, 0), Z - 1) * ps2;
-        v[j] = __builtin_amdgcn_raw_buffer_load_b32(rs, vo, so, AUX);
+        if constexpr (BITS) v[j] = __builtin_amdgcn_raw_buffer_load_b64(rs, vo, so, AUX);
+        else v[j] = __builtin_amdgcn_raw_buffer_load_b32(rs, vo, so, AUX);
     }
 #pragma unroll
     for (int j0 = 0; j0 < NP; j0 += GIE_ZS_ROWS) {
 #pragma unroll
         for (int j = j0; j < j0 + GIE_ZS_ROWS; j++) {
             const bool po = (pm >> j) & 1ull;
-            if (lane < GIE_ZS_XW / 2)
-                *reinterpret_cast<uint2 *>(&srow[j - j0][2 * lane]) = make_uint2(gie_zs_col(v[j] & 0xffffu, po && ok0, y8), gie_zs_col(v[j] >> 16, po && ok1, y8));
+            if (lane < GIE_ZS_XW / 2) {
+                if constexpr (BITS)
+                    *reinterpret_cast<uint2 *>(&srow[j - j0][2 * lane]) = make_uint2(gie_zs_col_bits(v[j][0], po && ok0, yv), gie_zs_col_bits(v[j][1], po && ok1, yv));
+                else
+                    *reinterpret_cast<uint2 *>(&srow[j - j0][2 * lane]) = make_uint2(gie_zs_col(v[j] & 0xffffu, po && ok0, yv), gie_zs_col(v[j] >> 16, po && ok1, yv));
+            }
         }
         gie_wave_sync();
         gie_lds_u32 *rp[GIE_ZS_CHAINS];
@@ -1160,32 +1212,58 @@
 }
 #define GIE_ZS_XW2 (64 + 2 * GIE_ZS_R2)
 static_assert(2 * GIE_ZS_XW2 <= GIE_ZS_ROWS * GIE_ZS_XW, "the wide trip's row and its cy fit the wave's LDS rows");
+__device__ __forceinline__ uint32_t gie_zs_wide_col_bits(const uint64_t f, const int p, const int y, uint32_t &cy)
+{
+    const uint64_t hi = f >> p, lo = f << (63 - p);
+    const uint32_t ua = hi ? (uint32_t)__builtin_ctzll(hi) : 64u, ub = lo ? (uint32_t)__builtin_clzll(lo) : 64u;
+    const uint32_t d = min(ua, ub);
+    cy = ua <= ub ? (uint32_t)(y + (int)ua) : (uint32_t)(y - (int)ub);
+    return d <= (uint32_t)GIE_ZS_R2 ? (d * d << 6) : 0x3fffffc0u;
+}
+template <bool BITS>
 __device__ __forceinline__ bool gie_zs_wide_trip_fused(const __amdgpu_buffer_rsrc_t rs_cy, const __amdgpu_buffer_rsrc_t rs_out, gie_lds_u32 *srow, const unsigned voff,
                                                        const unsigned pstride, const unsigned ps2, const int zc, const int z1, const int Z, const int x0, const int x,
-                                                       const int y, const int X, const uint8_t *occ, const int lane)
+                                                       const int y, const int X, const int Y, const uint8_t *occ, const int lane)
 {
     const int xa = x0 - GIE_ZS_R2 + lane, xb = x0 + 64 - GIE_ZS_R2 + lane;
     const bool oka = xa >= 0 && xa < X, okb = lane < 2 * GIE_ZS_R2 && xb < X;
-    const unsigned voa = oka ? (unsigned)(y * X + xa) * 2u : GIE_BUF_OOB, vob = okb ? (unsigned)(y * X + xb) * 2u : GIE_BUF_OOB;
+    const int nb = (Y + 15) >> 4, b = y >> 4, p = (y & 15) + 24;
+    const unsigned es = BITS ? 4u : 2u, bs = (unsigned)X * 4u;
+    const unsigned voa = oka ? (unsigned)((BITS ? b * X : y * X) + xa) * es : GIE_BUF_OOB, vob = okb ? (unsigned)((BITS ? b * X : y * X) + xb) * es : GIE_BUF_OOB;
+    const unsigned bm = b > 0 ? bs : 0u, bp = b + 1 < nb ? bs : 0u;
+    const unsigned voa_m = oka ? voa - bm : GIE_BUF_OOB, vob_m = okb ? vob - bm : GIE_BUF_OOB, voa_p = oka ? voa + bp : GIE_BUF_OOB, vob_p = okb ? vob + bp : GIE_BUF_OOB;
+    constexpr int NB = BITS ? 4 : 8;
     gie_lds_u32 *sq = srow, *scy = srow + GIE_ZS_XW2;
     uint32_t best[GIE_ZS_C], bc[GIE_ZS_C];
 #pragma unroll
     for (int t = 0; t < GIE_ZS_C; t++) { best[t] = 0xffffffffu; bc[t] = GIE_BCOC_NONE; }
     const int lo = max(zc - GIE_ZS_R2, 0), hi = min(zc + GIE_ZS_C + GIE_ZS_R2, Z);
 #pragma unroll 1
-    for (int i0 = lo; i0 < hi; i0 += 8) {
-        uint16_t va[8], vb[8];
-#pragma unroll
-        for (int k = 0; k < 8; k++) {
+    for (int i0 = lo; i0 < hi; i0 += NB) {
+        uint16_t va[NB], vb[NB];
+        uint32_t wa[NB][2], wb[NB][2];
+#pragma unroll
+        for (int k = 0; k < NB; k++) {
             const unsigned so = (unsigned)min(i0 + k, Z - 1) * ps2;
-            va[k] = __builtin_amdgcn_raw_buffer_load_b16(rs_cy, voa, so, 0);
-            vb[k] = __builtin_amdgcn_raw_buffer_load_b16(rs_cy, vob, so, 0);
-        }
-#pragma unroll
-        for (int k = 0; k < 8; k++) {
+            if constexpr (BITS) {
+                wa[k][0] = __builtin_amdgcn_raw_buffer_load_b32(rs_cy, voa_m, so, 0); wa[k][1] = __builtin_amdgcn_raw_buffer_load_b32(rs_cy, voa_p, so, 0);
+                wb[k][0] = __builtin_amdgcn_raw_buffer_load_b32(rs_cy, vob_m, so, 0); wb[k][1] = __builtin_amdgcn_raw_buffer_load_b32(rs_cy, vob_p, so, 0);
+            } else {
+                va[k] = __builtin_amdgcn_raw_buffer_load_b16(rs_cy, voa, so, 0);
+                vb[k] = __builtin_amdgcn_raw_buffer_load_b16(rs_cy, vob, so, 0);
+            }
+        }
+#pragma unroll
+        for (int k = 0; k < NB; k++) {
             const int i = i0 + k;
             if (i >= hi || !occ[i]) continue;
-            {
+            if constexpr (BITS) {
+                uint32_t ca, cb;
+                const uint32_t qa = gie_zs_wide_col_bits((uint64_t)gie_yb_frame_half(wa[k][0], false, b, nb) | ((uint64_t)gie_yb_frame_half(wa[k][1], true, b, nb) << 32), p, y, ca);
+                const uint32_t qb = gie_zs_wide_col_bits((uint64_t)gie_yb_frame_half(wb[k][0], false, b, nb) | ((uint64_t)gie_yb_frame_half(wb[k][1], true, b, nb) << 32), p, y, cb);
+                sq[lane] = oka ? qa : 0x3fffffc0u; scy[lane] = ca;
+                if (lane < 2 * GIE_ZS_R2) { sq[64 + lane] = okb ? qb : 0x3fffffc0u; scy[64 + lane] = cb; }
+            } else {
                 const int da = y - (int)va[k], db = y - (int)vb[k];
                 sq[lane] = (oka && va[k] != 0xffffu) ? ((uint32_t)(da * da) << 6) : 0x3fffffc0u; scy[lane] = va[k];
                 if (lane < 2 * GIE_ZS_R2) { sq[64 + lane] = (okb && vb[k] != 0xffffu) ? ((uint32_t)(db * db) << 6) : 0x3fffffc0u; scy[64 + lane] = vb[k]; }
@@ -1215,9 +1293,10 @@
         __builtin_amdgcn_raw_buffer_store_b32(bc[t], rs_out, (zc + t < z1) ? voff : GIE_BUF_OOB, (unsigned)min(zc + t, Z - 1) * pstride, 0);
     return true;
 }
-template <bool FUSED>
-__global__ __launch_bounds__(256, FUSED ? GIE_ZS_FUSED_WGS : 6) void k_edt_z_stream(const gie_ctx c, const int full, const int nseg, const int seg_len, const int zs)
-{
+template <int FORM>
+__global__ __launch_bounds__(256, FORM == 3 ? GIE_ZS_BITS_WGS : FORM == 2 ? GIE_ZS_FUSED_WGS : 6) void k_edt_z_stream(const gie_ctx c, const int full, const int nseg, const int seg_len, const int zs)
+{
+    constexpr bool FUSED = FORM >= 2, BITS = FORM == 3;
     __shared__ uint8_t s_occ[1024 + 2 * (32 + 2 * GIE_ZS_R)];
     const int Z = c.Z, X = c.X, Y = c.Y;
     if (full == 0 && gie_z_use_lists(c, c.cnt[GIE_CNT_TL_KNOWN])) { gie_edt_z_direct_body(c); return; }
@@ -1232,9 +1311,11 @@
     const size_t plane = (size_t)X * Y;
     const unsigned nbytes = (unsigned)((size_t)X * Y * Z * 4u);
     const __amdgpu_buffer_rsrc_t rs_in = __builtin_amdgcn_make_buffer_rsrc(const_cast<uint32_t *>(c.cxy2), 0, nbytes, 0x00020000);
-    const __amdgpu_buffer_rsrc_t rs_cy = __builtin_amdgcn_make_buffer_rsrc(const_cast<uint16_t *>(c.cy1), 0, nbytes / 2u, 0x00020000);
+    const int nb = (Y + 15) >> 4;
+    const __amdgpu_buffer_rsrc_t rs_cy = BITS ? __builtin_amdgcn_make_buffer_rsrc(c.yb32, 0, (unsigned)((size_t)nb * X * Z * 4u), 0x00020000)
+                                              : __builtin_amdgcn_make_buffer_rsrc(const_cast<uint16_t *>(c.cy1), 0, nbytes / 2u, 0x00020000);
     const __amdgpu_buffer_rsrc_t rs_out = __builtin_amdgcn_make_buffer_rsrc(c.bcoc, 0, nbytes, 0x00020000);
-    const unsigned pstride = (unsigned)(plane * 4u), pstride2 = (unsigned)(plane * 2u);
+    const unsigned pstride = (unsigned)(plane * 4u), pstride2 = BITS ? (unsigned)nb * X * 4u : (unsigned)(plane * 2u);
     for (int w = (int)blockIdx.x * 4 + (int)(threadIdx.x >> 6); w < total; w += (int)gridDim.x * 4) {
         const int wu = __builtin_amdgcn_readfirstlane(w);
         const int xr = wu % nxr, seg = (wu / nxr) % nseg, y = wu / (nxr * nseg);
@@ -1246,12 +1327,13 @@
         uint32_t wk[GIE_ZS_W];
         const int xa = xr * 64 - GIE_ZS_R + 2 * lane;
         const bool oka = lane < GIE_ZS_XW / 2 && xa >= 0 && xa < X, okb = lane < GIE_ZS_XW / 2 && xa + 1 >= 0 && xa + 1 < X;
-        const unsigned vpa = (oka || okb) ? (unsigned)(y * X + xa) * 2u : GIE_BUF_OOB;
+        const unsigned vpa = (oka || okb) ? (BITS ? (unsigned)((y >> 4) * X + xa) * 4u : (unsigned)(y * X + xa) * 2u) : GIE_BUF_OOB;
+        const int yv = BITS ? (y & 15) + 8 : y + 8;
         uint32_t (*srow)[GIE_ZS_XW] = s_row[FUSED ? (threadIdx.x >> 6) : 0];
         if (FUSED) {
             const int zz = z0 - GIE_ZS_R + lane;
             const unsigned long long pm = __ballot(lane < 2 * GIE_ZS_R && s_occ[zz + GIE_ZS_W] != 0);
-            gie_zs_fused_keys<2 * GIE_ZS_R, 0, 0>(wk, srow, rs_cy, vpa, pstride2, z0 - GIE_ZS_R, Z, pm, oka, okb, y8, lane);
+            gie_zs_fused_keys<2 * GIE_ZS_R, 0, 0, BITS>(wk, srow, rs_cy, vpa, pstride2, z0 - GIE_ZS_R, Z, pm, oka, okb, yv, lane);
         } else {
             const int zz = z0 - GIE_ZS_R + lane;
             const unsigned long long pm = __ballot(lane < 2 * GIE_ZS_R && s_occ[zz + GIE_ZS_W] != 0);
@@ -1268,7 +1350,7 @@
             if (FUSED) {
                 const int zz = zc + GIE_ZS_R + lane;
                 const unsigned long long pm = __ballot(lane < GIE_ZS_C && s_occ[zz + GIE_ZS_W] != 0);
-                gie_zs_fused_keys<GIE_ZS_C, 2 * GIE_ZS_R, GIE_ZS_LDAUX>(wk, srow, rs_cy, vpa, pstride2, zc + GIE_ZS_R, Z, pm, oka, okb, y8, lane);
+                gie_zs_fused_keys<GIE_ZS_C, 2 * GIE_ZS_R, GIE_ZS_LDAUX, BITS>(wk, srow, rs_cy, vpa, pstride2, zc + GIE_ZS_R, Z, pm, oka, okb, yv, lane);
             } else {
                 const int zz = zc + GIE_ZS_R + lane;
                 const unsigned long long pm = __ballot(lane < GIE_ZS_C && s_occ[zz + GIE_ZS_W] != 0);
@@ -1316,8 +1398,8 @@
         if (FUSED) {
 #pragma unroll 1
             for (int k = 0; k < wide && !failed; k++)
-                failed = !gie_zs_wide_trip_fused(rs_cy, rs_out, (gie_lds_u32 *)&srow[0][0], voff, pstride, pstride2, __builtin_amdgcn_readfirstlane(k ? wz1 : wz0), z1, Z, xr * 64, x, y, X,
-                                                 s_occ + GIE_ZS_W, lane);
+                failed = !gie_zs_wide_trip_fused<BITS>(rs_cy, rs_out, (gie_lds_u32 *)&srow[0][0], voff, pstride, pstride2, __builtin_amdgcn_readfirstlane(k ? wz1 : wz0), z1, Z, xr * 64, x, y,
+                                                       X, Y, s_occ + GIE_ZS_W, lane);
         } else {
             if (!failed && wide > 0) failed = !gie_zs_wide_trip(c.cxy2, c.bcoc, nbytes, voff, pstride, wz0, z1, Z, x, y, x < X, s_occ + GIE_ZS_W);
             if (!failed && wide > 1) failed = !gie_zs_wide_trip(c.cxy2, c.bcoc, nbytes, voff, pstride, wz1, z1, Z, x, y, x < X, s_occ + GIE_ZS_W);
diff --git a/gie-mapping_amd/csrc/gie_types.h b/gie-mapping_amd/csrc/gie_types.h
--- a/gie-mapping_amd/csrc/gie_types.h
+++ b/gie-mapping_amd/csrc/gie_types.h
@@ -67,6 +67,7 @@
     int8_t *glb_type;
     float *edt;
     uint16_t *cy1;
+    uint32_t *yb32;
     uint32_t *cxy2;
     uint32_t *bcoc;
     uint64_t *pair;
```

New measurement: 96720 Mvoxels/s, median of 2. -2.2%, worse.
